# rvignav/diffusion-tts

Hardware: AMD Instinct MI355X
Metric: candidate U-Net steps/sec, EDM ImageNet-64 eps-greedy N=64 (higher is better)
Workload: dtype f16x3; 1 GPU; EDM ImageNet-64 (ADM 295.9M) eps-greedy search iteration, imagenet scorer, sigma step 5/18; candidates_total=64, candidates_per_gpu=64, scorer=imagenet, scorer_dtype=f16x3, denoiser_dtype=f16x3, graph_replay=True, parity_grade=True, parallelism=candidates sharded x1, 1 all-gather of rewards per step

## Files before the change

diffusion_tts_amd/_lib.py:

```python
import ctypes as C
import os

import torch

_HERE = os.path.dirname(os.path.abspath(__file__))
LIB_PATH = os.environ.get('DTS_LIB_PATH') or os.path.join(_HERE, 'libdts_hip.so')

DTS_F32, DTS_BF16, DTS_F16, DTS_F16X3 = 0, 1, 2, 3

_p, _i, _f, _d, _i64 = C.c_void_p, C.c_int, C.c_float, C.c_double, C.c_int64


class ConvArgs(C.Structure):
    _fields_ = [('x1', _p), ('c1', C.c_int32), ('x2', _p), ('c2', C.c_int32), ('w', _p), ('bias', _p),
                ('bias_nc', _p), ('ld_bias_nc', C.c_int32), ('residual', _p), ('out', _p),
                ('n', C.c_int32), ('hin', C.c_int32), ('win', C.c_int32), ('cout', C.c_int32),
                ('ksize', C.c_int32), ('up', C.c_int32), ('out_scale', C.c_float), ('dtype', C.c_int32),
                ('workspace', _p), ('workspace_bytes', C.c_int64), ('stats_out', _p), ('stats_written', C.c_int32),
                ('ev_start', _p), ('ev_stop', _p), ('gn_coef', _p), ('gn_silu', C.c_int32), ('acc_scale', C.c_float), ('out_split2', C.c_int32),
                ('skip_c', C.c_int32), ('skip_x', _p), ('skip_w', _p), ('skip_acc_scale', C.c_float), ('skip_up', C.c_int32)]


class ConvPlanInfo(C.Structure):
    _fields_ = [(f, C.c_int32) for f in ('kernel', 'tile', 'waves', 'stages', 'pf', 'gn', 'sk', 'dbg', 'splits', 'ks_per_split', 'n_ct', 'n_pt', 'nblk',
                                         'threads', 'lds_bytes', 'stats_in_kernel', 'stats_in_reduce', 'stats_written', 'epi_rows', 'fuses_gn',
                                         'folds_skip', 'refused', 'phases')]


SIGNATURES = {
    'dts_nchw_to_nhwc': [_p, _p, _i, _i, _i, _i, _i, _p],
    'dts_nhwc_to_nchw': [_p, _i, _p, _i, _i, _i, _i, _p],
    'dts_nchw_to_nhwc_pad': [_p, _p, _i, _i, _i, _i, _i, _i, _p],
    'dts_pack_conv_weight': [_p, _p, _i, _i, _i, _i, _i, _p, _p],
    'dts_conv2d': [C.POINTER(ConvArgs), _p],
    'dts_conv_in3': [_p, _p, _p, _p, _i, _i, _i, _i, _i, _p],
    'dts_conv_out3': [_p, _i, _p, _p, _p, _i, _i, _i, _i, _p],
    'dts_gn_coef': [_p, _i, _p, _i, _i, _i, _i, _i, _f, _p, _p, _p, _i, _p, _p, _p],
    'dts_gn_coef_strips': [_p, _i, _p, _i, _i, _i, _i, _i, _f, _p, _p, _p, _i, _p, _p],
    'dts_gn_apply': [_p, _i, _p, _i, _i, _p, _p, _i, _i, _i, _i, _i, _p],
    'dts_gn_apply_x3': [_p, _i, _p, _i, _p, _p, _p, _i, _i, _i, _i, _i, _p],
    'dts_gn_fused': [_p, _i, _p, _i, _i, _i, _i, _i, _f, _p, _p, _p, _i, _p, _i, _p],
    'dts_resample2x': [_p, _p, _i, _i, _i, _i, _i, _i, _p],
    'dts_resample_fir': [_p, _p, _i, _i, _i, _i, _i, _i, _i, _p],
    'dts_space_to_depth2': [_p, _i, _p, _i, _i, _i, _i, _i, _i, _i, _p],
    'dts_attention': [_p, _p, _i, _i, _i, _i, _i, _f, _p],
    'dts_attention_masked': [_p, _p, _i, _i, _i, _i, _i, _f, _i, _p, _p],
    'dts_cross_attention': [_p, _p, _p, _i, _p, _i, _i, _i, _i, _i, _i, _f, _p],
    'dts_layer_norm': [_p, _p, _i, _i64, _i, _f, _p, _p, _p],
    'dts_geglu': [_p, _p, _i, _i64, _i, _p],
    'dts_group_rows': [_p, _i, _i64, _p, _p, _p, _p, _p],
    'dts_patchify': [_p, _p, _i, _i, _i, _i, _i, _p],
    'dts_vit_tokens': [_p, _p, _p, _p, _i, _i, _i, _i, _p],
    'dts_text_tokens': [_p, _p, _p, _p, _i, _i, _i, _i, _i, _p],
    'dts_gelu': [_p, _p, _i, _i64, _i, _p],
    'dts_vit_head': [_p, _p, _i, _i, _i, _i, _f, _p, _p, _p],
    'dts_layer_norm_x3': [_p, _p, _p, _i64, _i, _f, _p, _p, _p],
    'dts_gelu_x3': [_p, _p, _i64, _i, _i, _p],
    'dts_patchify_x3': [_p, _p, _i, _i, _i, _i, _p],
    'dts_vit_tokens_f32': [_p, _p, _p, _p, _i, _i, _i, _p],
    'dts_vit_head_f32': [_p, _p, _i, _i, _i, _f, _p, _p, _p],
    'dts_text_tokens_f32': [_p, _p, _p, _p, _i, _i, _i, _i, _p],
    'dts_linear': [_p, _i, _p, _p, _p, _i, _i, _i, _i, _i, _i, _i, _p],
    'dts_pos_embedding': [_p, _p, _p, _i, _i, _i, _p],
    'dts_edm_precond_in': [_p, _p, _i, _f, _p, _p, _i, _i, _p],
    'dts_edm_precond_out': [_p, _p, _p, _p, _i, _i, _p],
    'dts_precond_in': [_i, _p, _p, _i, _p, _p, _i, _p, _p, _i, _i, _p],
    'dts_split3_f16': [_p, _i, _p, _i, _p, _i64, _p],
    'dts_split2_f16': [_p, _i, _p, _i64, _p],
    'dts_attention_x3': [_p, _p, _i, _i, _i, _i, _i, _f, _p],
    'dts_attention_x3_masked': [_p, _p, _i, _i, _i, _i, _i, _f, _i, _p, _p],
    'dts_cast_from_f32': [_p, _p, _i, _i64, _p],
    'dts_cast_to_f32': [_p, _i, _p, _i64, _p],
    'dts_heun_xhat': [_p, _i, _i, _p, _i, _d, _p, _i, _i, _p],
    'dts_heun_euler': [_p, _p, _d, _d, _p, _p, _i64, _p],
    'dts_heun_correct': [_p, _p, _p, _d, _d, _p, _i64, _p],
    'dts_ode_xhat': [_p, _p, _i, _d, _d, _d, _p, _p, _i64, _p],
    'dts_ode_slope': [_p, _p, _d, _d, _p, _d, _d, _p, _p, _p, _i64, _p],
    'dts_ode_correct': [_p, _p, _p, _p, _d, _d, _d, _d, _d, _p, _i64, _p],
    'dts_quantize_u8': [_p, _i, _p, _i64, _p],
    'dts_brightness': [_p, _p, _i, _i, _p],
    'dts_u8_to_unit_f32': [_p, _p, _i64, _p],
    'dts_resample_u8': [_p, _p, _i, _i, _i, _i, _i, _p, _p, _i, _p],
    'dts_lut_u8_f32': [_p, _p, _p, _i, _i, _i, _p],
    'dts_jpeg_size': [_p, _p, _i, _i, _i, _p, _p, _i64, _p, _p],
    'dts_cosine_rows': [_p, _p, _i, _p, _i, _i, _p],
    'dts_attnpool_tokens': [_p, _p, _p, _i, _i, _i, _i, _p],
    'dts_take_token': [_p, _i, _p, _i, _i, _i, _i, _p],
    'dts_softmax_gather': [_p, _p, _p, _i, _i, _p],
    'dts_candidate_noise': [_p, _p, _p, _p, _p, _i, _i, _i, _p],
    'dts_candidate_noise_rows': [_p, _p, _p, _p, _p, _i, _i, _i, _p],
    'dts_candidate_noise_sd': [_p, _p, _p, _p, _p, _i, _i, _i64, _p],
    'dts_candidate_noise_sd_rows': [_p, _p, _p, _p, _p, _i, _i, _i, _i64, _p],
    'dts_cfg_combine': [_p, _p, _f, _p, _i, _i64, _p],
    'dts_ddim_candidates': [_p, _p, _p, _p, _p, _i, _f, _f, _f, _i, _i64, _p],
    'dts_ddim_candidates_groups': [_p, _p, _p, _p, _p, _i, _f, _f, _f, _i, _i, _i64, _p],
}
OTHER = {'dts_version': ([], _i), 'dts_conv_fuses_gn': ([C.POINTER(ConvArgs)], _i), 'dts_conv_kernel': ([C.POINTER(ConvArgs)], _i), 'dts_conv_folds_skip': ([C.POINTER(ConvArgs)], _i), 'dts_conv_takes_phases': ([C.POINTER(ConvArgs)], _i), 'dts_conv_plan': ([C.POINTER(ConvArgs), C.POINTER(ConvPlanInfo)], _i), 'dts_set_tuning': ([_i, _i], _i), 'dts_get_tuning': ([_i], _i), 'dts_last_error': ([], C.c_char_p), 'dts_gn_ws_floats': ([_i, _i], _i64),
         'dts_jpeg_workspace_bytes': ([_i, _i, _i], _i64)}

_lib = None
ABI_VERSION = 125


def load():
    global _lib
    if _lib is not None:
        return _lib
    if not os.path.exists(LIB_PATH):
        raise RuntimeError(f'{LIB_PATH} not found: the HIP extension is required (no CPU fallback). '
                           f'Build it with `python -m diffusion_tts_amd.build` or __graft_entry__.build().')
    lib = C.CDLL(LIB_PATH)
    for name, argt in SIGNATURES.items():
        fn = getattr(lib, name)
        fn.argtypes, fn.restype = argt, _i
    for name, (argt, rest) in OTHER.items():
        fn = getattr(lib, name)
        fn.argtypes, fn.restype = argt, rest
    got = lib.dts_version()
    if got != ABI_VERSION or C.sizeof(ConvArgs) != 208:
        raise RuntimeError(f'{LIB_PATH} has ABI version {got}, this binding needs {ABI_VERSION}: rebuild with `python -m diffusion_tts_amd.build --force`')
    _lib = lib
    return lib


def check(status, what=''):
    if status != 0:
        msg = load().dts_last_error().decode(errors='replace')
        raise RuntimeError(f'libdts_hip {what} failed ({status}): {msg}')


KNOBS = {'att_xcd': 0, 'att_qt': 1, 'conv_tile': 2, 'conv_splits': 3, 'conv_variant': 4, 'gn_fuse': 5, 'att_db': 6, 'conv_stages': 7, 'conv_waves': 8, 'conv_half_round': 9, 'conv_epi32': 10, 'conv_skip_fold': 11, 'conv_up_phases': 12}


def set_tuning(name, value):
    check(load().dts_set_tuning(KNOBS[name], int(value)), 'dts_set_tuning')
```

diffusion_tts_amd/classifier.py:

```python
import math
from typing import Dict

import torch

from . import ops
from .config import ClassifierConfig, ClsLayer, classifier_layers


def _qkv_perm_legacy(heads: int, d: int) -> torch.Tensor:
    s, h, c = torch.meshgrid(torch.arange(3), torch.arange(heads), torch.arange(d), indexing='ij')
    return (h * 3 * d + s * d + c).reshape(-1).to(torch.int32)


class _P:
    pass


class EncoderUNetModel:
    def __init__(self, cfg: ClassifierConfig, state_dict: Dict[str, torch.Tensor], device='cuda', dtype=ops.F16X3):
        if not torch.cuda.is_available():
            raise RuntimeError('EncoderUNetModel (HIP) needs a GPU: there is no CPU fallback in this package')
        self.cfg, self.device, self.dtype = cfg, torch.device(device), dtype
        self.act_dtype = ops.act_dtype(dtype)
        self.x3 = dtype == ops.F16X3
        from .graphs import GraphCache
        self._graphs = GraphCache(self._device_forward)
        f = lambda t: t.detach().to(self.device, torch.float32).contiguous()
        sd, dt = state_dict, dtype
        mc = cfg.model_channels
        half = mc // 2
        self.freqs = torch.exp(-math.log(10000) * torch.arange(0, half, dtype=torch.float32) / half).to(self.device)
        self.te0_w, self.te0_b = f(sd['time_embed.0.weight']), f(sd['time_embed.0.bias'])
        self.te2_w, self.te2_b = f(sd['time_embed.2.weight']), f(sd['time_embed.2.bias'])
        self.layers, self.ch, self.res = classifier_layers(cfg)
        self.params: Dict[str, _P] = {}
        emb_w, emb_b, off = [], [], 0
        hc = cfg.num_head_channels
        for L in self.layers:
            P, p = _P(), L.prefix
            if L.kind == 'conv_in':
                P.w, P.b = f(sd[f'{p}.weight']), f(sd[f'{p}.bias'])
            elif L.kind == 'res':
                P.g0, P.b0 = f(sd[f'{p}.in_layers.0.weight']), f(sd[f'{p}.in_layers.0.bias'])
                P.w0, P.cb0 = ops.pack_conv_weight(f(sd[f'{p}.in_layers.2.weight']), dt), f(sd[f'{p}.in_layers.2.bias'])
                emb_w.append(sd[f'{p}.emb_layers.1.weight'])
                emb_b.append(sd[f'{p}.emb_layers.1.bias'])
                P.off, off = off, off + 2 * L.cout
                P.g1, P.b1 = f(sd[f'{p}.out_layers.0.weight']), f(sd[f'{p}.out_layers.0.bias'])
                P.w1, P.cb1 = ops.pack_conv_weight(f(sd[f'{p}.out_layers.3.weight']), dt), f(sd[f'{p}.out_layers.3.bias'])
                P.sw = P.sb = None
                if L.cin != L.cout:
                    P.sw, P.sb = ops.pack_conv_weight(f(sd[f'{p}.skip_connection.weight']), dt), f(sd[f'{p}.skip_connection.bias'])
                    P.cb1_skip = (P.cb1 + P.sb).contiguous()
            else:
                heads = L.cin // hc
                perm = _qkv_perm_legacy(heads, hc).to(self.device)
                P.g, P.b = f(sd[f'{p}.norm.weight']), f(sd[f'{p}.norm.bias'])
                P.wqkv = ops.pack_conv_weight(f(sd[f'{p}.qkv.weight']), dt, out_perm=perm)
                P.bqkv = f(sd[f'{p}.qkv.bias'])[perm.long()].contiguous()
                P.wproj, P.bproj = ops.pack_conv_weight(f(sd[f'{p}.proj_out.weight']), dt), f(sd[f'{p}.proj_out.bias'])
                P.heads = heads
            self.params[p] = P
        self.emb_w = ops.pack_conv_weight(f(torch.cat(emb_w, 0))[:, :, None, None].contiguous(), dt)
        self.emb_b = f(torch.cat(emb_b, 0))
        self.emb_total = off
        self.out_g, self.out_b = f(sd['out.0.weight']), f(sd['out.0.bias'])
        self.pos = f(sd['out.2.positional_embedding'])
        self.pool_wqkv = ops.pack_conv_weight(f(sd['out.2.qkv_proj.weight']), dt)
        self.pool_bqkv = f(sd['out.2.qkv_proj.bias'])
        self.cproj_w = f(sd['out.2.c_proj.weight']).reshape(cfg.out_channels, self.ch).contiguous()
        self.cproj_b = f(sd['out.2.c_proj.bias'])
        torch.cuda.synchronize(self.device)

    def _res(self, L: ClsLayer, x, emb_all):
        P = self.params[L.prefix]
        raw = self.x3 and P.sw is not None
        h = ops.group_norm(x, 32, 1e-5, P.g0, P.b0, silu=True, pool=L.down, split_out=self.x3, raw_split=raw)
        if raw:
            h, x = h
        elif L.down:
            x = ops.resample2x(x, up=False)
        h = ops.conv2d(h, P.w0, P.cb0, gn_stats=True)
        ss = emb_all[:, P.off:P.off + 2 * L.cout]
        h = ops.group_norm(h, 32, 1e-5, P.g1, P.b1, scale_shift=ss, silu=True, split_out=self.x3)
        if raw and ops.conv_folds_skip(h, P.w1, (x, P.sw, False)):
            return ops.conv2d(h, P.w1, P.cb1_skip, skip=(x, P.sw, False), gn_stats=True)
        sk = x if P.sw is None else ops.conv2d(x, P.sw, P.sb)
        return ops.conv2d(h, P.w1, P.cb1, residual=sk, gn_stats=True)

    def _attn(self, L: ClsLayer, x):
        P = self.params[L.prefix]
        n, hh, ww, c = x.shape
        hn = ops.group_norm(x, 32, 1e-5, P.g, P.b, silu=False, split_out=self.x3)
        fx3 = self.x3 and ops.attention_x3_ok(hh * ww, c // P.heads)
        qkv = ops.conv2d(hn, P.wqkv, P.bqkv, out_split2=fx3)
        a = ops.attention(qkv.view(n, hh * ww, 3 * c), P.heads, 1.0 / math.sqrt(c // P.heads), x3=self.x3, split_out=fx3)
        a = ops.SplitAct(a.data.view(n, hh, ww, 2 * c), c) if fx3 else a.view(n, hh, ww, c)
        return ops.conv2d(a, P.wproj, P.bproj, residual=x, gn_stats=True)

    @torch.no_grad()
    def __call__(self, x, timesteps):
        t = timesteps.to(self.device, torch.float32).contiguous()
        return self._graphs(x.to(self.device, torch.float32).contiguous(), t)

    @torch.no_grad()
    def _device_forward(self, x, t):
        n = x.shape[0]
        emb = ops.pos_embedding(t, self.freqs)
        emb = ops.linear(emb, self.te0_w, self.te0_b, act_out=True)
        emb = ops.linear(emb, self.te2_w, self.te2_b, act_out=True)
        e = ops.cast_from_f32(emb, self.act_dtype)
        emb_all = ops.conv2d(e.view(1, n, 1, -1), self.emb_w, self.emb_b).view(n, self.emb_total)
        h = None
        for L in self.layers:
            if L.kind == 'conv_in':
                P = self.params[L.prefix]
                h = ops.conv_in3(x.contiguous(), P.w, P.b, L.cout, self.act_dtype)
            elif L.kind == 'res':
                h = self._res(L, h, emb_all)
            else:
                h = self._attn(L, h)
        h = ops.group_norm(h, 32, 1e-5, self.out_g, self.out_b, silu=True)
        tok = ops.attnpool_tokens(h, self.pos)
        nt = tok.shape[1]
        qkv = ops.conv2d(tok.view(n, nt, 1, self.ch), self.pool_wqkv, self.pool_bqkv)
        heads = self.ch // self.cfg.num_head_channels
        a = ops.attention(qkv.view(n, nt, 3 * self.ch), heads, 1.0 / math.sqrt(self.cfg.num_head_channels), x3=self.x3)
        return ops.linear(ops.take_token(a, 0), self.cproj_w, self.cproj_b)
```

diffusion_tts_amd/csrc/conv_igemm.hip:

```cpp
#include "dts_common.h"
#include <hip/hip_ext.h>
#include <type_traits>

static_assert(sizeof(dts_conv_args) == 208, "dts_conv_args layout changed: bump DTS_ABI_VERSION and update the bindings (_lib.py ConvArgs)");

int dts_conv_launch_phase_form(const void* plan, const void* params, const void* call);

namespace {

struct ConvCall {
  hipStream_t st;
  hipEvent_t ev_start = nullptr, ev_stop = nullptr;
};

struct ConvP {
  const char* x1; const char* x2;
  const char* w;
  const float* bias;
  const char* bias_nc;
  const char* residual;
  char* out;
  int c1, c2, cin;
  int ld_bias_nc;
  int n, hin, win, hout, wout, cout;
  int taps;
  int up;
  int P;
  int n_ct;
  int n_pt;
  int splits;
  int ks_per_split;
  float* partial;
  float* stats;
  float out_scale;
  float acc_scale;
  int out_split2;
  int w_shift, hw_shift;
  const float* gn_coef;
  int gn_silu;
  int epi_rows;
  const char* sk_x; const char* sk_w;
  int sk_c, sk_up;
  float sk_ratio;
};

template <typename T> struct Mma;
template <> struct Mma<bf16_t> {
  static __device__ __forceinline__ void run(f32x4_t& acc, const uint4& a, const uint4& b) {
    acc = __builtin_amdgcn_mfma_f32_16x16x32_bf16(__builtin_bit_cast(bf16x8_t, a), __builtin_bit_cast(bf16x8_t, b), acc, 0, 0, 0);
  }
};
template <> struct Mma<f16_t> {
  static __device__ __forceinline__ void run(f32x4_t& acc, const uint4& a, const uint4& b) {
    acc = __builtin_amdgcn_mfma_f32_16x16x32_f16(__builtin_bit_cast(f16x8_t, a), __builtin_bit_cast(f16x8_t, b), acc, 0, 0, 0);
  }
};
template <> struct Mma<float> {
  static __device__ __forceinline__ void run(f32x4_t& acc, const uint4& a, const uint4& b) {
    acc = __builtin_amdgcn_mfma_f32_16x16x4f32(__builtin_bit_cast(float, a.x), __builtin_bit_cast(float, b.x), acc, 0, 0, 0);
    acc = __builtin_amdgcn_mfma_f32_16x16x4f32(__builtin_bit_cast(float, a.y), __builtin_bit_cast(float, b.y), acc, 0, 0, 0);
    acc = __builtin_amdgcn_mfma_f32_16x16x4f32(__builtin_bit_cast(float, a.z), __builtin_bit_cast(float, b.z), acc, 0, 0, 0);
    acc = __builtin_amdgcn_mfma_f32_16x16x4f32(__builtin_bit_cast(float, a.w), __builtin_bit_cast(float, b.w), acc, 0, 0, 0);
  }
};

__device__ __forceinline__ uint4 f16x8_mul_2m11(const uint4& v) {
  const f16x8_t h = __builtin_bit_cast(f16x8_t, v) * (_Float16)0x1p-11f;
  return __builtin_bit_cast(uint4, h);
}

template <typename T> struct Vec4;
template <> struct Vec4<float> {
  using type = float4;
  static __device__ __forceinline__ void unpack(const float4& v, float* f) { f[0] = v.x; f[1] = v.y; f[2] = v.z; f[3] = v.w; }
  static __device__ __forceinline__ float4 pack(const float* f) { return make_float4(f[0], f[1], f[2], f[3]); }
  static __device__ __forceinline__ void load(const float* p, float* f) {
    const float4 v = *reinterpret_cast<const float4*>(p);
    f[0] = v.x; f[1] = v.y; f[2] = v.z; f[3] = v.w;
  }
  static __device__ __forceinline__ void store(float* p, const float* f) {
    *reinterpret_cast<float4*>(p) = make_float4(f[0], f[1], f[2], f[3]);
  }
};
template <> struct Vec4<bf16_t> {
  using type = uint2;
  static __device__ __forceinline__ uint2 pack(const float* f) {
    return make_uint2(pack2_bf16(f[0], f[1]), pack2_bf16(f[2], f[3]));
  }
  static __device__ __forceinline__ void unpack(const uint2& v, float* f) {
    f[0] = __builtin_bit_cast(float, v.x << 16); f[1] = __builtin_bit_cast(float, v.x & 0xffff0000u);
    f[2] = __builtin_bit_cast(float, v.y << 16); f[3] = __builtin_bit_cast(float, v.y & 0xffff0000u);
  }
  static __device__ __forceinline__ void load(const bf16_t* p, float* f) {
    const uint2 v = *reinterpret_cast<const uint2*>(p);
    f[0] = bf16_bits_to_f32(v.x & 0xffffu); f[1] = bf16_bits_to_f32(v.x >> 16);
    f[2] = bf16_bits_to_f32(v.y & 0xffffu); f[3] = bf16_bits_to_f32(v.y >> 16);
  }
  static __device__ __forceinline__ void store(bf16_t* p, const float* f) {
    *reinterpret_cast<uint2*>(p) = make_uint2(pack2_bf16(f[0], f[1]), pack2_bf16(f[2], f[3]));
  }
};
template <> struct Vec4<f16_t> {
  using type = uint2;
  static __device__ __forceinline__ uint2 pack(const float* f) {
    return make_uint2(pack2_f16(f[0], f[1]), pack2_f16(f[2], f[3]));
  }
  static __device__ __forceinline__ void unpack(const uint2& v, float* f) {
    f[0] = f16_bits_to_f32(v.x & 0xffffu); f[1] = f16_bits_to_f32(v.x >> 16);
    f[2] = f16_bits_to_f32(v.y & 0xffffu); f[3] = f16_bits_to_f32(v.y >> 16);
  }
  static __device__ __forceinline__ void load(const f16_t* p, float* f) {
    const uint2 v = *reinterpret_cast<const uint2*>(p);
    f[0] = f16_bits_to_f32(v.x & 0xffffu); f[1] = f16_bits_to_f32(v.x >> 16);
    f[2] = f16_bits_to_f32(v.y & 0xffffu); f[3] = f16_bits_to_f32(v.y >> 16);
  }
  static __device__ __forceinline__ void store(f16_t* p, const float* f) {
    *reinterpret_cast<uint2*>(p) = make_uint2(pack2_f16(f[0], f[1]), pack2_f16(f[2], f[3]));
  }
};

#ifdef DTS_STAMPS
__device__ unsigned long long g_stamps[8192 * 8];
#define DTS_STAMP(slot_)                                                                                       \
  if (threadIdx.x == 0 && (blockIdx.x + blockIdx.y * gridDim.x) < 8192) {                                       \
    unsigned long long t_;                                                                                      \
    asm volatile("s_memtime %0\n\ts_waitcnt lgkmcnt(0)" : "=s"(t_)::"memory");                                 \
    g_stamps[(blockIdx.x + blockIdx.y * gridDim.x) * 8 + (slot_)] = t_;                                         \
  }
// ... 150 lines not shown
    const int hw = kp.hout * kp.wout;
#pragma unroll
    for (int nt = 0; nt < NT; ++nt) {
      const int pp = tm.pix(prow0 + nt * 16);
      np[nt] = bnc + (size_t)(kp.hw_shift >= 0 ? pp >> kp.hw_shift : pp / hw) * kp.ld_bias_nc + cm0 + col0;
    }
  }
  constexpr bool want_stats = STATS && NT == 4;
  float* sp = want_stats ? kp.stats + ((size_t)tm.strip(wn) * p_cout + cm0 + col0) * 2 : nullptr;
  char* sw = smem + prow0 * ROWB + (lq & 1) * 8;
  int coff[MT];
#pragma unroll
  for (int mt = 0; mt < MT; ++mt) coff[mt] = (((wm * 2 * MT + 2 * mt + (lq >> 1)) ^ (lrow & 7)) << 4);
  const float osc = kp.out_scale;
  if constexpr (RES) {
    if (early_u0 > 0 || early_u1 < ITERS) {
      asm volatile("s_waitcnt vmcnt(0)" ::: "memory");
      __syncthreads();
    }
  }
#pragma unroll
  for (int mt = 0; mt < MT; ++mt) {
    V4 nv[NT], rv[NT];
    if constexpr (BNC) {
#pragma unroll
      for (int nt = 0; nt < NT; ++nt) nv[nt] = *reinterpret_cast<const V4*>(np[nt] + mt * 16);
    }
    if constexpr (RES) {
#pragma unroll
      for (int nt = 0; nt < NT; ++nt) rv[nt] = *reinterpret_cast<const V4*>(sw + nt * 16 * ROWB + coff[mt]);
    }
    typedef float f32x2 __attribute__((ext_vector_type(2)));
    f32x2 ssa = {0.f, 0.f}, ssb = {0.f, 0.f}, sqa = {0.f, 0.f}, sqb = {0.f, 0.f};
#pragma unroll
    for (int nt = 0; nt < NT; ++nt) {
      f32x2 va = {acc[mt][nt][0], acc[mt][nt][1]}, vb = {acc[mt][nt][2], acc[mt][nt][3]};
      if constexpr (BNC) {
        float f[4];
        Vec4<T>::unpack(nv[nt], f);
        va += f32x2{f[0], f[1]}; vb += f32x2{f[2], f[3]};
      }
      if constexpr (RES) {
        float f[4];
        Vec4<T>::unpack(rv[nt], f);
        va += f32x2{f[0], f[1]}; vb += f32x2{f[2], f[3]};
      }
      va *= osc; vb *= osc;
      const float v[4] = {va.x, va.y, vb.x, vb.y};
      const V4 pk = Vec4<T>::pack(v);
      *reinterpret_cast<V4*>(sw + nt * 16 * ROWB + coff[mt]) = pk;
      if constexpr (want_stats) {
        float f[4];
        Vec4<T>::unpack(pk, f);
        const f32x2 fa = {f[0], f[1]}, fb = {f[2], f[3]};
        ssa += fa; ssb += fb;
        sqa = __builtin_elementwise_fma(fa, fa, sqa); sqb = __builtin_elementwise_fma(fb, fb, sqb);
      }
    }
    if constexpr (want_stats) {
      float ss4[4] = {ssa.x, ssa.y, ssb.x, ssb.y}, sq4[4] = {sqa.x, sqa.y, sqb.x, sqb.y};
      row16_sum8(ss4, sq4);
      if (lrow == 0) {
        float4* d = reinterpret_cast<float4*>(sp + mt * 32);
        d[0] = make_float4(ss4[0], sq4[0], ss4[1], sq4[1]);
        d[1] = make_float4(ss4[2], sq4[2], ss4[3], sq4[3]);
      }
    }
  }
  DTS_STAMP(6);
  __syncthreads();
  DTS_STAMP(7);
  int row = tid / CPR, c = tid - row * CPR;
  char* outb = kp.out + (size_t)cm0 * 2;
  typedef unsigned int u32x4_nt __attribute__((ext_vector_type(4)));
#pragma unroll
  for (int u = 0; u < ITERS; ++u) {
    const u32x4_nt v_ = *reinterpret_cast<const u32x4_nt*>(smem + row * ROWB + c * 16);
    __builtin_nontemporal_store(v_, reinterpret_cast<u32x4_nt*>(outb + (size_t)tm.pix(row) * rstride + ((c ^ (row & 7)) << 4)));
    row += DR; c += DC;
    if (c >= CPR) { c -= CPR; ++row; }
  }
}

template <int MT, int NT, typename TM = TileMap>
__device__ __forceinline__ void conv_epilogue_rows_f32(const ConvP& kp, f32x4_t (&acc)[MT][NT], int cm0, const TM& tm, int wm, int wn,
                                                       int lrow, int lq, char* smem, int wave) {
  static_assert(NT == 4, "64-pixel wave strips");
  constexpr int CW = 16 * MT;
  constexpr int LPR = 4 * MT;
  constexpr int RPI = LPR <= 8 ? 8 : (LPR <= 16 ? 4 : 2);
  constexpr int ITERS = 32 / RPI;
  constexpr int ROWB = CW * 4 + 16;
  char* const ws = smem + (size_t)wave * (32 * ROWB);
  const int lane = threadIdx.x & 63;
  const int rsub = lane / LPR, c4 = lane - rsub * LPR;
  const bool act = rsub < RPI;
  const int p_cout = kp.cout;
  const int co = cm0 + wm * CW + c4 * 4;
  const float* __restrict__ res = reinterpret_cast<const float*>(kp.residual);
  if (tm.pix(wn * 64) >= kp.P) return;
  float4 b4 = make_float4(0.f, 0.f, 0.f, 0.f), n4 = make_float4(0.f, 0.f, 0.f, 0.f);
  if (act) {
    if (kp.bias) b4 = *reinterpret_cast<const float4*>(kp.bias + co);
    if (kp.bias_nc) {
      const int pp0 = tm.pix(wn * 64), hw = kp.hout * kp.wout;
      n4 = *reinterpret_cast<const float4*>(reinterpret_cast<const float*>(kp.bias_nc) + (size_t)(kp.hw_shift >= 0 ? pp0 >> kp.hw_shift : pp0 / hw) * kp.ld_bias_nc + co);
    }
  }
  const float asc = kp.acc_scale, osc = kp.out_scale;
  const bool want_stats = kp.stats != nullptr;
  float ss4[4] = {0.f, 0.f, 0.f, 0.f}, sq4[4] = {0.f, 0.f, 0.f, 0.f};
  typedef float f32x4_nt __attribute__((ext_vector_type(4)));
  constexpr int CH = ITERS < 8 ? ITERS : 8;
#pragma unroll
  for (int half = 0; half < 2; ++half) {
#pragma unroll
    for (int n2 = 0; n2 < 2; ++n2)
#pragma unroll
      for (int mt = 0; mt < MT; ++mt)
        *reinterpret_cast<f32x4_t*>(ws + (n2 * 16 + lrow) * ROWB + (mt * 16 + lq * 4) * 4) = acc[mt][half * 2 + n2];
#pragma unroll
   for (int u0 = 0; u0 < ITERS; u0 += CH) {
    size_t prow[CH];
    float4 rv[CH];
#pragma unroll
    for (int u = 0; u < CH; ++u) {
      prow[u] = (size_t)tm.pix(wn * 64 + half * 32 + (u0 + u) * RPI + (act ? rsub : 0)) * p_cout + co;
      rv[u] = make_float4(0.f, 0.f, 0.f, 0.f);
      if (res && act) rv[u] = *reinterpret_cast<const float4*>(res + prow[u]);
    }
#pragma unroll
    for (int u = 0; u < CH; ++u) {
      if (!act) continue;
      const f32x4_t a = *reinterpret_cast<const f32x4_t*>(ws + ((u0 + u) * RPI + rsub) * ROWB + c4 * 16);
      float v[4] = {a[0] * asc + b4.x, a[1] * asc + b4.y, a[2] * asc + b4.z, a[3] * asc + b4.w};
      if (kp.bias_nc) { v[0] += n4.x; v[1] += n4.y; v[2] += n4.z; v[3] += n4.w; }
      if (res) { v[0] += rv[u].x; v[1] += rv[u].y; v[2] += rv[u].z; v[3] += rv[u].w; }
#pragma unroll
      for (int r = 0; r < 4; ++r) v[r] *= osc;
      if (kp.out_split2) {
        float hi[4], lo[4];
#pragma unroll
        for (int r = 0; r < 4; ++r) x2_split(v[r], hi[r], lo[r]);
        const uint2 h = make_uint2(pack2_f16(hi[0], hi[1]), pack2_f16(hi[2], hi[3])), l = make_uint2(pack2_f16(lo[0], lo[1]), pack2_f16(lo[2], lo[3]));
        const bool odd = (c4 & 1) != 0;
        const uint32_t rx = (uint32_t)__builtin_amdgcn_update_dpp(0, (int)(odd ? h.x : l.x), 0xB1, 0xf, 0xf, false);
        const uint32_t ry = (uint32_t)__builtin_amdgcn_update_dpp(0, (int)(odd ? h.y : l.y), 0xB1, 0xf, 0xf, false);
        if (kp.epi_rows == 2) {
          f16_t* o8 = reinterpret_cast<f16_t*>(kp.out) + 2 * (prow[u] - co) + co;
          *reinterpret_cast<uint2*>(o8) = h;
          *reinterpret_cast<uint2*>(o8 + p_cout) = l;
          continue;
        }
        f16_t* orow = reinterpret_cast<f16_t*>(kp.out) + 2 * (prow[u] - co) + (odd ? co - 4 + p_cout : co);
        *reinterpret_cast<uint4*>(orow) = odd ? make_uint4(rx, ry, l.x, l.y) : make_uint4(h.x, h.y, rx, ry);
      } else {
        const f32x4_nt o = {v[0], v[1], v[2], v[3]};
        __builtin_nontemporal_store(o, reinterpret_cast<f32x4_nt*>(reinterpret_cast<float*>(kp.out) + prow[u]));
      }
      if (want_stats) {
#pragma unroll
        for (int r = 0; r < 4; ++r) { ss4[r] += v[r]; sq4[r] += v[r] * v[r]; }
      }
    }
   }
  }
  if (want_stats) {
#pragma unroll
    for (int r = 0; r < 4; ++r) {
      float s_ = ss4[r], q_ = sq4[r];
#pragma unroll
      for (int k = 1; k < RPI; ++k) { s_ += __shfl(ss4[r], c4 + k * LPR, 64); q_ += __shfl(sq4[r], c4 + k * LPR, 64); }
      ss4[r] = s_; sq4[r] = q_;
    }
    if (rsub == 0) {
      float4* d = reinterpret_cast<float4*>(kp.stats + ((size_t)tm.strip(wn) * p_cout + co) * 2);
      d[0] = make_float4(ss4[0], sq4[0], ss4[1], sq4[1]);
      d[1] = make_float4(ss4[2], sq4[2], ss4[3], sq4[3]);
    }
  }
}

template <typename T, int MT, int NT, int BM, int BN, int NTHR, int RING, typename TM = TileMap>
__device__ __forceinline__ void conv_epilogue(const ConvP& kp, f32x4_t (&acc)[MT][NT], int cm0, const TM& tm, int split, int wm, int wn,
                                              int lrow, int lq, char* smem, bool bias_in_acc, int stage_off, int early_u0, int early_u1) {
  const int p_P = kp.P, p_cout = kp.cout, p_hout = kp.hout, p_wout = kp.wout;
  if (kp.splits > 1) {
    float* part = kp.partial + (size_t)split * p_P * p_cout;
#pragma unroll
    for (int nt = 0; nt < NT; ++nt) {
      const int pp = tm.pix(wn * 16 * NT + nt * 16 + lrow);
      if (pp >= p_P) continue;
#pragma unroll
      for (int mt = 0; mt < MT; ++mt) {
        const int co = cm0 + wm * 16 * MT + mt * 16 + lq * 4;
        *reinterpret_cast<float4*>(part + (size_t)pp * p_cout + co) =
            make_float4(acc[mt][nt][0], acc[mt][nt][1], acc[mt][nt][2], acc[mt][nt][3]);
      }
    }
    return;
  }
  if constexpr (sizeof(T) == 4 && NT == 4) {
    constexpr int NWV = NTHR / 64;
    static_assert(NWV * 32 * (16 * MT * 4 + 16) <= RING, "the waves' private transpose slices must fit the caller's LDS ring");
    if (kp.epi_rows && (p_hout * p_wout) % 64 == 0) {
      conv_epilogue_rows_f32<MT, NT>(kp, acc, cm0, tm, wm, wn, lrow, lq, smem, (int)(threadIdx.x >> 6));
      return;
    }
  }
  if constexpr (sizeof(T) == 2) {
    if (tm.pn0 + BN <= p_P) {
      const bool r_ = kp.residual != nullptr, b_ = kp.bias_nc != nullptr, s_ = NT == 4 && kp.stats != nullptr;
#define DTS_EPI(R_, B_, S_) conv_epilogue_fast<T, MT, NT, BM, BN, R_, B_, S_, NTHR>(kp, acc, cm0, tm, wm, wn, lrow, lq, smem, bias_in_acc, stage_off, early_u0, early_u1)
      if (r_) { if (b_) { if (s_) DTS_EPI(true, true, true); else DTS_EPI(true, true, false); }
                else    { if (s_) DTS_EPI(true, false, true); else DTS_EPI(true, false, false); } }
      else    { if (b_) { if (s_) DTS_EPI(false, true, true); else DTS_EPI(false, true, false); }
                else    { if (s_) DTS_EPI(false, false, true); else DTS_EPI(false, false, false); } }
#undef DTS_EPI
      return;
    }
  }
  const T* __restrict__ res = reinterpret_cast<const T*>(kp.residual);
  const T* __restrict__ bnc = reinterpret_cast<const T*>(kp.bias_nc);
  T* __restrict__ out = reinterpret_cast<T*>(kp.out);
  const int hw = p_hout * p_wout;
  using V4 = typename Vec4<T>::type;
  int ppv[NT], nsv[NT];
#pragma unroll
  for (int nt = 0; nt < NT; ++nt) {
    const int pp = tm.pix(wn * 16 * NT + nt * 16 + lrow);
    ppv[nt] = pp < p_P ? pp : -1;
    nsv[nt] = pp < p_P ? pp / hw : 0;
  }
  constexpr int RG = (sizeof(T) == 4 && MT > 4) ? 2 : MT;
  static_assert(MT % RG == 0, "residual slice groups");
  V4 rv[RG][NT], nv[NT];
  float4 bv[MT];
#pragma unroll
  for (int mt = 0; mt < MT; ++mt)
    bv[mt] = (kp.bias && !bias_in_acc) ? *reinterpret_cast<const float4*>(kp.bias + cm0 + wm * 16 * MT + mt * 16 + lq * 4) : make_float4(0.f, 0.f, 0.f, 0.f);
  const float asc = kp.acc_scale;
  constexpr bool VIA_LDS = sizeof(T) == 2;
  constexpr int ROWP = BM * 2 + 16;
  static_assert(!VIA_LDS || BN * ROWP <= RING, "staged tile must fit the caller's LDS ring");
  const bool want_stats = NT == 4 && kp.stats != nullptr;
  float* sp = want_stats ? kp.stats + ((size_t)tm.strip(wn) * p_cout) * 2 : nullptr;
#pragma unroll
  for (int mt = 0; mt < MT; ++mt) {
    const int co = cm0 + wm * 16 * MT + mt * 16 + lq * 4;
    const float4 bcur = bv[mt];
    if (res && mt % RG == 0) {
#pragma unroll
      for (int m2 = 0; m2 < RG; ++m2) {
        const int co_ = cm0 + wm * 16 * MT + (mt + m2) * 16 + lq * 4;
#pragma unroll
        for (int nt = 0; nt < NT; ++nt)
          if (ppv[nt] >= 0) rv[m2][nt] = *reinterpret_cast<const V4*>(res + (size_t)ppv[nt] * p_cout + co_);
      }
    }
    if (bnc) {
#pragma unroll
      for (int nt = 0; nt < NT; ++nt)
        if (ppv[nt] >= 0) nv[nt] = *reinterpret_cast<const V4*>(bnc + (size_t)nsv[nt] * kp.ld_bias_nc + co);
    }
    float ss4[4] = {0.f, 0.f, 0.f, 0.f}, sq4[4] = {0.f, 0.f, 0.f, 0.f};
#pragma unroll
    for (int nt = 0; nt < NT; ++nt) {
      if (ppv[nt] < 0) continue;
      float v[4];
      v[0] = acc[mt][nt][0] * asc + bcur.x; v[1] = acc[mt][nt][1] * asc + bcur.y;
      v[2] = acc[mt][nt][2] * asc + bcur.z; v[3] = acc[mt][nt][3] * asc + bcur.w;
      if (bnc) {
        float f[4];
        Vec4<T>::unpack(nv[nt], f);
#pragma unroll
        for (int r = 0; r < 4; ++r) v[r] += f[r];
      }
      if (res) {
        float f[4];
        Vec4<T>::unpack(rv[mt % RG][nt], f);
#pragma unroll
        for (int r = 0; r < 4; ++r) v[r] += f[r];
      }
#pragma unroll
      for (int r = 0; r < 4; ++r) v[r] *= kp.out_scale;
      const V4 pk = Vec4<T>::pack(v);
      if constexpr (VIA_LDS)
        *reinterpret_cast<V4*>(smem + (wn * 16 * NT + nt * 16 + lrow) * ROWP + (wm * 16 * MT + mt * 16 + lq * 4) * 2) = pk;
      else if (sizeof(T) == 4 && kp.out_split2) {
        float hi[4], lo[4];
#pragma unroll
        for (int r = 0; r < 4; ++r) x2_split(v[r], hi[r], lo[r]);
        f16_t* orow = reinterpret_cast<f16_t*>(kp.out) + (size_t)ppv[nt] * 2 * p_cout + co;
        *reinterpret_cast<uint2*>(orow) = make_uint2(pack2_f16(hi[0], hi[1]), pack2_f16(hi[2], hi[3]));
        *reinterpret_cast<uint2*>(orow + p_cout) = make_uint2(pack2_f16(lo[0], lo[1]), pack2_f16(lo[2], lo[3]));
      } else
        *reinterpret_cast<V4*>(out + (size_t)ppv[nt] * p_cout + co) = pk;
      if (want_stats) {
        float f[4];
        Vec4<T>::unpack(pk, f);
#pragma unroll
        for (int r = 0; r < 4; ++r) { ss4[r] += f[r]; sq4[r] += f[r] * f[r]; }
      }
    }
    if (want_stats) {
#pragma unroll
      for (int r = 0; r < 4; ++r) {
#pragma unroll
        for (int o = 1; o < 16; o <<= 1) { ss4[r] += __shfl_xor(ss4[r], o, 64); sq4[r] += __shfl_xor(sq4[r], o, 64); }
      }
      if (lrow == 0 && tm.pix(wn * 64) < p_P) {
        float4* d = reinterpret_cast<float4*>(sp + (size_t)co * 2);
        d[0] = make_float4(ss4[0], sq4[0], ss4[1], sq4[1]);
        d[1] = make_float4(ss4[2], sq4[2], ss4[3], sq4[3]);
      }
    }
  }
  if constexpr (VIA_LDS) {
    __syncthreads();
    constexpr int CPR = BM / 8;
    char* outb = kp.out + (size_t)cm0 * 2;
    const int rows = min(BN, p_P - tm.pn0);
#pragma unroll 4
    for (int t = threadIdx.x; t < rows * CPR; t += NTHR) {
      const int row = t / CPR, c = t - row * CPR;
      typedef unsigned int u32x4_nt __attribute__((ext_vector_type(4)));
      const u32x4_nt v_ = *reinterpret_cast<const u32x4_nt*>(smem + row * ROWP + c * 16);
      __builtin_nontemporal_store(v_, reinterpret_cast<u32x4_nt*>(outb + (size_t)tm.pix(row) * p_cout * 2 + c * 16));
    }
  }
}

template <typename T, int MT, int NT, int WM, int WN, bool PF, int STAGES = 2, typename OT = T, bool PH = false>
__global__ __launch_bounds__(64 * WM * WN, (WM * WN == 8 || STAGES == 2 ? 2 : 1)) void conv_igemm_kernel(const ConvP kp) {
  const char* const p_x1 = kp.x1; const char* const p_x2 = kp.x2; const char* const p_w = kp.w;
  const int p_c1 = kp.c1, p_c2 = kp.c2, p_cin = kp.cin, p_hin = kp.hin, p_win = kp.win, p_hout = kp.hout, p_wout = kp.wout;
  const int p_taps = kp.taps, p_up = kp.up, p_P = kp.P, p_n_ct = kp.n_ct, p_n_pt = kp.n_pt;
  constexpr int NW = WM * WN;
  constexpr bool X3I = !std::is_same<T, OT>::value;
  static_assert(!X3I || std::is_same<T, f16_t>::value, "split precision runs on the f16 matrix instruction");
  static_assert(!PH || X3I, "the phase form is the split-precision mode's");
  static_assert(NW == 4 || NW == 8, "4 or 8 waves");
  static_assert(STAGES >= 2 && STAGES <= 4, "ring depth");
  constexpr int SLAB = 8 * NW;
  constexpr int BM = 16 * MT * WM;
  constexpr int BN = 16 * NT * WN;
  constexpr int EPV = ET<T>::EPV;
  constexpr int BKE = 8 * EPV;
  constexpr int ES = 16 / EPV;
  constexpr int RA = BM / SLAB;
  constexpr int RB = BN / SLAB;
  static_assert(BM % SLAB == 0 && BN % SLAB == 0, "tile rows must split over the waves x 8 rows");
  constexpr int A_BYTES = BM * 128, B_BYTES = BN * 128, STAGE_BYTES = A_BYTES + B_BYTES;
  extern __shared__ __attribute__((aligned(16))) char smem[];
  DTS_STAMP_RT(4);
  DTS_STAMP(0);

  const int nblk = p_n_ct * p_n_pt * (PH ? 4 : 1);
  int bid = blockIdx.x;
  {
    const int q = nblk >> 3, r = nblk & 7, xcd = bid & 7, j = bid >> 3;
    bid = (xcd < r ? xcd * (q + 1) : r * (q + 1) + (xcd - r) * q) + j;
  }
  const int ct = bid % p_n_ct, pt = PH ? (bid / p_n_ct) >> 2 : bid / p_n_ct;
  const int cm0 = ct * BM, pn0 = pt * BN;
  const int phase = PH ? (bid / p_n_ct) & 3 : 0, ph_y = phase >> 1, ph_x = phase & 1;
  const int g_h = PH ? p_hin : p_hout, g_w = PH ? p_win : p_wout, g_P = PH ? p_P >> 2 : p_P;
  const int g_hw_shift = PH ? kp.hw_shift - 2 : kp.hw_shift, g_w_shift = PH ? kp.w_shift - 1 : kp.w_shift;

  const int tid = threadIdx.x, lane = tid & 63, wid = tid >> 6;
  const int wm = wid % WM, wn = wid / WM;
  const int chunk = tid & 7, r0 = tid >> 3;

  int pix_n[RB], pix_hw[RB];
  const int K = p_taps * p_cin;
  const int steps_per_tap = p_cin / BKE;
  const int nk_all = p_taps * steps_per_tap;
  const int ks_begin = blockIdx.y * kp.ks_per_split;
  const int ks_end = min(nk_all, ks_begin + kp.ks_per_split);

  const int schunk = (chunk ^ (r0 & 7)) * 16;
  const char* zsrc = reinterpret_cast<const char*>(g_zero16);
  const char* arow[RA];
  const char* brow[RB];
  const uint32_t lds_base = (uint32_t)(uintptr_t)(__attribute__((address_space(3))) char*)smem;
  const uint32_t wave_rows = __builtin_amdgcn_readfirstlane(lds_base + (tid >> 6) * 8 * 128);

#define SET_ROWS(tap_, ci0_)                                                                                  \
  {                                                                                                           \
    const int dh_ = PH ? ((tap_) >> 1) - 1 + ph_y : ((p_taps == 9) ? (tap_) / 3 - 1 : 0);                     \
    const int dw_ = PH ? ((tap_) & 1) - 1 + ph_x : ((p_taps == 9) ? (tap_) % 3 - 1 : 0);                      \
    const char* xb; int cs, cofs;                                                                             \
    if ((ci0_) < p_c1) { xb = p_x1; cs = p_c1; cofs = (ci0_); } else { xb = p_x2; cs = p_c2; cofs = (ci0_) - p_c1; } \
    _Pragma("unroll") for (int j = 0; j < RB; ++j) {                                                          \
      const int hu = (pix_hw[j] >> 16) + dh_, wu = (pix_hw[j] & 0xffff) + dw_;                                \
      const bool ok = pix_n[j] >= 0 && (unsigned)hu < (unsigned)g_h && (unsigned)wu < (unsigned)g_w;          \
      const int hs = (!PH && p_up) ? (hu >> 1) : hu, ws = (!PH && p_up) ? (wu >> 1) : wu;                     \
      brow[j] = ok ? xb + ((size_t)(pix_n[j] + hs * p_win + ws) * cs + cofs) * ES + schunk : zsrc;            \
    }                                                                                                         \
  }
#define ISSUE_TILE(buf_)                                                                                      \
  {                                                                                                           \
    const uint32_t sa_ = wave_rows + (buf_) * STAGE_BYTES;                                                    \
    const uint32_t sb_ = sa_ + A_BYTES;                                                                       \
    _Pragma("unroll") for (int j = 0; j < RA; ++j) glds16(arow[j], sa_ + j * SLAB * 128);                     \
    _Pragma("unroll") for (int j = 0; j < RB; ++j) glds16(brow[j], sb_ + j * SLAB * 128);                     \
  }
#define ADVANCE_K()                                                                                           \
  {                                                                                                           \
    ci0 += BKE;                                                                                               \
    _Pragma("unroll") for (int j = 0; j < RA; ++j) arow[j] += BKE * ES;                                       \
    if (ci0 == p_cin) { ci0 = 0; ++tap; SET_ROWS(tap, 0); }                                                   \
    else if (ci0 == p_c1) { SET_ROWS(tap, ci0); }                                                             \
    else { _Pragma("unroll") for (int j = 0; j < RB; ++j) brow[j] += BKE * ES; }                              \
  }

// ... 61 lines not shown
  static_assert(STAGED_BYTES % PIECE == 0 && STAGED_BYTES <= RING_BYTES, "staged tile pieces");
  const bool res_early = sizeof(OT) == 2 && kp.residual != nullptr && kp.splits == 1 && pn0 + BN <= p_P;
  int stage_off = 0, early_u0 = 0, early_u1 = 0;
  int buf = 0;
  for (int ks = ks_begin; ks < ks_end; ++ks) {
    const char* sa = smem + buf * STAGE_BYTES + (wm * 16 * MT) * 128;
    const char* sb = smem + buf * STAGE_BYTES + A_BYTES + (wn * 16 * NT) * 128;
    uint4 fa[MT], fb[NT], ga[MT], gb[NT];
#pragma unroll
    for (int i = 0; i < NT; ++i) fb[i] = *reinterpret_cast<const uint4*>(sb + swz(i * 16 + lrow, lq));
#pragma unroll
    for (int i = 0; i < MT; ++i) fa[i] = *reinterpret_cast<const uint4*>(sa + swz(i * 16 + lrow, lq));
    if (PF) {
#pragma unroll
      for (int i = 0; i < NT; ++i) gb[i] = *reinterpret_cast<const uint4*>(sb + swz(i * 16 + lrow, lq + 4));
#pragma unroll
      for (int i = 0; i < MT; ++i) ga[i] = *reinterpret_cast<const uint4*>(sa + swz(i * 16 + lrow, lq + 4));
    }
    if (ks + STAGES - 1 < ks_end) {
      ADVANCE_K();
      int wr = buf + STAGES - 1;
      if (wr >= STAGES) wr -= STAGES;
      ISSUE_TILE(wr);
    } else if (res_early && ks + 1 == ks_end) {
      const int lo_free = buf * STAGE_BYTES, hi_free = (STAGES - 1 - buf) * STAGE_BYTES;
      int f0, f1;
      if (lo_free >= hi_free) { f0 = 0; f1 = lo_free; stage_off = 0; }
      else { f0 = (buf + 1) * STAGE_BYTES; f1 = RING_BYTES; stage_off = min(f0, RING_BYTES - STAGED_BYTES); }
      early_u0 = max(0, (f0 - stage_off + PIECE - 1) / PIECE);
      early_u1 = min(PIECES, max(0, (f1 - stage_off) / PIECE));
      if (early_u1 < early_u0) early_u1 = early_u0;
      issue_residual_pieces<BM, 64 * NW>(kp, cm0, linear_tile(pn0), lds_base + stage_off, tid, early_u0, early_u1);
    }
    uint4 fs[X3I ? MT : 1];
    if constexpr (X3I) {
#pragma unroll
      for (int i = 0; i < MT; ++i) fs[i] = f16x8_mul_2m11(fa[i]);
    }
    __builtin_amdgcn_s_setprio(1);
#pragma unroll
    for (int i = 0; i < MT; ++i)
#pragma unroll
      for (int j = 0; j < NT; ++j) Mma<T>::run(acc[i][j], fa[i], fb[j]);
    if (!PF) {
      __builtin_amdgcn_s_setprio(0);
#pragma unroll
      for (int i = 0; i < NT; ++i) gb[i] = *reinterpret_cast<const uint4*>(sb + swz(i * 16 + lrow, lq + 4));
#pragma unroll
      for (int i = 0; i < MT; ++i) ga[i] = *reinterpret_cast<const uint4*>(sa + swz(i * 16 + lrow, lq + 4));
      __builtin_amdgcn_s_setprio(1);
    }
    if constexpr (X3I) {
#pragma unroll
      for (int i = 0; i < MT; ++i)
#pragma unroll
        for (int j = 0; j < NT; ++j) Mma<T>::run(acc[i][j], fs[i], gb[j]);
#pragma unroll
      for (int i = 0; i < MT; ++i)
#pragma unroll
        for (int j = 0; j < NT; ++j) Mma<T>::run(acc[i][j], ga[i], fb[j]);
    } else {
#pragma unroll
      for (int i = 0; i < MT; ++i)
#pragma unroll
        for (int j = 0; j < NT; ++j) Mma<T>::run(acc[i][j], ga[i], gb[j]);
    }
    __builtin_amdgcn_s_setprio(0);
    if constexpr (STAGES > 2) {
      const int later = min(STAGES - 2, ks_end - 2 - ks);
      if (later >= 2) asm volatile("s_waitcnt vmcnt(%0) lgkmcnt(0)" ::"n"(2 * LPT) : "memory");
      else if (later == 1) asm volatile("s_waitcnt vmcnt(%0) lgkmcnt(0)" ::"n"(LPT) : "memory");
      else asm volatile("s_waitcnt vmcnt(0) lgkmcnt(0)" ::: "memory");
    } else {
      asm volatile("s_waitcnt vmcnt(0) lgkmcnt(0)" ::: "memory");
    }
    __syncthreads();
    if (++buf == STAGES) buf = 0;
  }

  DTS_STAMP(2);
  if constexpr (PH) {
    const bool sh = kp.hw_shift >= 0;
    const PhaseTileMap tm{pn0, ph_y, ph_x, p_win, p_hin * p_win, sh ? g_w_shift : -1, sh ? g_hw_shift : -1};
    conv_epilogue<OT, MT, NT, BM, BN, 64 * NW, RING_BYTES>(kp, acc, cm0, tm, (int)blockIdx.y, wm, wn, lrow, lq, smem, bias_in_acc, stage_off, early_u0, early_u1);
  } else
  conv_epilogue<OT, MT, NT, BM, BN, 64 * NW, RING_BYTES>(kp, acc, cm0, linear_tile(pn0), (int)blockIdx.y, wm, wn, lrow, lq, smem, bias_in_acc, stage_off, early_u0, early_u1);
  DTS_STAMP(3);
  DTS_STAMP_RT(5);
}
#undef SET_ROWS
#undef ISSUE_TILE
#undef ADVANCE_K

template <typename T>
__device__ __forceinline__ uint4 gn_act8(const uint4 v, const float (&ca)[8], const float (&cb)[8], int silu) {
  float f[8];
  unpack16<T>(v, f);
#pragma unroll
  for (int e = 0; e < 8; ++e) {
    const float y = f[e] * ca[e] + cb[e];
    f[e] = silu ? y * __builtin_amdgcn_rcpf(1.0f + __expf(-y)) : y;
  }
  return pack16<T>(f);
}

template <typename T, int TAPS, int DBG = 0, bool GN = false, int MT = 6, typename OT = T, bool SK = false>
__global__ __launch_bounds__(512, 2) void conv_pp_kernel(const ConvP kp) {
  static_assert(MT == 6 || MT == 4, "cout tile");
  constexpr bool X3I = !std::is_same<T, OT>::value;
  static_assert(!X3I || (std::is_same<T, f16_t>::value && DBG == 0 && !GN), "split precision: the shipped f16 form only");
  constexpr int NT = 4, GM = 16 * MT, BM = 2 * GM, BN = 256, NTHR = 512, AJ = MT / 2;
  constexpr int BKE = 64, ES = 2;
  constexpr int A_HALF = GM * 128, A_RING = 3 * A_HALF, H_OFF = 2 * A_RING, H_BUF = 328 * 128;
  extern __shared__ __attribute__((aligned(16))) char smem[];
  DTS_STAMP_RT(4);
  DTS_STAMP(0);
  const char* const p_x1 = kp.x1; const char* const p_x2 = kp.x2; const char* const p_w = kp.w;
  const int p_c1 = kp.c1, p_c2 = kp.c2, p_cin = kp.cin, W = kp.wout, H = kp.hout, Wi = kp.win, Hi = kp.hin, ups = kp.up ? 1 : 0;
  constexpr int p_taps = TAPS;
  const int p_n_ct = kp.n_ct, p_n_pt = kp.n_pt;

  const int nblk = p_n_ct * p_n_pt;
  int bid = blockIdx.x;
  {
    const int q = nblk >> 3, r = nblk & 7, xcd = bid & 7, j = bid >> 3;
    bid = (xcd < r ? xcd * (q + 1) : r * (q + 1) + (xcd - r) * q) + j;
  }
  const int ct = bid % p_n_ct, pt = bid / p_n_ct;
  const int cm0 = ct * BM;

  const int tid = threadIdx.x, lane = tid & 63;
  const int w = __builtin_amdgcn_readfirstlane(tid >> 6);
  const int grp = w >> 2, wi = w & 3;
  const int wm = grp, wn = wi;
  const int chunk = lane & 7, r0 = lane >> 3;
  const int lrow = lane & 15, lq = lane >> 4;

  const int hw = H * W;
  TileMap tm;
  tm.pn0 = pt * BN; tm.w = W;
  int img0, y0 = 0, x0 = 0;
  if (W >= 32) {
    const int tpr = W >> 4, tpi = tpr * (H >> 4);
    const int tin = pt & (tpi - 1);
    img0 = pt / tpi;
    y0 = (tin / tpr) << 4; x0 = (tin & (tpr - 1)) << 4;
    tm.patch = 1; tm.porg = img0 * hw + y0 * W + x0;
    tm.strip0 = img0 * (hw >> 6) + tin * 4;
  } else {
    img0 = tm.pn0 / hw;
    tm.patch = 0; tm.porg = 0; tm.strip0 = tm.pn0 >> 6;
  }
  constexpr int bd = (p_taps == 9) ? 1 : 0;
  constexpr int hwid = 16 + 2 * bd;
  constexpr int hr_total = hwid * hwid;
  constexpr int npieces = (hr_total + 7) / 8;
  constexpr int NHP = (npieces + 7) / 8;

  const int K = p_taps * p_cin;
  const int nk_all = p_taps * (p_cin / BKE);
  const int ks_begin = blockIdx.y * kp.ks_per_split;
  const int ks_end = min(nk_all, ks_begin + kp.ks_per_split);
  const int nk = ks_end - ks_begin;

  const int schunk = (chunk ^ (r0 & 7)) * 16;
  const uint32_t lds_base = (uint32_t)(uintptr_t)(__attribute__((address_space(3))) char*)smem;

  const dts_i32x4 rs_w = make_rsrc(p_w, (uint32_t)((size_t)kp.cout * K * ES));
  uint32_t avo[AJ];
#pragma unroll
  for (int j = 0; j < AJ; ++j) avo[j] = DBG == 5 ? DTS_OOR : (uint32_t)((cm0 + grp * GM + 8 * (wi + 4 * j) + r0) * K) * ES + schunk;
  const uint32_t a_dst = lds_base + grp * A_RING + (8 * wi) * 128;
  const uint32_t h_dst = lds_base + H_OFF + (8 * w) * 128;

  int hpix[NHP];
#pragma unroll
  for (int j = 0; j < NHP; ++j) {
    const int hr = 8 * (w + 8 * j) + r0;
    hpix[j] = -1;
    if (hr < hr_total) {
      const int hy = hr / hwid, hx = hr - hy * hwid;
      const int y = y0 + hy - bd, x = x0 + hx - bd;
      if ((unsigned)y < (unsigned)H && (unsigned)x < (unsigned)W) hpix[j] = (img0 * Hi + (y >> ups)) * Wi + (x >> ups);
    }
  }
  uint32_t hvo[NHP];
  uint32_t hval = 0;
#pragma unroll
  for (int j = 0; j < NHP; ++j) hval |= (hpix[j] >= 0 ? 1u : 0u) << j;
// ... 250 lines not shown
    static_assert(X3I, "skip fold: split precision only");
    const int sC = kp.sk_c, nks = sC / BKE, su = kp.sk_up & 1, Hs = H >> su, Ws = W >> su;
    const float ratio = kp.sk_ratio;
#pragma unroll
    for (int i = 0; i < MT; ++i)
#pragma unroll
      for (int j = 0; j < NT; ++j) acc[i][j] *= ratio;
    constexpr int S_A = BM * 128, S_B = BN * 128, B_OFF = 2 * S_A;
    static_assert(B_OFF + 3 * S_B <= H_OFF + 2 * H_BUF, "skip fold: the rings fit the kernel's LDS");
    dts_i32x4 rs_sw = make_rsrc(kp.sk_w, (uint32_t)((size_t)kp.cout * sC * ES));
    dts_i32x4 rs_sx = make_rsrc(kp.sk_x, (uint32_t)((size_t)kp.n * Hs * Ws * sC * ES));
#pragma unroll
    for (int e = 0; e < 4; ++e) { rs_sw[e] = __builtin_amdgcn_readfirstlane(rs_sw[e]); rs_sx[e] = __builtin_amdgcn_readfirstlane(rs_sx[e]); }
    uint32_t savo[AJ], sbvo[4];
#pragma unroll
    for (int j = 0; j < AJ; ++j) savo[j] = (uint32_t)((cm0 + 8 * (w + 8 * j) + r0) * sC) * ES + schunk;
#pragma unroll
    for (int j = 0; j < 4; ++j) {
      const int pl = 8 * (w + 8 * j) + r0, y = y0 + (pl >> 4), x = x0 + (pl & 15);
      sbvo[j] = (uint32_t)(((img0 * Hs + (y >> su)) * Ws + (x >> su)) * sC) * ES + schunk;
    }
    const uint32_t sa_dst = lds_base + (8 * w) * 128, sb_dst = lds_base + B_OFF + (8 * w) * 128;
#define SK_ISSUE_A(kt_, slot_)                                                                                 \
    {                                                                                                         \
      const uint32_t so_ = (uint32_t)(kt_) * 128u, d_ = sa_dst + (uint32_t)(slot_) * S_A;                      \
      _Pragma("unroll") for (int j = 0; j < AJ; ++j) bdma16(savo[j], rs_sw, so_, d_ + j * (64 * 128));         \
    }
#define SK_ISSUE_B(kt_, slot_)                                                                                 \
    {                                                                                                         \
      const uint32_t so_ = (uint32_t)(kt_) * 128u, d_ = sb_dst + (uint32_t)(slot_) * S_B;                      \
      _Pragma("unroll") for (int j = 0; j < 4; ++j) bdma16(sbvo[j], rs_sx, so_, d_ + j * (64 * 128));          \
    }
    SK_ISSUE_A(0, 0);
    SK_ISSUE_B(0, 0);
    if (nks > 1) SK_ISSUE_B(1, 1);
    int bs = 0;
#pragma unroll 1
    for (int kt = 0; kt < nks; ++kt) {
      if (kt + 1 < nks) asm volatile("s_waitcnt vmcnt(4)" ::: "memory");
      else asm volatile("s_waitcnt vmcnt(0)" ::: "memory");
      asm volatile("s_barrier" ::: "memory");
      __builtin_amdgcn_sched_barrier(0);
      const int as = kt & 1;
      if (kt + 1 < nks) SK_ISSUE_A(kt + 1, as ^ 1);
      if (kt + 2 < nks) SK_ISSUE_B(kt + 2, bs == 0 ? 2 : bs - 1);
      const char* sa = smem + as * S_A + (grp * GM) * 128;
      const char* sb = smem + B_OFF + bs * S_B;
      bs = bs == 2 ? 0 : bs + 1;
      uint4 fa[MT], fb[NT], ga[MT], gb[NT], fs[MT];
#pragma unroll
      for (int i = 0; i < NT; ++i) fb[i] = *reinterpret_cast<const uint4*>(sb + swz(wn * 64 + i * 16 + lrow, lq));
#pragma unroll
      for (int i = 0; i < MT; ++i) fa[i] = *reinterpret_cast<const uint4*>(sa + swz(i * 16 + lrow, lq));
#pragma unroll
      for (int i = 0; i < NT; ++i) gb[i] = *reinterpret_cast<const uint4*>(sb + (swz(wn * 64 + i * 16 + lrow, lq) ^ 64));
#pragma unroll
      for (int i = 0; i < MT; ++i) ga[i] = *reinterpret_cast<const uint4*>(sa + (swz(i * 16 + lrow, lq) ^ 64));
      __builtin_amdgcn_sched_barrier(0);
#pragma unroll
      for (int i = 0; i < MT; ++i) fs[i] = f16x8_mul_2m11(fa[i]);
      __builtin_amdgcn_sched_barrier(0);
      __builtin_amdgcn_s_setprio(1);
#pragma unroll
      for (int i = 0; i < MT; ++i)
#pragma unroll
        for (int j = 0; j < NT; ++j) Mma<T>::run(acc[i][j], fa[i], fb[j]);
#pragma unroll
      for (int i = 0; i < MT; ++i)
#pragma unroll
        for (int j = 0; j < NT; ++j) Mma<T>::run(acc[i][j], fs[i], gb[j]);
#pragma unroll
      for (int i = 0; i < MT; ++i)
#pragma unroll
        for (int j = 0; j < NT; ++j) Mma<T>::run(acc[i][j], ga[i], fb[j]);
      __builtin_amdgcn_s_setprio(0);
      __builtin_amdgcn_sched_barrier(0);
    }
#undef SK_ISSUE_A
#undef SK_ISSUE_B
  }
  __syncthreads();
  DTS_STAMP(2);

  conv_epilogue<OT, MT, NT, BM, BN, NTHR, H_OFF + 2 * H_BUF>(kp, acc, cm0, tm, (int)blockIdx.y, wm, wn, lrow, lq, smem, bias_in_acc, 0, 0, 0);
  DTS_STAMP(3);
  DTS_STAMP_RT(5);
}

template <typename T, int SPLITS>
__global__ __launch_bounds__(256) void conv_splitk_reduce_kernel(const ConvP kp) {
  const long long total = (long long)kp.P * (kp.cout / 4);
  const T* res = reinterpret_cast<const T*>(kp.residual);
  const T* bnc = reinterpret_cast<const T*>(kp.bias_nc);
  T* out = reinterpret_cast<T*>(kp.out);
  const int hw = kp.hout * kp.wout, c4 = kp.cout / 4;
  const size_t slab = (size_t)kp.P * kp.cout;
  for (long long idx = (long long)blockIdx.x * blockDim.x + threadIdx.x; idx < total; idx += (long long)gridDim.x * blockDim.x) {
    const int pp = (int)(idx / c4), co = (int)(idx - (long long)pp * c4) * 4;
    const float* base = kp.partial + (size_t)pp * kp.cout + co;
    float4 q[SPLITS];
#pragma unroll
    for (int s = 0; s < SPLITS; ++s) q[s] = *reinterpret_cast<const float4*>(base + (size_t)s * slab);
    float v[4] = {0.f, 0.f, 0.f, 0.f};
#pragma unroll
    for (int s = 0; s < SPLITS; ++s) { v[0] += q[s].x; v[1] += q[s].y; v[2] += q[s].z; v[3] += q[s].w; }
    for (int r = 0; r < 4; ++r) v[r] *= kp.acc_scale;
    if (kp.bias) {
      const float4 bv = *reinterpret_cast<const float4*>(kp.bias + co);
      v[0] += bv.x; v[1] += bv.y; v[2] += bv.z; v[3] += bv.w;
    }
    if (bnc) {
      float f[4];
      Vec4<T>::load(bnc + (size_t)(pp / hw) * kp.ld_bias_nc + co, f);
      for (int r = 0; r < 4; ++r) v[r] += f[r];
    }
    if (res) {
      float f[4];
      Vec4<T>::load(res + (size_t)pp * kp.cout + co, f);
      for (int r = 0; r < 4; ++r) v[r] += f[r];
    }
    for (int r = 0; r < 4; ++r) v[r] *= kp.out_scale;
    Vec4<T>::store(out + (size_t)pp * kp.cout + co, v);
  }
}

template <typename T, int SPLITS>
__global__ __launch_bounds__(256) void conv_splitk_reduce_stats_kernel(const ConvP kp) {
  __shared__ float red[16][16][8];
  const int strip = blockIdx.x, q = threadIdx.x & 15, pl = threadIdx.x >> 4;
  const int co = (blockIdx.y * 16 + q) * 4;
  const bool live = co < kp.cout;
  const T* res = reinterpret_cast<const T*>(kp.residual);
  const T* bnc = reinterpret_cast<const T*>(kp.bias_nc);
  T* out = reinterpret_cast<T*>(kp.out);
  const int hw = kp.hout * kp.wout;
  float ss[4] = {0.f, 0.f, 0.f, 0.f}, sq[4] = {0.f, 0.f, 0.f, 0.f};
  if (live) {
    const int p0 = strip * 64 + pl;
    float v[4][4];
#pragma unroll
    for (int i = 0; i < 4; ++i) { v[i][0] = v[i][1] = v[i][2] = v[i][3] = 0.f; }
    {
      const float* base = kp.partial + (size_t)p0 * kp.cout + co;
      const size_t slab = (size_t)kp.P * kp.cout;
      float4 t4[SPLITS][4];
#pragma unroll
      for (int s_ = 0; s_ < SPLITS; ++s_)
#pragma unroll
        for (int i = 0; i < 4; ++i) t4[s_][i] = *reinterpret_cast<const float4*>(base + (size_t)s_ * slab + (size_t)(16 * i) * kp.cout);
#pragma unroll
      for (int s_ = 0; s_ < SPLITS; ++s_)
#pragma unroll
        for (int i = 0; i < 4; ++i) { v[i][0] += t4[s_][i].x; v[i][1] += t4[s_][i].y; v[i][2] += t4[s_][i].z; v[i][3] += t4[s_][i].w; }
    }
    float4 bv = make_float4(0.f, 0.f, 0.f, 0.f);
    if (kp.bias) bv = *reinterpret_cast<const float4*>(kp.bias + co);
    float nb[4] = {0.f, 0.f, 0.f, 0.f};
    if (bnc) Vec4<T>::load(bnc + (size_t)((strip * 64) / hw) * kp.ld_bias_nc + co, nb);
#pragma unroll
    for (int i = 0; i < 4; ++i) {
      const int pp = p0 + 16 * i;
      for (int r = 0; r < 4; ++r) v[i][r] *= kp.acc_scale;
      v[i][0] += bv.x; v[i][1] += bv.y; v[i][2] += bv.z; v[i][3] += bv.w;
      if (bnc) { for (int r = 0; r < 4; ++r) v[i][r] += nb[r]; }
      if (res) {
        float f[4];
        Vec4<T>::load(res + (size_t)pp * kp.cout + co, f);
        for (int r = 0; r < 4; ++r) v[i][r] += f[r];
      }
      for (int r = 0; r < 4; ++r) v[i][r] *= kp.out_scale;
      const typename Vec4<T>::type pk = Vec4<T>::pack(v[i]);
      *reinterpret_cast<typename Vec4<T>::type*>(out + (size_t)pp * kp.cout + co) = pk;
      float f[4];
      Vec4<T>::unpack(pk, f);
      for (int r = 0; r < 4; ++r) { ss[r] += f[r]; sq[r] += f[r] * f[r]; }
    }
  }
  for (int r = 0; r < 4; ++r) { red[pl][q][2 * r] = ss[r]; red[pl][q][2 * r + 1] = sq[r]; }
  __syncthreads();
  if (pl == 0 && live) {
    float o[8];
    for (int j = 0; j < 8; ++j) {
      float a_ = red[0][q][j];
      for (int k = 1; k < 16; ++k) a_ += red[k][q][j];
      o[j] = a_;
    }
    float4* d = reinterpret_cast<float4*>(kp.stats + ((size_t)strip * kp.cout + co) * 2);
    d[0] = make_float4(o[0], o[1], o[2], o[3]);
    d[1] = make_float4(o[4], o[5], o[6], o[7]);
  }
}

constexpr int DTS_MAX_DEVICES = 64;
inline int current_device() {
  int d = 0;
  if (hipGetDevice(&d) != hipSuccess || d < 0 || d >= DTS_MAX_DEVICES) d = 0;
  return d;
}

template <typename T, int SPLITS>
int launch_reduce_n(const ConvP& q, bool with_stats, hipStream_t st) {
  if (with_stats) {
    hipLaunchKernelGGL((conv_splitk_reduce_stats_kernel<T, SPLITS>), dim3(q.P / 64, (q.cout + 63) / 64), dim3(256), 0, st, q);
    DTS_CHECK_LAUNCH("dts_conv2d(split-K reduce + statistics)");
  } else {
    long long g = ((long long)q.P * (q.cout / 4) + 255) / 256;
    if (g > 2048) g = 2048;
    hipLaunchKernelGGL((conv_splitk_reduce_kernel<T, SPLITS>), dim3((int)g), dim3(256), 0, st, q);
    DTS_CHECK_LAUNCH("dts_conv2d(split-K reduce)");
  }
  return DTS_OK;
}
template <typename T>
int launch_reduce(const ConvP& q, bool with_stats, hipStream_t st) {
  switch (q.splits) {
    case 2: return launch_reduce_n<T, 2>(q, with_stats, st);
    case 3: return launch_reduce_n<T, 3>(q, with_stats, st);
    case 4: return launch_reduce_n<T, 4>(q, with_stats, st);
    case 5: return launch_reduce_n<T, 5>(q, with_stats, st);
    case 6: return launch_reduce_n<T, 6>(q, with_stats, st);
    case 7: return launch_reduce_n<T, 7>(q, with_stats, st);
    case 8: return launch_reduce_n<T, 8>(q, with_stats, st);
    default: dts_set_error("dts_conv2d: split-K factor %d outside 2..8", q.splits); return DTS_ERR_ARG;
  }
}


struct ConvKnobs { int variant, tile, splits, stages, waves, half_round, epi32, skip_fold, up_phases; bool f32_tile192; };
ConvKnobs conv_knobs() {
  static const bool f32_192 = !(getenv("DTS_F32_TILE192") && atoi(getenv("DTS_F32_TILE192")) == 0);
  return {dts_knob_get(DTS_KNOB_CONV_VARIANT), dts_knob_get(DTS_KNOB_CONV_TILE), dts_knob_get(DTS_KNOB_CONV_SPLITS),
          dts_knob_get(DTS_KNOB_CONV_STAGES), dts_knob_get(DTS_KNOB_CONV_WAVES), dts_knob_get(DTS_KNOB_CONV_HALF_ROUND),
          dts_knob_get(DTS_KNOB_CONV_EPI32), dts_knob_get(DTS_KNOB_CONV_SKIP_FOLD), dts_knob_get(DTS_KNOB_CONV_UP_PHASES), f32_192};
}

struct ConvPlan : dts_conv_plan_info { char refuse[200]; };

template <auto KERNEL>
int conv_launch(const ConvPlan& pl, const ConvP& q, const ConvCall& call) {
  static bool attr_done[DTS_MAX_DEVICES] = {};
  const int dev = current_device();
  if (!attr_done[dev]) {
    (void)hipFuncSetAttribute(reinterpret_cast<const void*>(KERNEL), hipFuncAttributeMaxDynamicSharedMemorySize, pl.lds_bytes);
    attr_done[dev] = true;
  }
  const dim3 grid(pl.nblk, pl.splits), block(pl.threads);
  if (call.ev_start != nullptr && call.ev_stop != nullptr)
    hipExtLaunchKernelGGL(KERNEL, grid, block, (size_t)pl.lds_bytes, call.st, call.ev_start, call.ev_stop, 0, q);
  else
    hipLaunchKernelGGL(KERNEL, grid, block, (size_t)pl.lds_bytes, call.st, q);
  DTS_CHECK_LAUNCH(pl.kernel != 0 ? "dts_conv2d(ping-pong)" : "dts_conv2d");
  return DTS_OK;
}

template <typename T, typename OT, int MT, int WM, int WN, bool PF, bool PH = false>
int conv_launch_igemm(const ConvPlan& pl, const ConvP& q, const ConvCall& call) {
#define DTS_IGEMM(MT_, WM_, STAGES_) conv_launch<&conv_igemm_kernel<T, MT_, 4, WM_, WN, PF, STAGES_, OT, PH>>(pl, q, call)
  if constexpr (sizeof(T) == 2) {
    if (pl.waves == 8) return pl.stages == 3 ? DTS_IGEMM(MT / 2, WM * 2, 3) : DTS_IGEMM(MT / 2, WM * 2, 2);
    if (pl.stages == 3) return DTS_IGEMM(MT, WM, 3);
    if constexpr (std::is_same<T, OT>::value)
      if (pl.stages == 4) return DTS_IGEMM(MT, WM, 4);
  }
  return DTS_IGEMM(MT, WM, 2);
#undef DTS_IGEMM
}

int igemm_splits(int nblk, int nk, double slab, bool can8, bool x3, bool ws, long long ws_bytes, int forced) {
  const int slots = 512;
  int splits = 1;
  if (ws && nblk < (slots * 3) / 4 && nk >= 16) {
    int smax = 8;
    if (smax > nk / 8) smax = nk / 8;
    while (smax > 1 && (long long)smax * (long long)slab > ws_bytes) --smax;
    if (smax < 1) smax = 1;
    const double KS = x3 ? 1.5 : 1.0;
    auto est = [&](int s_) {
      const int steps = (nk + s_ - 1) / s_;
      double t;
      if (can8 && (long long)nblk * s_ <= 256) t = 5.0 + steps * 0.75 * KS;
      else t = (double)((nblk * s_ + slots - 1) / slots) * (5.5 + steps * 1.25 * KS);
      if (s_ > 1) t += 3.0 + (s_ + 0.5) * slab / 4.0e6;
      return t;
    };
    int best = 1;
    for (int s_ = 2; s_ <= smax; ++s_)
      if (est(s_) < est(best)) best = s_;
    splits = best;
  }
  const int f8 = forced > 8 ? 8 : forced;
  if (f8 > 0 && ws && nk >= 2 * f8 && (long long)f8 * (long long)slab <= ws_bytes) splits = f8;
  return splits;
}

inline bool pp_considers_split(long long nblk) { return nblk < 192; }

int pp_splits(int nblk, int nk, double slab, bool x3, bool ws, long long ws_bytes, int forced) {
  int splits = 1;
  if (!ws || nk < 16) return splits;
  if (forced > 0) splits = forced;
  else if (pp_considers_split(nblk)) {
    const int nchunk = nk / 9;
    double best = 1e30;
    for (int s_ = 1; s_ <= 8 && s_ <= nchunk; ++s_) {
      const int cps = (nchunk + s_ - 1) / s_, se = (nchunk + cps - 1) / cps;
      if (se != s_ || nblk * se > 256) continue;
      double t = 5.0 + cps * 9 * (x3 ? 1.4 : 1.05);
      if (se > 1) t += 3.0 + (se + 0.5) * slab / 4.0e6;
      if (t < best) { best = t; splits = se; }
    }
  }
  if (splits > 8) splits = 8;
  if (forced > 0 && splits > nk / 8) splits = nk / 8;
  if (splits > nk / 9) splits = nk / 9;
  while (splits > 1 && (long long)splits * (long long)slab > ws_bytes) --splits;
  if (splits < 1) splits = 1;
  return splits;
}

bool conv_pp_eligible(int dtype, int ksize, int cout, int c1, int c2, int n, int hin, int win, int up) {
  const int ho = up ? 2 * hin : hin, wo = up ? 2 * win : win;
  const long long P = (long long)n * ho * wo;
  return dtype != DTS_F32 && cout % 192 == 0 && ho == wo && wo >= 16 && (wo & (wo - 1)) == 0 && P % 256 == 0 && P < (1ll << 30) &&
         (long long)n * hin * win * (c1 > c2 ? c1 : c2) * 2 < (1ll << 31) && (long long)cout * ksize * ksize * (c1 + c2) * 2 < (1ll << 31) &&
         (c1 % 64 == 0) && (c2 % 64 == 0);
}

int conv_pick_pp(const ConvKnobs& k, bool f32, const ConvP& p, bool x3) {
  if (f32 || k.variant == 0 || k.tile > 0) return 0;
  if (p.taps != 9) return 0;
  const int mt = p.cout % 192 == 0 ? 6 : (p.cout % 128 == 0 ? 4 : 0);
  if (mt == 0 || !conv_pp_eligible(DTS_BF16, 3, 192, p.c1, p.c2, p.n, p.hin, p.win, p.up)) return 0;
  if ((long long)p.cout * p.taps * p.cin * 2 >= (1ll << 31)) return 0;
  if (p.gn_coef != nullptr) return (mt == 6 && !p.up) ? 6 : 0;
  if (k.variant >= 1) return mt;
  const long long blocks_pp = (long long)(p.cout / (32 * mt)) * ((p.P + 255) / 256);
  const bool short_small = blocks_pp <= 128 && p.taps * (p.cin / 64) <= 27;
  const bool half_round_128 = mt == 4 && blocks_pp > 64 && blocks_pp <= 128 && p.wout >= 32 && p.cout <= 256 && (x3 ? k.half_round == 1 : k.half_round != 0);
  const bool auto_pp = !short_small && !half_round_128;
  return (auto_pp && blocks_pp >= 64) ? mt : 0;
}

int conv_pp_dbg(int variant) {
  if (variant <= 1) return 0;
#ifdef DTS_DIAG_KERNELS
  const int d = variant / 10;
  return (variant % 10 == 1 && d >= 1 && d <= 9 && d != 3) ? d : 0;
#else
  return -1;
#endif
}

template <typename T, typename OT = T>
int conv_launch_plan(const ConvPlan& pl, const ConvP& q, const ConvCall& call) {
  if constexpr (sizeof(T) == 2) {
#define DTS_PP(DBG_, GN_, MT_, SK_) conv_launch<&conv_pp_kernel<T, 9, DBG_, GN_, MT_, OT, SK_>>(pl, q, call)
    if constexpr (!std::is_same<T, OT>::value) {
      if (pl.phases) return dts_conv_launch_phase_form(&pl, &q, &call);
      if (pl.kernel == 6 && pl.sk) return DTS_PP(0, false, 6, true);
      if (pl.kernel == 4 && pl.sk) return DTS_PP(0, false, 4, true);
    } else if (pl.kernel == 6) {
      if (pl.gn) return DTS_PP(0, true, 6, false);
#ifdef DTS_DIAG_KERNELS
      switch (pl.dbg) {
        case 1: return DTS_PP(1, false, 6, false);
        case 2: return DTS_PP(2, false, 6, false);
        case 4: return DTS_PP(4, false, 6, false);
        case 5: return DTS_PP(5, false, 6, false);
        case 6: return DTS_PP(6, false, 6, false);
        case 7: return DTS_PP(7, false, 6, false);
        case 8: return DTS_PP(8, false, 6, false);
        case 9: return DTS_PP(9, false, 6, false);
      }
#endif
    }
    if (pl.kernel == 6) return DTS_PP(0, false, 6, false);
    if (pl.kernel == 4) return DTS_PP(0, false, 4, false);
#undef DTS_PP
  }
  switch (pl.tile) {
    case 192: return pl.pf ? conv_launch_igemm<T, OT, 6, 2, 2, true>(pl, q, call) : conv_launch_igemm<T, OT, 6, 2, 2, false>(pl, q, call);
    case 128: return pl.pf ? conv_launch_igemm<T, OT, 4, 2, 2, true>(pl, q, call) : conv_launch_igemm<T, OT, 4, 2, 2, false>(pl, q, call);
    default: return pl.pf ? conv_launch_igemm<T, OT, 4, 1, 4, true>(pl, q, call) : conv_launch_igemm<T, OT, 4, 1, 4, false>(pl, q, call);
  }
}

void conv_shape_from_args(const dts_conv_args* a, ConvP& p) {
  p.c1 = a->c1; p.c2 = a->c2; p.cin = a->c1 + a->c2;
  p.n = a->n; p.hin = a->hin; p.win = a->win;
  p.hout = a->up ? 2 * a->hin : a->hin; p.wout = a->up ? 2 * a->win : a->win;
  p.cout = a->cout; p.taps = a->ksize * a->ksize; p.up = a->up;
  p.P = (int)((long long)p.n * p.hout * p.wout);
  p.residual = (const char*)a->residual; p.gn_coef = a->gn_coef;
  p.out_split2 = a->out_split2;
}

ConvPlan conv_plan(const dts_conv_args* a) {
  ConvPlan pl{};
  pl.kernel = -1; pl.splits = 1;
  auto refuse = [&](const char* fmt, int v0 = 0, int v1 = 0, int v2 = 0) { pl.refused = 1; snprintf(pl.refuse, sizeof(pl.refuse), fmt, v0, v1, v2); return pl; };
  if (a == nullptr) return refuse("dts_conv2d: null args");
  const ConvKnobs k = conv_knobs();
  const bool f32 = a->dtype == DTS_F32, x3 = a->dtype == DTS_F16X3;
  pl.fuses_gn = a->ksize == 3 && k.variant != 0 && k.tile <= 0 && !a->up &&
                conv_pp_eligible(a->dtype, a->ksize, a->cout, a->c1, a->c2, a->n, a->hin, a->win, a->up) &&
                (k.variant == 1 || (long long)(a->cout / 192) * (((long long)a->n * a->hin * a->win + 255) / 256) >= 64);
  if (a->ksize != 1 && a->ksize != 3) return refuse("dts_conv2d: ksize %d", a->ksize);
  if (a->n <= 0 || a->hin <= 0 || a->win <= 0) return refuse("dts_conv2d: bad shape");
  if (a->cout <= 0) return refuse("dts_conv2d: cout %d must be a multiple of 64", a->cout);
  if ((long long)a->n * a->hin * a->win * (a->up ? 4 : 1) >= (1ll << 30)) return refuse("dts_conv2d: too many pixels");
  ConvP p;
  conv_shape_from_args(a, p);
  const bool ph = a->up == 2;
  if (ph) p.taps = 4;
  const int mt = ph ? 0 : conv_pick_pp(k, f32, p, x3);
  pl.kernel = mt;
  int unit = 1;
  if (mt != 0) {
    pl.n_ct = p.cout / (32 * mt); pl.n_pt = (p.P + 255) / 256;
    pl.threads = 512;
    pl.lds_bytes = (6 * 16 * mt + 2 * 328) * 128;
    unit = 9;
  } else {
    pl.tile = (p.cout % 192 == 0) ? 192 : (p.cout % 128 == 0 ? 128 : 64);
    if (f32 && pl.tile == 192 && !k.f32_tile192) pl.tile = (p.cout % 128 == 0) ? 128 : 64;
    if (k.tile > 0 && p.cout % k.tile == 0) pl.tile = (k.tile == 192 || k.tile == 128) ? k.tile : 64;
    pl.n_ct = p.cout / pl.tile; pl.n_pt = (p.P + (pl.tile == 64 ? 255 : 127)) / (pl.tile == 64 ? 256 : 128);
    if (ph) pl.n_pt = (p.P / 4 + 127) / 128;
    pl.pf = a->ksize == 3 && !f32;
  }
  pl.nblk = pl.n_ct * pl.n_pt * (ph ? 4 : 1);
  const int bke = f32 ? 32 : 64, nk = p.taps * (p.cin / bke);
  pl.gn = a->gn_coef != nullptr;
  {
    const int su = a->skip_up ? 1 : 0;
    pl.folds_skip = x3 && mt != 0 && !a->up && a->residual == nullptr && !a->out_split2 && a->gn_coef == nullptr &&
                    a->skip_c > 0 && a->skip_c % 64 == 0 && k.skip_fold != 0 && k.splits <= 0 && !(su && ((a->hin | a->win) & 1)) &&
                    (!pp_considers_split(pl.nblk) || k.variant == 1) &&
                    (long long)a->n * (a->hin >> su) * (a->win >> su) * a->skip_c * 2 < (1ll << 31) && (long long)a->cout * a->skip_c * 2 < (1ll << 31);
  }
  if (a->cout % 64 != 0) return refuse("dts_conv2d: cout %d must be a multiple of 64", a->cout);
  if (a->c1 <= 0 || a->c1 % bke != 0 || a->c2 % bke != 0) return refuse("dts_conv2d: channels (%d,%d) must be multiples of %d", a->c1, a->c2, bke);
  if ((long long)p.cin * (f32 ? 4 : 2) + 128 > (long long)sizeof(g_zero16))
    return refuse("dts_conv2d: %d input channels exceed the zero-row page (%d bytes)", p.cin, (int)sizeof(g_zero16));
  if (p.hout >= 32768 || p.wout >= 32768) return refuse("dts_conv2d: spatial size too large");
  if (a->out_split2 && !(x3 && a->stats_out == nullptr)) return refuse("dts_conv2d: out_split2 is the split-precision mode's, without strip statistics");
  if (a->acc_scale != 0.f && a->acc_scale != 1.f && !x3) return refuse("dts_conv2d: acc_scale is the split-precision mode's (DTS_F16X3)");
  if (pl.gn && !pl.fuses_gn) return refuse("dts_conv2d: gn_coef given for a launch that cannot fuse the GroupNorm apply (ask dts_conv_fuses_gn first)");
  if (a->skip_c != 0 || a->skip_w != nullptr || a->skip_x != nullptr) {
    if (a->skip_w == nullptr || a->skip_x == nullptr || !pl.folds_skip)
      return refuse("dts_conv2d: skip_* given for a launch that cannot fold the 1x1 skip convolution (ask dts_conv_folds_skip first)");
    pl.sk = true;
  }
  if (pl.gn && x3) return refuse("dts_conv2d: gn_coef is not available in the split-precision mode");
  if (a->dtype < DTS_F32 || a->dtype > DTS_F16X3) return refuse("bad dtype %d", a->dtype);
  if (ph) {
    if (!x3) return refuse("dts_conv2d: up = 2 (phase-packed weights) is the split-precision mode's (DTS_F16X3), dtype %d", a->dtype);
    if (a->ksize != 3) return refuse("dts_conv2d: up = 2 needs ksize 3, got %d", a->ksize);
    if (a->c2 != 0 || a->x2 != nullptr) return refuse("dts_conv2d: up = 2 takes no second input");
    if (a->gn_coef != nullptr || pl.sk || a->out_split2) return refuse("dts_conv2d: up = 2 takes no gn_coef, skip_* or out_split2");
    if (pl.tile == 64) return refuse("dts_conv2d: up = 2 needs cout %d to be a multiple of 128 or 192", a->cout);
    if (a->stats_out != nullptr && (a->hin * a->win) % 64 != 0)
      return refuse("dts_conv2d: up = 2 with strip statistics needs hin*win = %d to be a multiple of 64 (a wave's strip is 64 low-resolution pixels)", a->hin * a->win);
    if (k.up_phases == 0) return refuse("dts_conv2d: up = 2 while DTS_CONV_UP_PHASES=0");
  }
  if (mt == 6 && !x3 && !pl.gn) {
    pl.dbg = conv_pp_dbg(k.variant);
    if (pl.dbg < 0) return refuse("dts_conv2d: DTS_CONV_VARIANT=%d selects a diagnostic kernel that this library was built without (-DDTS_DIAG_KERNELS)", k.variant);
  }
  const bool ws = a->workspace != nullptr && !a->out_split2 && !pl.sk;
  const double slab = (double)p.P * p.cout * 4.0;
  pl.splits = mt != 0 ? pp_splits(pl.nblk, nk, slab, x3, ws, (long long)a->workspace_bytes, k.splits)
                      : igemm_splits(pl.nblk, nk, slab, !f32, x3, ws, (long long)a->workspace_bytes, k.splits);
  {
    const int nunit = nk / unit, per = (nunit + pl.splits - 1) / pl.splits;
    pl.ks_per_split = per * unit;
    pl.splits = (nunit + per - 1) / per;
  }
  if (ph) {
    if (pl.splits > 1) return refuse("dts_conv2d: up = 2 with a K split of %d (the phase form takes none: use the fused-gather route)", pl.splits);
    pl.phases = 1;
  }
  pl.stats_in_kernel = a->stats_out != nullptr && pl.splits == 1;
  pl.stats_in_reduce = a->stats_out != nullptr && pl.splits > 1 && (p.hout * p.wout) % 64 == 0 && p.cout % 4 == 0;
  pl.stats_written = pl.stats_in_kernel || pl.stats_in_reduce;
  pl.epi_rows = k.epi32 < 0 ? (x3 ? 1 : 0) : (k.epi32 == 2 ? 2 : (k.epi32 != 0));
  if (ph && (a->hin * a->win) % 64 != 0) pl.epi_rows = 0;
  if (mt != 0) return pl;
  const bool one_per_cu = (long long)pl.nblk * pl.splits <= 256;
  pl.stages = (one_per_cu && pl.ks_per_split >= 3) ? 3 : 2;
  if (k.stages >= 2 && k.stages <= 4) pl.stages = k.stages;
  if (f32) pl.stages = 2;
  const int stage_bytes = (pl.tile + (pl.tile == 64 ? 256 : 128)) * 128;
  if (pl.stages * stage_bytes > 160 * 1024) pl.stages = 3;
  pl.waves = (!f32 && (k.waves == 8 || (k.waves != 4 && one_per_cu))) ? 8 : 4;
  if (pl.stages == 4 && (pl.waves == 8 || x3)) pl.stages = 3;
  pl.threads = 64 * pl.waves;
  pl.lds_bytes = pl.stages * stage_bytes;
  return pl;
}

}

#ifdef DTS_CONV_PHASE_TU
int dts_conv_launch_phase_form(const void* plan, const void* params, const void* call) {
  const ConvPlan& pl = *static_cast<const ConvPlan*>(plan);
  const ConvP& q = *static_cast<const ConvP*>(params);
  const ConvCall& c = *static_cast<const ConvCall*>(call);
  return pl.tile == 192 ? conv_launch_igemm<f16_t, float, 6, 2, 2, true, true>(pl, q, c) : conv_launch_igemm<f16_t, float, 4, 2, 2, true, true>(pl, q, c);
}
#else

#ifdef DTS_STAMPS
extern "C" int dts_debug_read_stamps(unsigned long long* host, int count) {
  return (int)hipMemcpyFromSymbol(host, HIP_SYMBOL(g_stamps), sizeof(unsigned long long) * (size_t)count);
}
extern "C" int dts_debug_clear_stamps(void) {
  void* p = nullptr;
  if (hipGetSymbolAddress(&p, HIP_SYMBOL(g_stamps)) != hipSuccess) return -1;
  if (hipMemset(p, 0, sizeof(g_stamps)) != hipSuccess) return -1;
  if (hipGetSymbolAddress(&p, HIP_SYMBOL(g_seg)) != hipSuccess) return -1;
  return (int)hipMemset(p, 0, sizeof(g_seg));
}
extern "C" int dts_debug_read_segments(unsigned long long* host, int count) {
  return (int)hipMemcpyFromSymbol(host, HIP_SYMBOL(g_seg), sizeof(unsigned long long) * (size_t)count);
}
#endif

extern "C" int dts_conv_kernel(const dts_conv_args* a) { return conv_plan(a).kernel; }

extern "C" int dts_conv_fuses_gn(const dts_conv_args* a) { return conv_plan(a).fuses_gn ? 1 : 0; }

extern "C" int dts_conv_folds_skip(const dts_conv_args* a) { return conv_plan(a).folds_skip ? 1 : 0; }

extern "C" int dts_conv_takes_phases(const dts_conv_args* a) {
  if (a == nullptr || a->up != 2) return 0;
  const ConvPlan pl = conv_plan(a);
  return (!pl.refused && pl.phases) ? 1 : 0;
}

extern "C" int dts_conv_plan(const dts_conv_args* a, dts_conv_plan_info* out) {
  DTS_CHECK_ARG(out != nullptr, "dts_conv_plan: null output");
  const ConvPlan pl = conv_plan(a);
  *out = pl;
  if (pl.refused) dts_set_error("%s", pl.refuse);
  return pl.kernel < 0 ? DTS_ERR_ARG : DTS_OK;
}

extern "C" int dts_conv2d(dts_conv_args* a, dts_stream s) {
  const ConvPlan pl = conv_plan(a);
  DTS_CHECK_ARG(!pl.refused, "%s", pl.refuse);
  DTS_CHECK_ARG(a->x1 && a->w && a->out, "dts_conv2d: null tensor");
  DTS_CHECK_ARG(a->c2 == 0 || a->x2 != nullptr, "dts_conv2d: c2 without x2");
  DTS_CHECK_ARG(a->bias_nc == nullptr || a->ld_bias_nc >= a->cout, "dts_conv2d: ld_bias_nc");
  ConvP p;
  conv_shape_from_args(a, p);
  if (pl.phases) p.taps = 4;
  DTS_CHECK_ARG(a->stats_out == nullptr || ((p.hout * p.wout) % 64 == 0 && (uintptr_t)a->stats_out % 16 == 0),
                "dts_conv2d: strip statistics need hout*wout to be a multiple of 64 and a 16-byte aligned buffer");
  DTS_CHECK_ARG(a->workspace == nullptr || ((uintptr_t)a->workspace % 16 == 0 && a->workspace_bytes >= 0), "dts_conv2d: workspace");
  p.x1 = (const char*)a->x1; p.x2 = (const char*)a->x2; p.w = (const char*)a->w;
  p.bias = a->bias; p.bias_nc = (const char*)a->bias_nc; p.out = (char*)a->out;
  p.ld_bias_nc = a->ld_bias_nc;
  p.out_scale = a->out_scale; p.acc_scale = a->acc_scale == 0.f ? 1.f : a->acc_scale;
  p.w_shift = p.hw_shift = -1;
  {
    const int hw = p.hout * p.wout;
    if ((p.wout & (p.wout - 1)) == 0 && (hw & (hw - 1)) == 0) { p.w_shift = __builtin_ctz(p.wout); p.hw_shift = __builtin_ctz(hw); }
  }
  p.gn_silu = a->gn_silu;
  p.sk_x = p.sk_w = nullptr; p.sk_c = p.sk_up = 0; p.sk_ratio = 1.f;
  if (pl.sk) {
    const float ss = a->skip_acc_scale == 0.f ? 1.f : a->skip_acc_scale;
    p.sk_x = (const char*)a->skip_x; p.sk_w = (const char*)a->skip_w; p.sk_c = a->skip_c; p.sk_up = a->skip_up ? 1 : 0;
    p.sk_ratio = p.acc_scale / ss; p.acc_scale = ss;
  }
  p.n_ct = pl.n_ct; p.n_pt = pl.n_pt; p.splits = pl.splits; p.ks_per_split = pl.ks_per_split; p.epi_rows = pl.epi_rows;
  p.partial = (float*)a->workspace;
  p.stats = pl.stats_in_kernel ? a->stats_out : nullptr;
  ConvCall call;
  call.st = to_stream(s); call.ev_start = (hipEvent_t)a->ev_start; call.ev_stop = (hipEvent_t)a->ev_stop;
  int rc = DTS_OK;
  if (a->dtype == DTS_F16X3) rc = conv_launch_plan<f16_t, float>(pl, p, call);
  else DTS_DISPATCH_DTYPE(a->dtype, rc = conv_launch_plan<T>(pl, p, call));
  if (rc == DTS_OK && pl.splits > 1) {
    if (pl.stats_in_reduce) p.stats = a->stats_out;
    DTS_DISPATCH_DTYPE(a->dtype == DTS_F16X3 ? DTS_F32 : a->dtype, rc = launch_reduce<T>(p, pl.stats_in_reduce, call.st));
  }
  a->stats_written = pl.stats_written ? 1 : 0;
  return rc;
}
#endif
```

diffusion_tts_amd/csrc/groupnorm.hip:

```cpp
#include "dts_common.h"

namespace {

constexpr int GN_SPLITS = 32;

template <typename T>
__global__ __launch_bounds__(256) void gn_partial_kernel(const T* __restrict__ x1, int c1, const T* __restrict__ x2, int c2,
                                                          int hw, int groups, int splits, float* __restrict__ partial) {
  constexpr int EPV = ET<T>::EPV;
  extern __shared__ float sm[];
  const int C = c1 + c2, cg = C / groups;
  const int nchunk = C / EPV;
  const int slots = nchunk < 256 ? nchunk : 256;
  const int planes = 256 / slots;
  const int n = blockIdx.y, split = blockIdx.x;
  const int per = (hw + splits - 1) / splits;
  const int p0 = split * per, p1 = min(hw, p0 + per);
  const int tid = threadIdx.x;
  const int plane = tid / slots, slot = tid - plane * slots;
  if (plane < planes) {
    for (int chunk = slot; chunk < nchunk; chunk += slots) {
      float s[EPV], ss[EPV];
#pragma unroll
      for (int e = 0; e < EPV; ++e) s[e] = ss[e] = 0.f;
// ... 136 lines not shown
}

__device__ __forceinline__ uint32_t dpp_swap_pair(uint32_t v) {
  return (uint32_t)__builtin_amdgcn_update_dpp(0, (int)v, 0xB1, 0xf, 0xf, false);
}
__device__ __forceinline__ void store_split4_paired(f16_t* orow, int c0, const float* f, bool odd) {
  float hi[4], lo[4];
#pragma unroll
  for (int e = 0; e < 4; ++e) x3_split(f[e], hi[e], lo[e]);
  const uint2 h = make_uint2(pack2_f16(hi[0], hi[1]), pack2_f16(hi[2], hi[3])), l = make_uint2(pack2_f16(lo[0], lo[1]), pack2_f16(lo[2], lo[3]));
  const uint32_t sx = odd ? h.x : l.x, sy = odd ? h.y : l.y;
  const uint32_t rx = dpp_swap_pair(sx), ry = dpp_swap_pair(sy);
  const uint4 v = odd ? make_uint4(rx, ry, l.x, l.y) : make_uint4(h.x, h.y, rx, ry);
  f16_t* d = orow + x3_off(odd ? c0 - 4 : c0) + (odd ? 32 : 0);
  *reinterpret_cast<uint4*>(d) = v;
}

template <typename T, bool SPLIT = false, bool W16 = false>
__global__ __launch_bounds__(256) void gn_apply_rows_kernel(const T* __restrict__ x1, int c1, const T* __restrict__ x2, int c2,
                                                             const float* __restrict__ coef, T* __restrict__ out, int hw, int ppb,
                                                             int silu, f16_t* __restrict__ raw = nullptr) {
  static_assert(!SPLIT || sizeof(T) == 4, "split-precision output is the f32 mode's");
  constexpr int EPV = ET<T>::EPV;
  const int C = c1 + c2, nchunk = C / EPV;
  const int k = blockDim.x / nchunk;
  const int pr = threadIdx.x / nchunk, chunk = threadIdx.x - pr * nchunk;
  const int n = blockIdx.y, c0 = chunk * EPV;
  const bool odd = (chunk & 1) != 0;
#define DTS_STORE_SPLIT(orow_, f_) { if constexpr (W16) store_split4_paired(orow_, c0, f_, odd); else store_split4(orow_, c0, f_); }
  float A[EPV], B[EPV];
#pragma unroll
  for (int e = 0; e < EPV; e += 2) {
    const float4 q = *reinterpret_cast<const float4*>(coef + ((size_t)n * C + c0 + e) * 2);
    A[e] = q.x; B[e] = q.y; A[e + 1] = q.z; B[e + 1] = q.w;
  }
  const T* src; int cs;
  if (c0 < c1) { src = x1 + (size_t)n * hw * c1 + c0; cs = c1; } else { src = x2 + (size_t)n * hw * c2 + (c0 - c1); cs = c2; }
  T* dst = out + (size_t)n * hw * C + c0;
  f16_t* const dst3 = reinterpret_cast<f16_t*>(out) + (size_t)n * hw * 2 * C;
  f16_t* const raw3 = raw ? raw + (size_t)n * hw * 2 * C : nullptr;
  const int p_begin = blockIdx.x * ppb, p_end = min(hw, p_begin + ppb);
  int p = p_begin + pr;
  for (; p + k < p_end; p += 2 * k) {
    const uint4 v0 = *reinterpret_cast<const uint4*>(src + (size_t)p * cs);
    const uint4 v1 = *reinterpret_cast<const uint4*>(src + (size_t)(p + k) * cs);
    float f0[EPV], f1[EPV];
    unpack16<T>(v0, f0);
    unpack16<T>(v1, f1);
    if constexpr (SPLIT) {
      if (raw3) { DTS_STORE_SPLIT(raw3 + (size_t)p * 2 * C, f0); DTS_STORE_SPLIT(raw3 + (size_t)(p + k) * 2 * C, f1); }
    }
#pragma unroll
    for (int e = 0; e < EPV; ++e) {
      const float y0 = f0[e] * A[e] + B[e], y1 = f1[e] * A[e] + B[e];
      f0[e] = silu ? silu_t<T>(y0) : y0;
      f1[e] = silu ? silu_t<T>(y1) : y1;
    }
    if constexpr (SPLIT) {
      DTS_STORE_SPLIT(dst3 + (size_t)p * 2 * C, f0);
      DTS_STORE_SPLIT(dst3 + (size_t)(p + k) * 2 * C, f1);
    } else {
      *reinterpret_cast<uint4*>(dst + (size_t)p * C) = pack16<T>(f0);
      *reinterpret_cast<uint4*>(dst + (size_t)(p + k) * C) = pack16<T>(f1);
    }
  }
  if (p < p_end) {
    const uint4 v0 = *reinterpret_cast<const uint4*>(src + (size_t)p * cs);
    float f0[EPV];
    unpack16<T>(v0, f0);
    if constexpr (SPLIT) {
      if (raw3) DTS_STORE_SPLIT(raw3 + (size_t)p * 2 * C, f0);
    }
#pragma unroll
    for (int e = 0; e < EPV; ++e) { const float y0 = f0[e] * A[e] + B[e]; f0[e] = silu ? silu_t<T>(y0) : y0; }
    if constexpr (SPLIT) DTS_STORE_SPLIT(dst3 + (size_t)p * 2 * C, f0)
    else *reinterpret_cast<uint4*>(dst + (size_t)p * C) = pack16<T>(f0);
  }
}
#undef DTS_STORE_SPLIT

template <typename T, bool POOL, bool SPLIT = false>
__global__ __launch_bounds__(256) void gn_apply_kernel(const T* __restrict__ x1, int c1, const T* __restrict__ x2, int c2,
                                                        const float* __restrict__ coef, T* __restrict__ out,
                                                        int n_total, int h, int w, int silu, f16_t* __restrict__ raw = nullptr) {
  constexpr int EPV = ET<T>::EPV;
  const int C = c1 + c2, nchunk = C / EPV;
  const int ho = POOL ? h / 2 : h, wo = POOL ? w / 2 : w;
  const long long total = (long long)n_total * ho * wo * nchunk;
  for (long long idx = (long long)blockIdx.x * blockDim.x + threadIdx.x; idx < total; idx += (long long)gridDim.x * blockDim.x) {
    const int chunk = (int)(idx % nchunk);
    long long pix = idx / nchunk;
    const int xo = (int)(pix % wo); pix /= wo;
    const int yo = (int)(pix % ho);
    const int n = (int)(pix / ho);
    const int c0 = chunk * EPV;
    const T* base; int cs, co;
    if (c0 < c1) { base = x1; cs = c1; co = c0; } else { base = x2; cs = c2; co = c0 - c1; }
    float A[EPV], B[EPV];
#pragma unroll
    for (int e = 0; e < EPV; e += 2) {
      const float4 q = *reinterpret_cast<const float4*>(coef + ((size_t)n * C + c0 + e) * 2);
      A[e] = q.x; B[e] = q.y; A[e + 1] = q.z; B[e + 1] = q.w;
    }
    float r[EPV], rr[EPV];
    if (!POOL) {
      const uint4 v = *reinterpret_cast<const uint4*>(base + (((size_t)n * h + yo) * w + xo) * cs + co);
      float f[EPV];
      unpack16<T>(v, f);
#pragma unroll
      for (int e = 0; e < EPV; ++e) { rr[e] = f[e]; const float y = f[e] * A[e] + B[e]; r[e] = silu ? silu_t<T>(y) : y; }
    } else {
#pragma unroll
      for (int e = 0; e < EPV; ++e) { r[e] = 0.f; rr[e] = 0.f; }
#pragma unroll
      for (int dy = 0; dy < 2; ++dy)
#pragma unroll
        for (int dx = 0; dx < 2; ++dx) {
          const uint4 v = *reinterpret_cast<const uint4*>(base + (((size_t)n * h + 2 * yo + dy) * w + 2 * xo + dx) * cs + co);
          float f[EPV];
          unpack16<T>(v, f);
#pragma unroll
          for (int e = 0; e < EPV; ++e) { rr[e] += 0.25f * f[e]; const float y = f[e] * A[e] + B[e]; r[e] += 0.25f * (silu ? silu_t<T>(y) : y); }
        }
    }
    if constexpr (SPLIT) {
      store_split4(reinterpret_cast<f16_t*>(out) + (((size_t)n * ho + yo) * wo + xo) * 2 * C, c0, r);
      if (raw) store_split4(raw + (((size_t)n * ho + yo) * wo + xo) * 2 * C, c0, rr);
    } else
      *reinterpret_cast<uint4*>(out + (((size_t)n * ho + yo) * wo + xo) * C + c0) = pack16<T>(r);
  }
}

template <typename T> struct Pair;
template <> struct Pair<float> {
  static __device__ __forceinline__ void load(const float* p, float& a, float& b) { const float2 v = *reinterpret_cast<const float2*>(p); a = v.x; b = v.y; }
  static __device__ __forceinline__ void store(float* p, float a, float b) { *reinterpret_cast<float2*>(p) = make_float2(a, b); }
};
template <> struct Pair<bf16_t> {
  static __device__ __forceinline__ void load(const bf16_t* p, float& a, float& b) {
    const uint32_t v = *reinterpret_cast<const uint32_t*>(p); a = bf16_bits_to_f32(v & 0xffffu); b = bf16_bits_to_f32(v >> 16);
  }
  static __device__ __forceinline__ void store(bf16_t* p, float a, float b) {
    *reinterpret_cast<uint32_t*>(p) = pack2_bf16(a, b);
  }
};
template <> struct Pair<f16_t> {
  static __device__ __forceinline__ void load(const f16_t* p, float& a, float& b) {
    const uint32_t v = *reinterpret_cast<const uint32_t*>(p); a = f16_bits_to_f32(v & 0xffffu); b = f16_bits_to_f32(v >> 16);
  }
  static __device__ __forceinline__ void store(f16_t* p, float a, float b) {
    *reinterpret_cast<uint32_t*>(p) = pack2_f16(a, b);
  }
};

template <typename T>
__global__ __launch_bounds__(256) void gn_fused_kernel(const T* __restrict__ x1, int c1, const T* __restrict__ x2, int c2, int hw,
                                                        int groups, float eps, const float* __restrict__ gamma,
                                                        const float* __restrict__ beta, const T* __restrict__ ss, int ld_ss,
                                                        T* __restrict__ out, int silu) {
  __shared__ double red[2][4];
  __shared__ float sAB[2][64];
  const int C = c1 + c2, cg = C / groups, hp = cg / 2;
  const int g = blockIdx.x, n = blockIdx.y, tid = threadIdx.x;
  const int npair = hw * hp;
  float s = 0.f, q = 0.f;
  for (int e = tid; e < npair; e += 256) {
    const int p = e / hp, c = g * cg + (e - p * hp) * 2;
    const T* src = c < c1 ? x1 + ((size_t)n * hw + p) * c1 + c : x2 + ((size_t)n * hw + p) * c2 + (c - c1);
    float a, b;
    Pair<T>::load(src, a, b);
    s += a + b;
    q += a * a + b * b;
  }
  double ds = wave_sum((double)s), dq = wave_sum((double)q);
  if ((tid & 63) == 0) { red[0][tid >> 6] = ds; red[1][tid >> 6] = dq; }
  __syncthreads();
  if (tid < cg) {
    const double cnt = (double)hw * cg;
    const double mean = (red[0][0] + red[0][1] + red[0][2] + red[0][3]) / cnt;
    double var = (red[1][0] + red[1][1] + red[1][2] + red[1][3]) / cnt - mean * mean;
    if (var < 0.0) var = 0.0;
    const float rstd = (float)(1.0 / sqrt(var + (double)eps));
    const int c = g * cg + tid;
    float A = rstd * (gamma ? gamma[c] : 1.f);
    float B = (beta ? beta[c] : 0.f) - (float)mean * A;
    if (ss) {
      const float sc = 1.f + ld1<T>(ss + (size_t)n * ld_ss + c);
      const float sh = ld1<T>(ss + (size_t)n * ld_ss + C + c);
      A = A * sc;
      B = B * sc + sh;
    }
    sAB[0][tid] = A;
    sAB[1][tid] = B;
  }
  __syncthreads();
  for (int e = tid; e < npair; e += 256) {
    const int p = e / hp, cl = (e - p * hp) * 2, c = g * cg + cl;
    const T* src = c < c1 ? x1 + ((size_t)n * hw + p) * c1 + c : x2 + ((size_t)n * hw + p) * c2 + (c - c1);
    float a, b;
    Pair<T>::load(src, a, b);
    a = a * sAB[0][cl] + sAB[1][cl];
    b = b * sAB[0][cl + 1] + sAB[1][cl + 1];
    if (silu) { a = silu_t<T>(a); b = silu_t<T>(b); }
    Pair<T>::store(out + ((size_t)n * hw + p) * C + c, a, b);
  }
}

template <typename T>
__global__ __launch_bounds__(256) void resample_kernel(const T* __restrict__ x, T* __restrict__ out, int n_total, int h, int w,
                                                        int c, int mode) {
// ... 17 lines not shown
#pragma unroll
      for (int dy = 0; dy < 2; ++dy)
#pragma unroll
        for (int dx = 0; dx < 2; ++dx) {
          const uint4 v = *reinterpret_cast<const uint4*>(x + (((size_t)n * h + 2 * yo + dy) * w + 2 * xo + dx) * c + chunk * EPV);
          float f[EPV];
          unpack16<T>(v, f);
#pragma unroll
          for (int e = 0; e < EPV; ++e) r[e] += 0.25f * f[e];
        }
      o = pack16<T>(r);
    }
    *reinterpret_cast<uint4*>(out + (((size_t)n * ho + yo) * wo + xo) * c + chunk * EPV) = o;
  }
}

inline int gn_splits(int hw) {
  int s = hw / 64;
  if (s < 1) s = 1;
  if (s > GN_SPLITS) s = GN_SPLITS;
  return s;
}

inline int grid_for(long long total, int block) {
  long long g = (total + block - 1) / block;
  if (g > 256 * 16) g = 256 * 16;
  if (g < 1) g = 1;
  return (int)g;
}

}

extern "C" int64_t dts_gn_ws_floats(int n, int groups) { return (int64_t)n * GN_SPLITS * groups * 2; }

extern "C" int dts_gn_coef(const void* x1, int c1, const void* x2, int c2, int dtype, int n, int hw, int groups, float eps,
                           const float* gamma, const float* beta, const void* scale_shift, int ld_ss,
                           float* coef, float* ws, dts_stream s) {
  const int C = c1 + c2;
  DTS_CHECK_ARG(x1 && coef && ws, "dts_gn_coef: null pointer");
  DTS_CHECK_ARG(n > 0 && hw > 0 && groups > 0 && C % groups == 0, "dts_gn_coef: C=%d groups=%d", C, groups);
  DTS_CHECK_ARG(c2 == 0 || x2, "dts_gn_coef: c2 without x2");
  const int epv = dtype == DTS_F32 ? 4 : 8;
  DTS_CHECK_ARG(c1 % epv == 0 && c2 % epv == 0, "dts_gn_coef: channels (%d,%d) unsupported", c1, c2);
  DTS_CHECK_ARG(scale_shift == nullptr || ld_ss >= 2 * C, "dts_gn_coef: ld_ss=%d < 2*C=%d", ld_ss, 2 * C);
  const int splits = gn_splits(hw);
  hipStream_t st = to_stream(s);
  DTS_DISPATCH_DTYPE(dtype, {
    const int nchunk = C / ET<T>::EPV;
    const int planes = 256 / (nchunk < 256 ? nchunk : 256);
    const size_t lds = (size_t)planes * C * 2 * sizeof(float);
    hipLaunchKernelGGL((gn_partial_kernel<T>), dim3(splits, n), dim3(256), lds, st, (const T*)x1, c1, (const T*)x2, c2, hw,
                       groups, splits, ws);
    DTS_CHECK_LAUNCH("dts_gn_coef(partial)");
    const int total = n * C;
    hipLaunchKernelGGL((gn_coef_kernel<T>), dim3((total + 255) / 256), dim3(256), 0, st, ws, splits, groups, C, hw, eps, gamma,
                       beta, (const T*)scale_shift, ld_ss, coef, n);
    DTS_CHECK_LAUNCH("dts_gn_coef(coef)");
  });
  return DTS_OK;
}

extern "C" int dts_gn_coef_strips(const float* st1, int c1, const float* st2, int c2, int dtype, int n, int hw, int groups, float eps,
                                  const float* gamma, const float* beta, const void* scale_shift, int ld_ss, float* coef,
                                  dts_stream s) {
  const int C = c1 + c2;
  DTS_CHECK_ARG(st1 && coef, "dts_gn_coef_strips: null pointer");
  DTS_CHECK_ARG(n > 0 && hw > 0 && hw % 64 == 0 && groups > 0 && C % groups == 0, "dts_gn_coef_strips: hw=%d C=%d groups=%d", hw, C,
                groups);
  DTS_CHECK_ARG(c2 == 0 || st2, "dts_gn_coef_strips: c2 without st2");
  DTS_CHECK_ARG(C / groups <= 128, "dts_gn_coef_strips: %d channels per group (max 128)", C / groups);
  DTS_CHECK_ARG(scale_shift == nullptr || ld_ss >= 2 * C, "dts_gn_coef_strips: ld_ss=%d < 2*C=%d", ld_ss, 2 * C);
  DTS_CHECK_ARG(n <= 65535, "dts_gn_coef_strips: n too large for grid.y");
  hipStream_t st = to_stream(s);
  DTS_DISPATCH_DTYPE(dtype, {
    const int threads = (long long)(hw / 64) * (C / groups) > 4096 ? 256 : 64;
    hipLaunchKernelGGL((gn_coef_strips_kernel<T>), dim3(groups, n), dim3(threads), 0, st, st1, c1, st2, c2, hw / 64, groups, hw, eps,
                       gamma, beta, (const T*)scale_shift, ld_ss, coef);
    DTS_CHECK_LAUNCH("dts_gn_coef_strips");
  });
  return DTS_OK;
}

static int gn_apply_impl(const void* x1, int c1, const void* x2, int c2, int dtype, const float* coef, void* out, int n, int h,
                         int w, int silu, int pool, bool split, dts_stream s, void* raw_out = nullptr);
extern "C" int dts_gn_apply(const void* x1, int c1, const void* x2, int c2, int dtype, const float* coef, void* out, int n, int h,
                            int w, int silu, int pool, dts_stream s) {
  return gn_apply_impl(x1, c1, x2, c2, dtype, coef, out, n, h, w, silu, pool, false, s);
}
extern "C" int dts_gn_apply_x3(const float* x1, int c1, const float* x2, int c2, const float* coef, void* out, void* raw_out, int n, int h,
                               int w, int silu, int pool, dts_stream s) {
  DTS_CHECK_ARG((c1 + c2) % 32 == 0, "dts_gn_apply_x3: %d channels are not a multiple of 32", c1 + c2);
  return gn_apply_impl(x1, c1, x2, c2, DTS_F32, coef, out, n, h, w, silu, pool, true, s, raw_out);
}
static int gn_apply_impl(const void* x1, int c1, const void* x2, int c2, int dtype, const float* coef, void* out, int n, int h,
                         int w, int silu, int pool, bool split, dts_stream s, void* raw_out) {
  const int C = c1 + c2;
  DTS_CHECK_ARG(x1 && coef && out, "dts_gn_apply: null pointer");
  DTS_CHECK_ARG(n > 0 && h > 0 && w > 0 && C > 0, "dts_gn_apply: n=%d h=%d w=%d C=%d", n, h, w, C);
  DTS_CHECK_ARG(c2 == 0 || x2, "dts_gn_apply: c2 without x2");
  const int epv = dtype == DTS_F32 ? 4 : 8;
  DTS_CHECK_ARG(c1 % epv == 0 && c2 % epv == 0, "dts_gn_apply: channels (%d,%d) unsupported", c1, c2);
  DTS_CHECK_ARG(!pool || (h % 2 == 0 && w % 2 == 0), "dts_gn_apply: pool needs even h,w");
  hipStream_t st = to_stream(s);
  const long long total = (long long)n * (pool ? h / 2 : h) * (pool ? w / 2 : w) * (C / epv);
  if (split) {
    using T = float;
    if (pool)
      hipLaunchKernelGGL((gn_apply_kernel<T, true, true>), dim3(grid_for(total, 256)), dim3(256), 0, st, (const T*)x1, c1, (const T*)x2,
                         c2, coef, (T*)out, n, h, w, silu, (f16_t*)raw_out);
    else if (C / epv <= 256 && n <= 65535) {
      const int nchunk = C / epv, k = 256 / nchunk, hw = h * w;
      long long ppb = ((long long)n * hw + 4095) / 4096;
      ppb = ((ppb + 2 * k - 1) / (2 * k)) * (2 * k);
      if (c1 % 8 == 0 && dts_knob_get(DTS_KNOB_GN_FUSE) != 2)
        hipLaunchKernelGGL((gn_apply_rows_kernel<T, true, true>), dim3((unsigned)((hw + ppb - 1) / ppb), n), dim3(k * nchunk), 0, st, (const T*)x1, c1,
                           (const T*)x2, c2, coef, (T*)out, hw, (int)ppb, silu, (f16_t*)raw_out);
      else
      hipLaunchKernelGGL((gn_apply_rows_kernel<T, true>), dim3((unsigned)((hw + ppb - 1) / ppb), n), dim3(k * nchunk), 0, st, (const T*)x1, c1,
                         (const T*)x2, c2, coef, (T*)out, hw, (int)ppb, silu, (f16_t*)raw_out);
    } else
      hipLaunchKernelGGL((gn_apply_kernel<T, false, true>), dim3(grid_for(total, 256)), dim3(256), 0, st, (const T*)x1, c1, (const T*)x2,
                         c2, coef, (T*)out, n, h, w, silu, (f16_t*)raw_out);
    DTS_CHECK_LAUNCH("dts_gn_apply_x3");
    return DTS_OK;
  }
  DTS_DISPATCH_DTYPE(dtype, {
    if (pool)
      hipLaunchKernelGGL((gn_apply_kernel<T, true>), dim3(grid_for(total, 256)), dim3(256), 0, st, (const T*)x1, c1, (const T*)x2,
                         c2, coef, (T*)out, n, h, w, silu);
    else if (C / epv <= 256 && n <= 65535) {
      const int nchunk = C / epv, k = 256 / nchunk, hw = h * w;
      long long ppb = ((long long)n * hw + 4095) / 4096;
      ppb = ((ppb + 2 * k - 1) / (2 * k)) * (2 * k);
      hipLaunchKernelGGL((gn_apply_rows_kernel<T>), dim3((unsigned)((hw + ppb - 1) / ppb), n), dim3(k * nchunk), 0, st, (const T*)x1, c1,
                         (const T*)x2, c2, coef, (T*)out, hw, (int)ppb, silu);
    } else
      hipLaunchKernelGGL((gn_apply_kernel<T, false>), dim3(grid_for(total, 256)), dim3(256), 0, st, (const T*)x1, c1, (const T*)x2,
                         c2, coef, (T*)out, n, h, w, silu);
    DTS_CHECK_LAUNCH("dts_gn_apply");
  });
  return DTS_OK;
}

extern "C" int dts_gn_fused(const void* x1, int c1, const void* x2, int c2, int dtype, int n, int hw, int groups, float eps,
                            const float* gamma, const float* beta, const void* scale_shift, int ld_ss, void* out, int silu,
                            dts_stream s) {
  const int C = c1 + c2;
  DTS_CHECK_ARG(x1 && out, "dts_gn_fused: null pointer");
  DTS_CHECK_ARG(n > 0 && hw > 0 && groups > 0 && C % groups == 0, "dts_gn_fused: C=%d groups=%d", C, groups);
  const int cg = C / groups;
  DTS_CHECK_ARG(cg % 2 == 0 && cg <= 64 && c1 % 2 == 0, "dts_gn_fused: channels per group %d unsupported", cg);
  DTS_CHECK_ARG(c2 == 0 || x2, "dts_gn_fused: c2 without x2");
  DTS_CHECK_ARG(scale_shift == nullptr || ld_ss >= 2 * C, "dts_gn_fused: ld_ss=%d < 2*C=%d", ld_ss, 2 * C);
  DTS_CHECK_ARG(n <= 65535, "dts_gn_fused: n too large for grid.y");
  hipStream_t st = to_stream(s);
  DTS_DISPATCH_DTYPE(dtype, {
    hipLaunchKernelGGL((gn_fused_kernel<T>), dim3(groups, n), dim3(256), 0, st, (const T*)x1, c1, (const T*)x2, c2, hw, groups, eps,
                       gamma, beta, (const T*)scale_shift, ld_ss, (T*)out, silu);
    DTS_CHECK_LAUNCH("dts_gn_fused");
  });
  return DTS_OK;
}

extern "C" int dts_resample2x(const void* x, void* out, int dtype, int n, int h, int w, int c, int mode, dts_stream s) {
  DTS_CHECK_ARG(x && out, "dts_resample2x: null pointer");
  const int epv = dtype == DTS_F32 ? 4 : 8;
  DTS_CHECK_ARG(c % epv == 0, "dts_resample2x: c=%d", c);
  DTS_CHECK_ARG(mode == 1 || (h % 2 == 0 && w % 2 == 0), "dts_resample2x: down needs even h,w");
  hipStream_t st = to_stream(s);
  const long long total = (long long)n * (mode ? 2 * h : h / 2) * (mode ? 2 * w : w / 2) * (c / epv);
  DTS_DISPATCH_DTYPE(dtype, {
    hipLaunchKernelGGL((resample_kernel<T>), dim3(grid_for(total, 256)), dim3(256), 0, st, (const T*)x, (T*)out, n, h, w, c, mode);
    DTS_CHECK_LAUNCH("dts_resample2x");
  });
  return DTS_OK;
}
```

diffusion_tts_amd/networks.py:

```python
import math
import os
from typing import Dict, Optional

import numpy as np
import torch

from . import ops
from .config import EDMConfig, Block, edm_blocks


def _qkv_perm_edm(heads: int, d: int) -> torch.Tensor:
    s, h, c = torch.meshgrid(torch.arange(3), torch.arange(heads), torch.arange(d), indexing='ij')
    return (h * 3 * d + c * 3 + s).reshape(-1).to(torch.int32)


class _BlockParams:
    pass


class EDMPrecond:

    def __init__(self, cfg: EDMConfig, state_dict: Dict[str, torch.Tensor], device='cuda', dtype=ops.F16X3):
        if not torch.cuda.is_available():
            raise RuntimeError('EDMPrecond (HIP) needs a GPU: there is no CPU fallback in this package')
# ... 86 lines not shown
                P.bqkv = f(g('qkv.bias'))[perm.long()].contiguous()
                P.wproj, P.bproj = ops.pack_conv_weight(f(g('proj.weight')), dt), f(g('proj.bias'))
            self.blocks[n] = P
        self.aff_w = ops.pack_conv_weight(f(torch.cat(aff_w, 0))[:, :, None, None].contiguous(), dt)
        self.aff_b = f(torch.cat(aff_b, 0))
        self.aff_total = off
        r = cfg.img_resolution
        on, oc = ('out_norm', 'out_conv') if self.adm else (f'dec.{r}x{r}_aux_norm', f'dec.{r}x{r}_aux_conv')
        self.out_g, self.out_b = f(sd[f'{on}.weight']), f(sd[f'{on}.bias'])
        ow, ob = sd[f'{oc}.weight'], sd[f'{oc}.bias']
        if ow.shape[0] != cfg.out_channels or ob.shape[0] != cfg.out_channels:
            raise ValueError(f'{oc}: {ow.shape[0]} output channels, {cfg.out_channels} expected for precond={cfg.precond!r}')
        self.out_w = f(ow[:cfg.img_channels]).permute(0, 2, 3, 1).contiguous()
        self.out_cb = f(ob[:cfg.img_channels])
        self.cfin = cfin
        torch.cuda.synchronize(dev)

    def _load_precond(self, state_dict):
        cfg = self.cfg
        self.u = self.u_dev = None
        if self.precond == 'edm':
            return
        self.pre_params = ops.precond_params(self.precond, M=cfg.M, beta_d=cfg.beta_d, beta_min=cfg.beta_min)
        if self.precond == 'iddpm':
            from .checkpoint import check_iddpm_table
            check_iddpm_table(state_dict.get('u'), cfg.M)
            self.u = state_dict['u'].detach().to('cpu', torch.float32).reshape(-1).contiguous()
            self.u_dev = self.u.to(self.device).contiguous()
            torch.cuda.synchronize(self.device)

    def to(self, device):
        return self

    def eval(self):
        return self

    def round_sigma(self, sigma, return_index=False):
        sigma = torch.as_tensor(sigma)
        if self.precond != 'iddpm':
            if return_index:
                raise TypeError('round_sigma(return_index=True): iDDPMPrecond only')
            return sigma
        index = torch.cdist(sigma.to('cpu', torch.float32).reshape(1, -1, 1), self.u.reshape(1, -1, 1)).argmin(2)
        result = index if return_index else self.u[index.flatten()].to(sigma.dtype)
        return result.reshape(sigma.shape).to(sigma.device)

    @staticmethod
    def _groups(c):
        return min(32, c // 4)

    def _embedding(self, c_noise, class_labels, n):
        cfg = self.cfg
        emb = ops.pos_embedding(c_noise, self.freqs, swap=not self.adm)
        if self.adm:
            h = ops.linear(emb, self.map0_w, self.map0_b, act_out=True)
            if not cfg.label_dim:
                return ops.linear(h, self.map1_w, self.map1_b, act_out=True)
            h = ops.linear(h, self.map1_w, self.map1_b)
            lab = self._labels(class_labels, n)
            return ops.linear(lab, self.label_w, None, out=h, accumulate=True, act_out=True)
        if cfg.label_dim:
            lab = self._labels(class_labels, n) * math.sqrt(cfg.label_dim)
            ops.linear(lab.contiguous(), self.label_w, self.label_b, out=emb, accumulate=True)
        h = ops.linear(emb, self.map0_w, self.map0_b, act_out=True)
        return ops.linear(h, self.map1_w, self.map1_b, act_out=True)

    def _labels(self, class_labels, n):
        L = self.cfg.label_dim
        if class_labels is None:
            lab = torch.zeros([1, L], device=self.device)
        else:
            lab = class_labels.to(self.device, torch.float32).reshape(-1, L)
        if lab.shape[0] == 1 and n > 1:
            lab = lab.expand(n, L)
        if lab.shape[0] != n:
            raise ValueError(f'class_labels rows {lab.shape[0]} != batch {n}')
        return lab.contiguous()

    def _block(self, b: Block, x1, x2, aff):
        P = self.blocks[b.name]
        G = self._groups
        ss = aff[:, P.aff_off:P.aff_off + P.caff]
        bnc = None if self.adm else ss
        skip_src = None
        fir = self.fir and (b.up or b.down)
        up = b.up and not fir
        if fir:
            h = ops.group_norm(x1, G(b.cin), self.eps, P.g0, P.b0, x2=x2, silu=True)
            h = ops.conv2d(ops.resample_fir(h, b.up, split_out=self.x3), P.w0, P.cb0, bias_nc=bnc, gn_stats=True)
            if x2 is not None:
                raise NotImplementedError('a resampling block with a concatenated input')
            skip_src = ops.resample_fir(x1, b.up, split_out=self.x3)
        elif self.fuse_gn and not b.down and ops.conv_fuses_gn(x1, P.w0, x2=x2, up=b.up):
            coef = ops.gn_coefficients(x1, G(b.cin), self.eps, P.g0, P.b0, x2=x2)
            h = ops.conv2d(x1, P.w0, P.cb0, x2=x2, up=b.up, bias_nc=bnc, gn_stats=True, gn_coef=coef, gn_silu=True)
        else:
            raw = self.x3 and P.skip_w is not None and os.environ.get('DTS_X3_RAW_SPLIT', '1') != '0'
            h = ops.group_norm(x1, G(b.cin), self.eps, P.g0, P.b0, x2=x2, silu=True, pool=b.down, split_out=self.x3, raw_split=raw)
            if raw:
                h, skip_src = h
            h = ops.conv2d(h, P.w0, P.cb0, up=b.up, bias_nc=bnc, gn_stats=True)
        fuse1 = self.fuse_gn and ops.conv_fuses_gn(h, P.w1)
        if fuse1:
            coef1 = ops.gn_coefficients(h, G(b.cout), self.eps, P.g1, P.b1, scale_shift=ss if self.adm else None)
        else:
            h = ops.group_norm(h, G(b.cout), self.eps, P.g1, P.b1, scale_shift=ss if self.adm else None, silu=True, split_out=self.x3)
        if P.skip_w is not None and skip_src is not None and ops.conv_folds_skip(h, P.w1, (skip_src, P.skip_w, up)):
            sk = None
        elif P.skip_w is not None and skip_src is not None:
            sk = ops.conv2d(skip_src, P.skip_w, P.skip_b, up=up)
        elif P.skip_w is not None:
            src1, src2 = (ops.resample2x(x1, up=False), None) if b.down else (x1, x2)
            sk = ops.conv2d(src1, P.skip_w, P.skip_b, x2=src2, up=b.up)
        elif b.up or b.down:
            sk = ops.resample2x(x1, up=b.up)
        else:
            sk = x1
        if sk is None:
            x = ops.conv2d(h, P.w1, P.cb1_skip, skip=(skip_src, P.skip_w, up), out_scale=self.skip_scale, gn_stats=True)
        else:
            x = ops.conv2d(h, P.w1, P.cb1, residual=sk, out_scale=self.skip_scale, gn_stats=True,
                           gn_coef=coef1 if fuse1 else None, gn_silu=True)
        if b.heads:
            n, hh, ww, c = x.shape
            hn = ops.group_norm(x, G(c), self.eps, P.g2, P.b2, silu=False, split_out=self.x3)
            fx3 = self.x3 and ops.attention_x3_ok(hh * ww, c // b.heads)
            qkv = ops.conv2d(hn, P.wqkv, P.bqkv, out_split2=fx3)
            a = ops.attention(qkv.view(n, hh * ww, 3 * c), b.heads, 1.0 / math.sqrt(c // b.heads), x3=self.x3, split_out=fx3)
            a = ops.SplitAct(a.data.view(n, hh, ww, 2 * c), c) if fx3 else a.view(n, hh, ww, c)
            x = ops.conv2d(a, P.wproj, P.bproj, residual=x, out_scale=self.skip_scale, gn_stats=True)
        return x

    @torch.no_grad()
    def unet(self, xin, c_noise, class_labels):
        n = xin.shape[0]
        emb = self._embedding(c_noise, class_labels, n)
        e = ops.cast_from_f32(emb, self.act_dtype)
        aff = ops.conv2d(e.view(1, n, 1, -1), self.aff_w, self.aff_b).view(n, self.aff_total)
        x = ops.conv_in3(xin, self.conv_in_w, self.conv_in_b, self.enc[0].cout, self.act_dtype)
        skips = [x]
        aux, aux_nchw = xin, True
        for b in self.enc[1:]:
            if b.kind == 'aux_residual':
                P = self.blocks[b.name]
                s2d = ops.space_to_depth2(aux, self.dtype, nchw=aux_nchw, cpad=P.cpad)
                x = ops.conv2d(s2d, P.w, P.b, residual=x, out_scale=math.sqrt(0.5), gn_stats=True)
                skips[-1] = aux = x
                aux_nchw = False
                continue
            x = self._block(b, x, None, aff)
            skips.append(x)
        for b in self.dec:
            x2 = skips.pop() if x.shape[-1] != b.cin else None
            x = self._block(b, x, x2, aff)
        h = ops.group_norm(x, self._groups(self.cfin), 1e-5 if self.adm else 1e-6, self.out_g, self.out_b, silu=True)
        return ops.conv_out3(h, self.out_w, self.out_cb)

    @torch.no_grad()
    def _device_forward(self, x, sigma, class_labels):
        if self.precond == 'edm':
            xin, coef = ops.edm_precond_in(x, sigma, self.sigma_data)
        else:
            xin, coef = ops.precond_in(self.precond, x, sigma, self.pre_params, self.u_dev)
        F = self.unet(xin, coef[:, 3].contiguous(), class_labels)
        return ops.edm_precond_out(x, F, coef)

    @torch.no_grad()
    def __call__(self, x, sigma, class_labels=None, force_fp32=False, **model_kwargs):
        if force_fp32 and self.dtype == torch.float16:
            raise ValueError('force_fp32=True: this network was built with dtype=float16; build it with dtype=ops.F16X3 (default) or float32')
        aug = model_kwargs.pop('augment_labels', None)
        if aug is not None:
            raise NotImplementedError('augment_labels: training-time augmentation conditioning is outside the sampling path (networks.py:330-331)')
        if model_kwargs:
            raise TypeError(f'unexpected keyword arguments {sorted(model_kwargs)} (the reference U-Nets would raise too)')
        x = x.to(self.device, torch.float64).contiguous()
        n = x.shape[0]
        sigma = torch.as_tensor(sigma).to(self.device, torch.float64).reshape(-1).contiguous()
        if sigma.numel() not in (1, n):
            raise ValueError(f'sigma has {sigma.numel()} entries for batch {n}')
        if class_labels is not None:
            class_labels = class_labels.to(self.device, torch.float32).contiguous()
        self.evals += n
        return self._graphs(x, sigma, class_labels)
```

diffusion_tts_amd/ops.py:

```python
import ctypes as C
import math
import os

import torch

from . import _lib as L

_DT = {torch.float32: L.DTS_F32, torch.bfloat16: L.DTS_BF16, torch.float16: L.DTS_F16}

F16X3 = 'f16x3'


def act_dtype(dtype):
    return torch.float32 if dtype == F16X3 else dtype


def dtype_name(dtype):
    return dtype if isinstance(dtype, str) else {torch.float32: 'f32', torch.bfloat16: 'bf16', torch.float16: 'f16'}[dtype]


class X3Weight:

    def __init__(self, packed, acc_scale, shape):
        self.packed, self.acc_scale, self.shape = packed, float(acc_scale), tuple(shape)
# ... 138 lines not shown
    out = torch.empty((O, kh, kw, I), dtype=dtype, device=w.device)
    _call('dts_pack_conv_weight', _ptr(w, 'w', torch.float32), _ptr(out), dt_code(dtype), O, I, kh, kw,
          _ptr(out_perm, 'perm', torch.int32))
    return out


_CONV_WS = {}
CONV_WS_BYTES = 96 << 20


def _conv_workspace(device):
    key = (device.type, device.index)
    ws = _CONV_WS.get(key)
    if ws is None:
        ws = _CONV_WS[key] = torch.empty(CONV_WS_BYTES, dtype=torch.uint8, device=device)
    return ws


def _conv_args(x1, w, x2, up):
    n, hin, win, c1 = x1.shape
    a = L.ConvArgs()
    a.c1, a.c2 = c1, 0 if x2 is None else x2.shape[-1]
    a.n, a.hin, a.win, a.cout, a.ksize = n, hin, win, w.shape[0], w.shape[1]
    a.up, a.dtype = int(up), dt_code(x1.dtype)
    return a


def conv_kernel(x1, w, x2=None, up=False, residual=None, gn_coef=None, gn_stats=False):
    a = _conv_args(x1, w, x2, up)
    if isinstance(w, X3Weight):
        a.c1, a.c2, a.dtype = 2 * (a.c1 + a.c2), 0, L.DTS_F16X3
    a.residual = _ptr(residual)
    a.gn_coef = _ptr(gn_coef, 'gn_coef', torch.float32)
    if up and x2 is None and getattr(w, 'phases', None) is not None:
        a.workspace, a.workspace_bytes = 16, CONV_WS_BYTES
        if gn_stats and (4 * a.hin * a.win) % 64 == 0:
            a.stats_out = 16
        _route_phases(a, w, None)
    return int(L.load().dts_conv_kernel(C.byref(a)))


def _route_phases(a, w, phases):
    if phases is False or getattr(w, 'phases', None) is None or a.up != 1:
        return False
    keep = (a.up, a.w, a.acc_scale)
    a.up, a.w, a.acc_scale = 2, (w.phases.data_ptr() if w.phases.is_cuda else None), w.phase_acc_scale
    if phases is None and not L.load().dts_conv_takes_phases(C.byref(a)):
        a.up, a.w, a.acc_scale = keep
        return False
    return True


def conv_takes_phases(x1, w, bias=None, **kw):
    kw.pop('up', None)
    a, *_keep = _conv2d_args(x1, w, bias, up=True, **kw)
    return a.up == 2


def conv_fuses_gn(x1, w, *, x2=None, up=False):
    return bool(L.load().dts_conv_fuses_gn(C.byref(_conv_args(x1, w, x2, up))))


def _skip_fields(a, skip, n, ho, wo, cout):
    src, sw, sup = skip
    if not isinstance(src, SplitAct) or not isinstance(sw, X3Weight):
        raise ValueError('conv2d: skip = (SplitAct, X3Weight, up)')
    sh = (n, ho // 2, wo // 2) if sup else (n, ho, wo)
    if tuple(src.shape[:3]) != sh or tuple(sw.shape) != (cout, 1, 1, src.shape[3]):
        raise ValueError(f'conv2d: skip source {tuple(src.shape)} / weight {tuple(sw.shape)} do not match an output of {(n, ho, wo, cout)} (up={bool(sup)})')
    a.skip_c, a.skip_x, a.skip_w = src.data.shape[-1], _ptr(src.data, 'skip_x', torch.float16), _ptr(sw.packed, 'skip_w', torch.float16)
    a.skip_acc_scale, a.skip_up = sw.acc_scale, int(bool(sup))


def conv_folds_skip(x1, w, skip):
    if not isinstance(w, X3Weight) or skip is None or not isinstance(skip[0], SplitAct):
        return False
    a = _conv_args(x1, w, None, False)
    a.c1, a.c2, a.dtype = 2 * a.c1, 0, L.DTS_F16X3
    _skip_fields(a, skip, a.n, a.hin, a.win, a.cout)
    return bool(L.load().dts_conv_folds_skip(C.byref(a)))


def _conv2d_args(x1, w, bias=None, *, x2=None, bias_nc=None, residual=None, up=False, out_scale=1.0, out=None, gn_stats=False,
                 timing_events=None, gn_coef=None, gn_silu=True, out_split2=False, skip=None, phases=None):
    n, hin, win, c1 = x1.shape
    c2 = 0 if x2 is None else x2.shape[-1]
    cout, kh, kw, cin = w.shape
    if cin != c1 + c2 or kh != kw:
        raise ValueError(f'conv2d: weight {tuple(w.shape)} does not match inputs ({c1}+{c2})')
    ho, wo = (2 * hin, 2 * win) if up else (hin, win)
    x3 = isinstance(w, X3Weight)
    if x3 and (x1.dtype != torch.float32 or gn_coef is not None):
        raise ValueError('conv2d: a split-precision weight takes float32 activations (and no fused input GroupNorm)')
    if isinstance(x1, SplitAct) and (not x3 or x2 is not None):
        raise ValueError('conv2d: a split activation feeds a split-precision weight, alone')
    out_split2 = bool(out_split2) and x3 and not gn_stats
    if out_split2:
        out = torch.empty((n, ho, wo, 2 * cout), dtype=torch.float16, device=x1.device)
    elif out is None:
        out = torch.empty((n, ho, wo, cout), dtype=x1.dtype, device=x1.device)
    a, xs = L.ConvArgs(), None
    a.out_split2 = int(out_split2)
    dt_in = x1.dtype
    if x3:
        xs = x1.data if isinstance(x1, SplitAct) else split3_f16(x1, x2)
        a.x1, a.c1, a.x2, a.c2 = _ptr(xs, 'x1', torch.float16), 2 * (c1 + c2), None, 0
        a.w, a.acc_scale = _ptr(w.packed, 'w', torch.float16), w.acc_scale
    else:
        a.x1, a.c1 = _ptr(x1, 'x1'), c1
        a.x2, a.c2 = _ptr(x2, 'x2', x1.dtype), c2
        a.w = _ptr(w, 'w', x1.dtype)
    a.bias = _ptr(bias, 'bias', torch.float32)
    a.bias_nc, a.ld_bias_nc = _rows(bias_nc, 'bias_nc', x1.dtype)
    a.residual = _ptr(residual, 'residual', x1.dtype)
    if residual is not None and tuple(residual.shape) != (n, ho, wo, cout):
        raise ValueError(f'conv2d: residual shape {tuple(residual.shape)} != {(n, ho, wo, cout)}')
    a.out = _ptr(out, 'out', torch.float16 if out_split2 else x1.dtype)
    a.n, a.hin, a.win, a.cout, a.ksize = n, hin, win, cout, kh
    a.up, a.out_scale, a.dtype = int(up), float(out_scale), (L.DTS_F16X3 if x3 else dt_code(x1.dtype))
    ws = _conv_workspace(x1.device)
    a.workspace, a.workspace_bytes = ws.data_ptr(), ws.numel()
    st = None
    if gn_stats and (ho * wo) % 64 == 0:
        st = torch.empty(((n * ho * wo) // 64, cout, 2), dtype=torch.float32, device=x1.device)
        a.stats_out = st.data_ptr()
    if timing_events is not None:
        a.ev_start, a.ev_stop = timing_events
    if skip is not None:
        if not x3 or residual is not None or up:
            raise ValueError('conv2d: skip= is the split-precision mode\'s, without residual / upsample')
        _skip_fields(a, skip, n, ho, wo, cout)
    if gn_coef is not None:
        if tuple(gn_coef.shape) != (n, c1 + c2, 2):
            raise ValueError(f'conv2d: gn_coef shape {tuple(gn_coef.shape)} != {(n, c1 + c2, 2)}')
        a.gn_coef, a.gn_silu = _ptr(gn_coef, 'gn_coef', torch.float32), int(gn_silu)
    if x3 and up:
        _route_phases(a, w, phases)
    return a, out, st, out_split2, (xs, ws)


def conv_plan(*args, **kw):
    a, *_keep = _conv2d_args(*args, **kw)
    info = L.ConvPlanInfo()
    _call('dts_conv_plan', C.byref(a), C.byref(info))
    return {f: int(getattr(info, f)) for f, _ in L.ConvPlanInfo._fields_}


def conv2d(x1, w, bias=None, *, x2=None, bias_nc=None, residual=None, up=False, out_scale=1.0, out=None, gn_stats=False,
           timing_events=None, gn_coef=None, gn_silu=True, out_split2=False, skip=None, phases=None):
    a, out, st, out_split2, _keep = _conv2d_args(x1, w, bias, x2=x2, bias_nc=bias_nc, residual=residual, up=up, out_scale=out_scale, out=out,
                                                 gn_stats=gn_stats, timing_events=timing_events, gn_coef=gn_coef, gn_silu=gn_silu,
                                                 out_split2=out_split2, skip=skip, phases=phases)
    _call('dts_conv2d', C.byref(a))
    if out_split2:
        return SplitQKV(out, (out.shape[0], out.shape[1], out.shape[2], out.shape[3] // 2))
    out._gn_stats = st if (st is not None and a.stats_written) else None
    return out


def split3_f16(x1, x2=None):
    n, h, w, c1 = x1.shape
    c2 = 0 if x2 is None else x2.shape[-1]
    out = torch.empty((n, h, w, 2 * (c1 + c2)), dtype=torch.float16, device=x1.device)
    _call('dts_split3_f16', _ptr(x1, 'x1', torch.float32), c1, _ptr(x2, 'x2', torch.float32), c2, _ptr(out), n * h * w)
    return out


def split2_f16(x):
    c = x.shape[-1]
    out = torch.empty(tuple(x.shape[:-1]) + (2 * c,), dtype=torch.float16, device=x.device)
    _call('dts_split2_f16', _ptr(x, 'x', torch.float32), c, _ptr(out), x.numel() // c)
    return out


def _out(who, out, shape, dtype, device):
    if out is None:
        return torch.empty(shape, dtype=dtype, device=device)
    if not torch.is_tensor(out) or tuple(out.shape) != tuple(shape) or out.dtype != dtype or out.device != device:
        raise ValueError(f'{who}: out {tuple(out.shape)} {out.dtype} on {out.device} != {tuple(shape)} {dtype} on {device}'
                         if torch.is_tensor(out) else f'{who}: out is a {type(out).__name__}')
    return out


def conv_in3(x, w, bias, cout, dtype, out=None):
    n, c, h, wd = x.shape
    assert c == 3
    out = _out('conv_in3', out, (n, h, wd, cout), dtype, x.device)
    _call('dts_conv_in3', _ptr(x, 'x', torch.float32), _ptr(w, 'w', torch.float32), _ptr(bias, 'bias', torch.float32),
          _ptr(out, 'out', dtype), dt_code(dtype), n, h, wd, cout)
    return out


def conv_out3(x, w_ohwi, bias, out=None):
    n, h, wd, c = x.shape
    out = _out('conv_out3', out, (n, 3, h, wd), torch.float32, x.device)
    _call('dts_conv_out3', _ptr(x), dt_code(x.dtype), _ptr(w_ohwi, 'w', torch.float32), _ptr(bias, 'bias', torch.float32),
          _ptr(out, 'out', torch.float32), n, h, wd, c)
    return out


def gn_coef(x1, groups, eps, gamma, beta, *, x2=None, scale_shift=None):
    n, h, w, c1 = x1.shape
    c2 = 0 if x2 is None else x2.shape[-1]
    C_ = c1 + c2
    lib = L.load()
    ws = torch.empty((lib.dts_gn_ws_floats(n, groups),), dtype=torch.float32, device=x1.device)
    coef = torch.empty((n, C_, 2), dtype=torch.float32, device=x1.device)
    ss_ptr, ss_ld = _rows(scale_shift, 'scale_shift', x1.dtype)
    _call('dts_gn_coef', _ptr(x1, 'x1'), c1, _ptr(x2, 'x2', x1.dtype), c2, dt_code(x1.dtype), n, h * w, groups, float(eps),
          _ptr(gamma, 'gamma', torch.float32), _ptr(beta, 'beta', torch.float32), ss_ptr, ss_ld, _ptr(coef), _ptr(ws))
    return coef


def gn_apply(x1, coef, *, x2=None, silu=True, pool=False, split_out=False, raw_split=False):
    n, h, w, c1 = x1.shape
    c2 = 0 if x2 is None else x2.shape[-1]
    ho, wo = (h // 2, w // 2) if pool else (h, w)
    if split_out:
        out = torch.empty((n, ho, wo, 2 * (c1 + c2)), dtype=torch.float16, device=x1.device)
        raw = torch.empty_like(out) if raw_split else None
        _call('dts_gn_apply_x3', _ptr(x1, 'x1', torch.float32), c1, _ptr(x2, 'x2', torch.float32), c2, _ptr(coef, 'coef', torch.float32),
              _ptr(out), _ptr(raw), n, h, w, int(silu), int(pool))
        return (SplitAct(out, c1 + c2), SplitAct(raw, c1 + c2)) if raw_split else SplitAct(out, c1 + c2)
    out = torch.empty((n, ho, wo, c1 + c2), dtype=x1.dtype, device=x1.device)
    _call('dts_gn_apply', _ptr(x1, 'x1'), c1, _ptr(x2, 'x2', x1.dtype), c2, dt_code(x1.dtype),
          _ptr(coef, 'coef', torch.float32), _ptr(out), n, h, w, int(silu), int(pool))
    return out


GN_FUSED_MAX_HW = 64


def _coef_from_strips(x1, x2, groups, eps, gamma, beta, scale_shift):
    n, h, w, c1 = x1.shape
    c2 = 0 if x2 is None else x2.shape[-1]
    st1 = getattr(x1, '_gn_stats', None)
    st2 = None if x2 is None else getattr(x2, '_gn_stats', None)
    if st1 is None or (x2 is not None and st2 is None) or (h * w) % 64 != 0:
        return None
    coef = torch.empty((n, c1 + c2, 2), dtype=torch.float32, device=x1.device)
    ss_ptr, ss_ld = _rows(scale_shift, 'scale_shift', x1.dtype)
    _call('dts_gn_coef_strips', _ptr(st1, 'st1', torch.float32), c1, _ptr(st2, 'st2', torch.float32), c2, dt_code(x1.dtype), n,
          h * w, groups, float(eps), _ptr(gamma, 'gamma', torch.float32), _ptr(beta, 'beta', torch.float32), ss_ptr, ss_ld,
          _ptr(coef))
    return coef


def gn_coefficients(x1, groups, eps, gamma, beta, *, x2=None, scale_shift=None):
    coef = _coef_from_strips(x1, x2, groups, eps, gamma, beta, scale_shift)
    return coef if coef is not None else gn_coef(x1, groups, eps, gamma, beta, x2=x2, scale_shift=scale_shift)


def group_norm(x1, groups, eps, gamma, beta, *, x2=None, scale_shift=None, silu=True, pool=False, path=None, split_out=False, raw_split=False):
    n, h, w, c1 = x1.shape
    c2 = 0 if x2 is None else x2.shape[-1]
    cg = (c1 + c2) // groups
    fused_ok = (not pool) and cg % 2 == 0 and cg <= 64
    if path in (None, 'strips'):
        coef = _coef_from_strips(x1, x2, groups, eps, gamma, beta, scale_shift)
        if coef is not None:
            return gn_apply(x1, coef, x2=x2, silu=silu, pool=pool, split_out=split_out, raw_split=raw_split)
    if path == 'strips':
        raise ValueError('strip statistics are not attached to the input(s)')
    if path is None:
        path = 'fused' if (fused_ok and h * w <= GN_FUSED_MAX_HW and not split_out) else 'split'
    if path == 'fused':
        if not fused_ok:
            raise ValueError('fused GroupNorm needs pool=False and an even number (<= 64) of channels per group')
        out = torch.empty((n, h, w, c1 + c2), dtype=x1.dtype, device=x1.device)
        ss_ptr, ss_ld = _rows(scale_shift, 'scale_shift', x1.dtype)
        _call('dts_gn_fused', _ptr(x1, 'x1'), c1, _ptr(x2, 'x2', x1.dtype), c2, dt_code(x1.dtype), n, h * w, groups, float(eps),
              _ptr(gamma, 'gamma', torch.float32), _ptr(beta, 'beta', torch.float32), ss_ptr, ss_ld, _ptr(out), int(silu))
        return out
    return gn_apply(x1, gn_coef(x1, groups, eps, gamma, beta, x2=x2, scale_shift=scale_shift), x2=x2, silu=silu, pool=pool,
                    split_out=split_out, raw_split=raw_split)


def resample2x(x, up):
    n, h, w, c = x.shape
    ho, wo = (2 * h, 2 * w) if up else (h // 2, w // 2)
    out = torch.empty((n, ho, wo, c), dtype=x.dtype, device=x.device)
    _call('dts_resample2x', _ptr(x), _ptr(out), dt_code(x.dtype), n, h, w, c, int(up))
    return out


FIR_TAPS = (1, 3, 3, 1)


def resample_fir(x, up, split_out=False):
    n, h, w, c = x.shape
    ho, wo = (2 * h, 2 * w) if up else (h // 2, w // 2)
    if split_out:
        out = torch.empty((n, ho, wo, 2 * c), dtype=torch.float16, device=x.device)
        _call('dts_resample_fir', _ptr(x, 'x', torch.float32), _ptr(out), L.DTS_F32, n, h, w, c, int(up), 1)
        return SplitAct(out, c)
    out = torch.empty((n, ho, wo, c), dtype=x.dtype, device=x.device)
    _call('dts_resample_fir', _ptr(x), _ptr(out), dt_code(x.dtype), n, h, w, c, int(up), 0)
    return out


def conv_cin_granule(dtype):
    return 32 if dtype in (F16X3, torch.float32) else 64


def space_to_depth2(x, dtype, nchw=False, cpad=None):
    if nchw:
        n, c, h, w = x.shape
    else:
        n, h, w, c = x.shape
    g = conv_cin_granule(dtype)
    cpad = -(-4 * c // g) * g if cpad is None else cpad
    x3, adt = dtype == F16X3, act_dtype(dtype)
    if x.dtype != (torch.float32 if nchw else adt):
        raise ValueError(f'space_to_depth2: input dtype {x.dtype} in compute mode {dtype_name(dtype)}')
    out = torch.empty((n, h // 2, w // 2, 2 * cpad if x3 else cpad), dtype=torch.float16 if x3 else adt, device=x.device)
    _call('dts_space_to_depth2', _ptr(x), int(nchw), _ptr(out), dt_code(adt), n, h, w, c, cpad, int(x3))
    return SplitAct(out, cpad) if x3 else out


def fused_down_weight(w, taps=FIR_TAPS, cpad=None, out_dtype=torch.float32):
    O, Cin, kh, kw = w.shape
    if (kh, kw) != (3, 3) or len(taps) != 4:
        raise ValueError('fused_down_weight: a 3x3 weight and a 4-tap filter')
    k = torch.tensor(list(taps), dtype=torch.float64, device=w.device)
    F2 = torch.outer(k, k) / k.sum() ** 2
    w64 = w.detach().to(torch.float64)
    w6 = torch.zeros((O, Cin, 6, 6), dtype=torch.float64, device=w.device)
    for a in range(4):
        for b in range(4):
            w6[:, :, a:a + 3, b:b + 3] += F2[a, b] * w64
    w3 = w6.view(O, Cin, 3, 2, 3, 2).permute(0, 3, 5, 1, 2, 4).reshape(O, 4 * Cin, 3, 3)
    cpad = 4 * Cin if cpad is None else cpad
    out = torch.zeros((O, cpad, 3, 3), dtype=out_dtype, device=w.device)
    out[:, :4 * Cin] = w3.to(out_dtype)
    return out


def attention(qkv, heads, scale, x3=False, split_out=False):
    n, t, c3 = qkv.shape
    c = c3 // 3
    d = c // heads
    pre = isinstance(qkv, SplitQKV)
    if pre or (x3 and d == 64 and t >= 128 and qkv.dtype == torch.float32):
        if pre:
            sp = qkv.data
        else:
            sp = torch.empty((n, t, 2 * c3), dtype=torch.float16, device=qkv.device)
            _call('dts_split2_f16', _ptr(qkv, 'qkv', torch.float32), c3, _ptr(sp), n * t)
        if split_out:
            out = torch.empty((n, t, 2 * c), dtype=torch.float16, device=qkv.device)
            _call('dts_attention_x3', _ptr(sp), _ptr(out), 1, n, t, heads, d, float(scale))
            return SplitAct(out.view(n, t, 1, 2 * c), c)
        out = torch.empty((n, t, c), dtype=torch.float32, device=qkv.device)
        _call('dts_attention_x3', _ptr(sp), _ptr(out), 0, n, t, heads, d, float(scale))
        return out
    out = torch.empty((n, t, c), dtype=qkv.dtype, device=qkv.device)
    _call('dts_attention', _ptr(qkv), _ptr(out), dt_code(qkv.dtype), n, t, heads, d, float(scale))
    return out
# ... 610 lines not shown
```

include/dts.h:

```cpp
#ifndef DTS_H_
#define DTS_H_

#include <stdint.h>

#ifdef __cplusplus
extern "C" {
#endif

typedef void* dts_stream;

enum dts_dtype { DTS_F32 = 0, DTS_BF16 = 1, DTS_F16 = 2,
                 DTS_F16X3 = 3 };
enum dts_status { DTS_OK = 0, DTS_ERR_ARG = -1, DTS_ERR_LAUNCH = -2, DTS_ERR_UNSUPPORTED = -3 };

#define DTS_ABI_VERSION 125
int dts_version(void);
const char* dts_last_error(void);
int dts_set_tuning(int knob, int value);
int dts_get_tuning(int knob);

int dts_nchw_to_nhwc(const float* src, void* dst, int dtype, int n, int c, int h, int w, dts_stream s);
int dts_nhwc_to_nchw(const void* src, int dtype, float* dst, int n, int c, int h, int w, dts_stream s);
int dts_nchw_to_nhwc_pad(const float* src, void* dst, int dtype, int n, int c, int h, int w, int cpad, dts_stream s);
int dts_pack_conv_weight(const float* w_oihw, void* dst, int dtype, int O, int I, int kh, int kw,
                         const int32_t* out_perm, dts_stream s);

typedef struct dts_conv_args {
  const void* x1; int32_t c1;
  const void* x2; int32_t c2;
  const void* w;
  const float* bias;
  const void* bias_nc;
  int32_t ld_bias_nc;
  const void* residual;
  void* out;
  int32_t n, hin, win;
  int32_t cout;
  int32_t ksize;
  int32_t up;
  float out_scale;
  int32_t dtype;
  void* workspace;
  int64_t workspace_bytes;
  float* stats_out;
  int32_t stats_written;
  void* ev_start; void* ev_stop;
  const float* gn_coef;
  int32_t gn_silu;
  float acc_scale;
  int32_t out_split2;
  int32_t skip_c;
  const void* skip_x;
  const void* skip_w;
  float skip_acc_scale;
  int32_t skip_up;
} dts_conv_args;
int dts_conv_fuses_gn(const dts_conv_args* a);
int dts_conv_folds_skip(const dts_conv_args* a);
int dts_conv_takes_phases(const dts_conv_args* a);
int dts_conv_kernel(const dts_conv_args* a);
typedef struct dts_conv_plan_info {
  int32_t kernel;
  int32_t tile, waves, stages, pf;
  int32_t gn, sk, dbg;
  int32_t splits, ks_per_split;
  int32_t n_ct, n_pt, nblk;
  int32_t threads, lds_bytes;
  int32_t stats_in_kernel, stats_in_reduce, stats_written;
  int32_t epi_rows;
  int32_t fuses_gn, folds_skip;
  int32_t refused;
  int32_t phases;
} dts_conv_plan_info;
int dts_conv_plan(const dts_conv_args* a, dts_conv_plan_info* out);
int dts_conv2d(dts_conv_args* a, dts_stream s);

int dts_conv_in3(const float* x, const float* w, const float* bias, void* out, int dtype,
                 int n, int h, int w_, int cout, dts_stream s);
int dts_conv_out3(const void* x, int dtype, const float* w, const float* bias, float* out,
                  int n, int h, int w_, int c, dts_stream s);

int64_t dts_gn_ws_floats(int n, int groups);
int dts_gn_coef(const void* x1, int c1, const void* x2, int c2, int dtype, int n, int hw, int groups, float eps,
                const float* gamma, const float* beta, const void* scale_shift, int ld_ss,
                float* coef, float* ws, dts_stream s);
int dts_gn_coef_strips(const float* st1, int c1, const float* st2, int c2, int dtype, int n, int hw, int groups, float eps,
                       const float* gamma, const float* beta, const void* scale_shift, int ld_ss, float* coef, dts_stream s);
int dts_gn_apply(const void* x1, int c1, const void* x2, int c2, int dtype, const float* coef,
                 void* out, int n, int h, int w, int silu, int pool, dts_stream s);
int dts_gn_apply_x3(const float* x1, int c1, const float* x2, int c2, const float* coef, void* out, void* raw_out, int n, int h, int w, int silu,
                    int pool, dts_stream s);
int dts_gn_fused(const void* x1, int c1, const void* x2, int c2, int dtype, int n, int hw, int groups, float eps,
                 const float* gamma, const float* beta, const void* scale_shift, int ld_ss, void* out, int silu, dts_stream s);
int dts_resample2x(const void* x, void* out, int dtype, int n, int h, int w, int c, int mode, dts_stream s);
int dts_resample_fir(const void* x, void* out, int dtype, int n, int h, int w, int c, int up, int split_out, dts_stream s);
int dts_space_to_depth2(const void* x, int x_nchw_f32, void* out, int dtype, int n, int h, int w, int c, int cpad, int split_out, dts_stream s);

int dts_attention(const void* qkv, void* out, int dtype, int n, int t, int heads, int d, float scale, dts_stream s);
int dts_attention_x3(const void* qkv_split, void* out, int out_split3, int n, int t, int heads, int d, float scale, dts_stream s);
int dts_attention_masked(const void* qkv, void* out, int dtype, int n, int t, int heads, int d, float scale, int causal,
                         const int32_t* key_len, dts_stream s);
int dts_attention_x3_masked(const void* qkv_split, void* out, int out_split3, int n, int t, int heads, int d, float scale, int causal,
                            const int32_t* key_len, dts_stream s);

int dts_cross_attention(const void* q, const void* kv, const int32_t* kv_rows, int kv_n, void* out, int dtype, int n, int tq, int tk,
                        int heads, int d, float scale, dts_stream s);
int dts_layer_norm(const void* x, void* out, int dtype, int64_t rows, int c, float eps, const float* gamma, const float* beta, dts_stream s);
int dts_geglu(const void* x, void* out, int dtype, int64_t rows, int inner, dts_stream s);
int dts_group_rows(const void* rows, int n, int64_t row_bytes, void* workspace, int32_t* slot, int32_t* reps, int32_t* count, dts_stream s);

int dts_patchify(const float* x, void* out, int dtype, int n, int size, int patch, int kpad, dts_stream s);
int dts_vit_tokens(const void* patches, const float* cls, const float* pos, void* tokens, int dtype, int n, int t, int c, dts_stream s);
int dts_gelu(const void* x, void* out, int dtype, int64_t count, int kind, dts_stream s);
int dts_text_tokens(const int32_t* ids, const float* tok, const float* pos, void* out, int dtype, int n, int t, int c, int vocab, dts_stream s);
int dts_vit_head(const void* tokens, float* out, int dtype, int n, int t, int c, float eps, const float* gamma, const float* beta, dts_stream s);

int dts_layer_norm_x3(const float* x, float* out_f32, void* out_split, int64_t rows, int c, float eps, const float* gamma, const float* beta,
                      dts_stream s);
int dts_gelu_x3(const float* x, void* out_split, int64_t rows, int c, int kind, dts_stream s);
int dts_patchify_x3(const float* x, void* out_split, int n, int size, int patch, int kpad, dts_stream s);
int dts_vit_tokens_f32(const float* patches, const float* cls, const float* pos, float* tokens, int n, int t, int c, dts_stream s);
int dts_vit_head_f32(const float* tokens, float* out, int n, int t, int c, float eps, const float* gamma, const float* beta, dts_stream s);
int dts_text_tokens_f32(const int32_t* ids, const float* tok, const float* pos, float* out, int n, int t, int c, int vocab, dts_stream s);

int dts_linear(const float* x, int ldx, const float* w, const float* bias, float* y, int ldy,
               int m, int k, int n, int act_in, int act_out, int accumulate, dts_stream s);
int dts_pos_embedding(const float* v, const float* freqs, float* out, int n, int half, int swap, dts_stream s);
int dts_edm_precond_in(const double* x, const double* sigma, int nsigma, float sigma_data,
                       float* xin, float* coef, int n, int chw, dts_stream s);
enum dts_precond_kind { DTS_PRECOND_VP = 1, DTS_PRECOND_VE = 2, DTS_PRECOND_IDDPM = 3 };
#define DTS_PRECOND_NPARAMS 5
int dts_precond_in(int kind, const float* params, const float* table, int table_n, const double* x, const double* sigma, int nsigma,
                   float* xin, float* coef, int n, int chw, dts_stream s);
int dts_edm_precond_out(const double* x, const float* F, const float* coef, float* D, int n, int chw, dts_stream s);
int dts_split3_f16(const float* x1, int c1, const float* x2, int c2, void* out, int64_t rows, dts_stream s);
int dts_split2_f16(const float* x, int c, void* out, int64_t rows, dts_stream s);
int dts_cast_from_f32(const float* src, void* dst, int dtype, int64_t count, dts_stream s);
int dts_cast_to_f32(const void* src, int dtype, float* dst, int64_t count, dts_stream s);

int dts_heun_xhat(const double* x_cur, int xb, int bcast, const void* eps, int eps_f32, double noise_coef,
                  double* x_hat, int nb, int chw, dts_stream s);
int dts_heun_euler(const double* x_hat, const float* D, double t_hat, double t_next,
                   double* d_cur, double* x_next, int64_t count, dts_stream s);
int dts_heun_correct(const double* x_hat, const float* D2, const double* d_cur, double t_hat, double t_next,
                     double* x_next, int64_t count, dts_stream s);

int dts_ode_xhat(const double* x_cur, const void* eps, int eps_f32, double ratio, double noise_coef, double s_hat,
                 double* x_hat, double* x_in, int64_t count, dts_stream s);
int dts_ode_slope(const double* x, const float* D, double a, double b, const double* base, double step, double s_out,
                  double* d, double* x_out, double* x_in, int64_t count, dts_stream s);
int dts_ode_correct(const double* x_hat, const double* x_prime, const float* D2, const double* d_cur, double a, double b,
                    double h, double w0, double w1, double* x_next, int64_t count, dts_stream s);

int dts_quantize_u8(const void* x, int is_f32, uint8_t* out, int64_t count, dts_stream s);
int dts_brightness(const uint8_t* img, float* rewards, int n, int hw, dts_stream s);
int dts_cosine_rows(const float* a, const float* b, int b_rows, float* out, int n, int d, dts_stream s);
int dts_resample_u8(const uint8_t* src, uint8_t* dst, int planes, int h, int w, int out_len, int axis, const int32_t* bounds,
                    const int32_t* coefs, int ksize, dts_stream s);
int dts_lut_u8_f32(const uint8_t* img, const float* lut, float* out, int n, int c, int hw, dts_stream s);
int dts_u8_to_unit_f32(const uint8_t* img, float* out, int64_t count, dts_stream s);

int64_t dts_jpeg_workspace_bytes(int n, int h, int w);
int dts_jpeg_size(const uint8_t* img, int32_t* sizes, int n, int h, int w, const uint16_t* qtab, void* workspace, int64_t workspace_bytes,
                  int16_t* coef_out, dts_stream s);

int dts_attnpool_tokens(const void* x, const float* pos, void* tokens, int dtype, int n, int hw, int c, dts_stream s);
int dts_take_token(const void* src, int dtype, float* out, int n, int t, int c, int token, dts_stream s);
int dts_softmax_gather(const float* logits, const int32_t* target, float* rewards, int n, int k, dts_stream s);

int dts_candidate_noise(const double* pivot, const double* g, const int32_t* mode, const float* scale,
                        double* cand, int nb, int b, int chw, dts_stream s);
int dts_candidate_noise_rows(const double* pivot, const double* g, const int32_t* mode, const float* scale,
                             double* cand, int nb, int b, int chw, dts_stream s);
int dts_candidate_noise_sd(const void* pivot, const void* u, const int32_t* mode, const float* scale, void* cand, int dtype, int n,
// ... 15 lines not shown
```

Before: 1532 candidate U-Net steps/sec.

## Read half-resolution residuals in place and emit pooled skip from GroupNorm pass

Adds a residual_up mode to the conv epilogues and split-K reduces, so a 3x3 conv at upsampled resolution reads the residual from the half-resolution tensor directly instead of from a separately materialized upsampled copy. The GroupNorm apply pass on down blocks can also write the pooled raw input alongside the normalized output, removing a separate resample2x pass. Both remove full-tensor memory passes and kernel launches, at the cost of more template instantiations, an ABI change to the conv args struct, and strided gather loads in the epilogue.

```diff
diff --git a/diffusion_tts_amd/_lib.py b/diffusion_tts_amd/_lib.py
--- a/diffusion_tts_amd/_lib.py
+++ b/diffusion_tts_amd/_lib.py
@@ -18,13 +18,14 @@
                 ('ksize', C.c_int32), ('up', C.c_int32), ('out_scale', C.c_float), ('dtype', C.c_int32),
                 ('workspace', _p), ('workspace_bytes', C.c_int64), ('stats_out', _p), ('stats_written', C.c_int32),
                 ('ev_start', _p), ('ev_stop', _p), ('gn_coef', _p), ('gn_silu', C.c_int32), ('acc_scale', C.c_float), ('out_split2', C.c_int32),
-                ('skip_c', C.c_int32), ('skip_x', _p), ('skip_w', _p), ('skip_acc_scale', C.c_float), ('skip_up', C.c_int32)]
+                ('skip_c', C.c_int32), ('skip_x', _p), ('skip_w', _p), ('skip_acc_scale', C.c_float), ('skip_up', C.c_int32),
+                ('residual_up', C.c_int32)]
 
 
 class ConvPlanInfo(C.Structure):
     _fields_ = [(f, C.c_int32) for f in ('kernel', 'tile', 'waves', 'stages', 'pf', 'gn', 'sk', 'dbg', 'splits', 'ks_per_split', 'n_ct', 'n_pt', 'nblk',
                                          'threads', 'lds_bytes', 'stats_in_kernel', 'stats_in_reduce', 'stats_written', 'epi_rows', 'fuses_gn',
-                                         'folds_skip', 'refused', 'phases')]
+                                         'folds_skip', 'refused', 'phases', 'residual_up_ok')]
 
 
 SIGNATURES = {
@@ -39,6 +40,7 @@
     'dts_gn_coef_strips': [_p, _i, _p, _i, _i, _i, _i, _i, _f, _p, _p, _p, _i, _p, _p],
     'dts_gn_apply': [_p, _i, _p, _i, _i, _p, _p, _i, _i, _i, _i, _i, _p],
     'dts_gn_apply_x3': [_p, _i, _p, _i, _p, _p, _p, _i, _i, _i, _i, _i, _p],
+    'dts_gn_apply_x3_pooled': [_p, _i, _p, _i, _p, _p, _p, _p, _i, _i, _i, _i, _p],
     'dts_gn_fused': [_p, _i, _p, _i, _i, _i, _i, _i, _f, _p, _p, _p, _i, _p, _i, _p],
     'dts_resample2x': [_p, _p, _i, _i, _i, _i, _i, _i, _p],
     'dts_resample_fir': [_p, _p, _i, _i, _i, _i, _i, _i, _i, _p],
@@ -95,7 +97,7 @@
     'dts_ddim_candidates': [_p, _p, _p, _p, _p, _i, _f, _f, _f, _i, _i64, _p],
     'dts_ddim_candidates_groups': [_p, _p, _p, _p, _p, _i, _f, _f, _f, _i, _i, _i64, _p],
 }
-OTHER = {'dts_version': ([], _i), 'dts_conv_fuses_gn': ([C.POINTER(ConvArgs)], _i), 'dts_conv_kernel': ([C.POINTER(ConvArgs)], _i), 'dts_conv_folds_skip': ([C.POINTER(ConvArgs)], _i), 'dts_conv_takes_phases': ([C.POINTER(ConvArgs)], _i), 'dts_conv_plan': ([C.POINTER(ConvArgs), C.POINTER(ConvPlanInfo)], _i), 'dts_set_tuning': ([_i, _i], _i), 'dts_get_tuning': ([_i], _i), 'dts_last_error': ([], C.c_char_p), 'dts_gn_ws_floats': ([_i, _i], _i64),
+OTHER = {'dts_version': ([], _i), 'dts_conv_args_size': ([], _i), 'dts_conv_fuses_gn': ([C.POINTER(ConvArgs)], _i), 'dts_conv_kernel': ([C.POINTER(ConvArgs)], _i), 'dts_conv_folds_skip': ([C.POINTER(ConvArgs)], _i), 'dts_conv_takes_phases': ([C.POINTER(ConvArgs)], _i), 'dts_conv_residual_up_ok': ([C.POINTER(ConvArgs)], _i), 'dts_conv_plan': ([C.POINTER(ConvArgs), C.POINTER(ConvPlanInfo)], _i), 'dts_set_tuning': ([_i, _i], _i), 'dts_get_tuning': ([_i], _i), 'dts_last_error': ([], C.c_char_p), 'dts_gn_ws_floats': ([_i, _i], _i64),
          'dts_jpeg_workspace_bytes': ([_i, _i, _i], _i64)}
 
 _lib = None
@@ -110,6 +112,9 @@
         raise RuntimeError(f'{LIB_PATH} not found: the HIP extension is required (no CPU fallback). '
                            f'Build it with `python -m diffusion_tts_amd.build` or __graft_entry__.build().')
     lib = C.CDLL(LIB_PATH)
+    missing = [name for name in list(SIGNATURES) + list(OTHER) if not hasattr(lib, name)]
+    if missing:
+        raise RuntimeError(f'{LIB_PATH} lacks {missing}: rebuild with `python -m diffusion_tts_amd.build --force`')
     for name, argt in SIGNATURES.items():
         fn = getattr(lib, name)
         fn.argtypes, fn.restype = argt, _i
@@ -117,7 +122,7 @@
         fn = getattr(lib, name)
         fn.argtypes, fn.restype = argt, rest
     got = lib.dts_version()
-    if got != ABI_VERSION or C.sizeof(ConvArgs) != 208:
+    if got != ABI_VERSION or C.sizeof(ConvArgs) != 216 or lib.dts_conv_args_size() != C.sizeof(ConvArgs):
         raise RuntimeError(f'{LIB_PATH} has ABI version {got}, this binding needs {ABI_VERSION}: rebuild with `python -m diffusion_tts_amd.build --force`')
     _lib = lib
     return lib
diff --git a/diffusion_tts_amd/classifier.py b/diffusion_tts_amd/classifier.py
--- a/diffusion_tts_amd/classifier.py
+++ b/diffusion_tts_amd/classifier.py
@@ -75,8 +75,9 @@
     def _res(self, L: ClsLayer, x, emb_all):
         P = self.params[L.prefix]
         raw = self.x3 and P.sw is not None
-        h = ops.group_norm(x, 32, 1e-5, P.g0, P.b0, silu=True, pool=L.down, split_out=self.x3, raw_split=raw)
-        if raw:
+        pooled = self.x3 and L.down and not raw and ops.residual_in_place()
+        h = ops.group_norm(x, 32, 1e-5, P.g0, P.b0, silu=True, pool=L.down, split_out=self.x3, raw_split=raw, pooled_out=pooled)
+        if raw or pooled:
             h, x = h
         elif L.down:
             x = ops.resample2x(x, up=False)
diff --git a/diffusion_tts_amd/csrc/conv_igemm.hip b/diffusion_tts_amd/csrc/conv_igemm.hip
--- a/diffusion_tts_amd/csrc/conv_igemm.hip
+++ b/diffusion_tts_amd/csrc/conv_igemm.hip
@@ -2,9 +2,11 @@
 #include <hip/hip_ext.h>
 #include <type_traits>
 
-static_assert(sizeof(dts_conv_args) == 208, "dts_conv_args layout changed: bump DTS_ABI_VERSION and update the bindings (_lib.py ConvArgs)");
+static_assert(sizeof(dts_conv_args) == 216, "dts_conv_args layout changed: update the bindings (_lib.py ConvArgs checks dts_conv_args_size()) and see DTS_ABI_VERSION");
 
 int dts_conv_launch_phase_form(const void* plan, const void* params, const void* call);
+int dts_conv_launch_res_up_form(const void* plan, const void* params, const void* call);
+int dts_conv_launch_res_up_reduce(const void* params, int with_stats, const void* call);
 
 namespace {
 
@@ -44,6 +46,21 @@
   float sk_ratio;
 };
 
+__device__ __forceinline__ int residual_up_row(const ConvP& kp, int pp) {
+  int n, y, x;
+  if (kp.hw_shift >= 0) {
+    n = pp >> kp.hw_shift;
+    const int rem = pp & ((1 << kp.hw_shift) - 1);
+    y = rem >> kp.w_shift; x = rem & ((1 << kp.w_shift) - 1);
+  } else {
+    const int hw = kp.hout * kp.wout;
+    n = pp / hw;
+    const int rem = pp - n * hw;
+    y = rem / kp.wout; x = rem - y * kp.wout;
+  }
+  return (n * (kp.hout >> 1) + (y >> 1)) * (kp.wout >> 1) + (x >> 1);
+}
+
 template <typename T> struct Mma;
 template <> struct Mma<bf16_t> {
   static __device__ __forceinline__ void run(f32x4_t& acc, const uint4& a, const uint4& b) {
@@ -360,7 +377,7 @@
   }
 }
 
-template <int MT, int NT, typename TM = TileMap>
+template <int MT, int NT, bool RU = false, typename TM = TileMap>
 __device__ __forceinline__ void conv_epilogue_rows_f32(const ConvP& kp, f32x4_t (&acc)[MT][NT], int cm0, const TM& tm, int wm, int wn,
                                                        int lrow, int lq, char* smem, int wave) {
   static_assert(NT == 4, "64-pixel wave strips");
@@ -403,9 +420,10 @@
     float4 rv[CH];
 #pragma unroll
     for (int u = 0; u < CH; ++u) {
-      prow[u] = (size_t)tm.pix(wn * 64 + half * 32 + (u0 + u) * RPI + (act ? rsub : 0)) * p_cout + co;
+      const int pp = tm.pix(wn * 64 + half * 32 + (u0 + u) * RPI + (act ? rsub : 0));
+      prow[u] = (size_t)pp * p_cout + co;
       rv[u] = make_float4(0.f, 0.f, 0.f, 0.f);
-      if (res && act) rv[u] = *reinterpret_cast<const float4*>(res + prow[u]);
+      if (res && act) rv[u] = *reinterpret_cast<const float4*>(res + (RU ? (size_t)residual_up_row(kp, pp) * p_cout + co : prow[u]));
     }
 #pragma unroll
     for (int u = 0; u < CH; ++u) {
@@ -459,7 +477,7 @@
   }
 }
 
-template <typename T, int MT, int NT, int BM, int BN, int NTHR, int RING, typename TM = TileMap>
+template <typename T, int MT, int NT, int BM, int BN, int NTHR, int RING, bool RU = false, typename TM = TileMap>
 __device__ __forceinline__ void conv_epilogue(const ConvP& kp, f32x4_t (&acc)[MT][NT], int cm0, const TM& tm, int split, int wm, int wn,
                                               int lrow, int lq, char* smem, bool bias_in_acc, int stage_off, int early_u0, int early_u1) {
   const int p_P = kp.P, p_cout = kp.cout, p_hout = kp.hout, p_wout = kp.wout;
@@ -482,7 +500,7 @@
     constexpr int NWV = NTHR / 64;
     static_assert(NWV * 32 * (16 * MT * 4 + 16) <= RING, "the waves' private transpose slices must fit the caller's LDS ring");
     if (kp.epi_rows && (p_hout * p_wout) % 64 == 0) {
-      conv_epilogue_rows_f32<MT, NT>(kp, acc, cm0, tm, wm, wn, lrow, lq, smem, (int)(threadIdx.x >> 6));
+      conv_epilogue_rows_f32<MT, NT, RU>(kp, acc, cm0, tm, wm, wn, lrow, lq, smem, (int)(threadIdx.x >> 6));
       return;
     }
   }
@@ -609,7 +627,7 @@
   }
 }
 
-template <typename T, int MT, int NT, int WM, int WN, bool PF, int STAGES = 2, typename OT = T, bool PH = false>
+template <typename T, int MT, int NT, int WM, int WN, bool PF, int STAGES = 2, typename OT = T, bool PH = false, bool RU = false>
 __global__ __launch_bounds__(64 * WM * WN, (WM * WN == 8 || STAGES == 2 ? 2 : 1)) void conv_igemm_kernel(const ConvP kp) {
   const char* const p_x1 = kp.x1; const char* const p_x2 = kp.x2; const char* const p_w = kp.w;
   const int p_c1 = kp.c1, p_c2 = kp.c2, p_cin = kp.cin, p_hin = kp.hin, p_win = kp.win, p_hout = kp.hout, p_wout = kp.wout;
@@ -837,9 +855,9 @@
   if constexpr (PH) {
     const bool sh = kp.hw_shift >= 0;
     const PhaseTileMap tm{pn0, ph_y, ph_x, p_win, p_hin * p_win, sh ? g_w_shift : -1, sh ? g_hw_shift : -1};
-    conv_epilogue<OT, MT, NT, BM, BN, 64 * NW, RING_BYTES>(kp, acc, cm0, tm, (int)blockIdx.y, wm, wn, lrow, lq, smem, bias_in_acc, stage_off, early_u0, early_u1);
+    conv_epilogue<OT, MT, NT, BM, BN, 64 * NW, RING_BYTES, RU>(kp, acc, cm0, tm, (int)blockIdx.y, wm, wn, lrow, lq, smem, bias_in_acc, stage_off, early_u0, early_u1);
   } else
-  conv_epilogue<OT, MT, NT, BM, BN, 64 * NW, RING_BYTES>(kp, acc, cm0, linear_tile(pn0), (int)blockIdx.y, wm, wn, lrow, lq, smem, bias_in_acc, stage_off, early_u0, early_u1);
+  conv_epilogue<OT, MT, NT, BM, BN, 64 * NW, RING_BYTES, RU>(kp, acc, cm0, linear_tile(pn0), (int)blockIdx.y, wm, wn, lrow, lq, smem, bias_in_acc, stage_off, early_u0, early_u1);
   DTS_STAMP(3);
   DTS_STAMP_RT(5);
 }
@@ -859,7 +877,7 @@
   return pack16<T>(f);
 }
 
-template <typename T, int TAPS, int DBG = 0, bool GN = false, int MT = 6, typename OT = T, bool SK = false>
+template <typename T, int TAPS, int DBG = 0, bool GN = false, int MT = 6, typename OT = T, bool SK = false, bool RU = false>
 __global__ __launch_bounds__(512, 2) void conv_pp_kernel(const ConvP kp) {
   static_assert(MT == 6 || MT == 4, "cout tile");
   constexpr bool X3I = !std::is_same<T, OT>::value;
@@ -1276,12 +1294,12 @@
   __syncthreads();
   DTS_STAMP(2);
 
-  conv_epilogue<OT, MT, NT, BM, BN, NTHR, H_OFF + 2 * H_BUF>(kp, acc, cm0, tm, (int)blockIdx.y, wm, wn, lrow, lq, smem, bias_in_acc, 0, 0, 0);
+  conv_epilogue<OT, MT, NT, BM, BN, NTHR, H_OFF + 2 * H_BUF, RU>(kp, acc, cm0, tm, (int)blockIdx.y, wm, wn, lrow, lq, smem, bias_in_acc, 0, 0, 0);
   DTS_STAMP(3);
   DTS_STAMP_RT(5);
 }
 
-template <typename T, int SPLITS>
+template <typename T, int SPLITS, bool RU = false>
 __global__ __launch_bounds__(256) void conv_splitk_reduce_kernel(const ConvP kp) {
   const long long total = (long long)kp.P * (kp.cout / 4);
   const T* res = reinterpret_cast<const T*>(kp.residual);
@@ -1310,7 +1328,7 @@
     }
     if (res) {
       float f[4];
-      Vec4<T>::load(res + (size_t)pp * kp.cout + co, f);
+      Vec4<T>::load(res + (size_t)(RU ? residual_up_row(kp, pp) : pp) * kp.cout + co, f);
       for (int r = 0; r < 4; ++r) v[r] += f[r];
     }
     for (int r = 0; r < 4; ++r) v[r] *= kp.out_scale;
@@ -1318,7 +1336,7 @@
   }
 }
 
-template <typename T, int SPLITS>
+template <typename T, int SPLITS, bool RU = false>
 __global__ __launch_bounds__(256) void conv_splitk_reduce_stats_kernel(const ConvP kp) {
   __shared__ float red[16][16][8];
   const int strip = blockIdx.x, q = threadIdx.x & 15, pl = threadIdx.x >> 4;
@@ -1359,7 +1377,7 @@
       if (bnc) { for (int r = 0; r < 4; ++r) v[i][r] += nb[r]; }
       if (res) {
         float f[4];
-        Vec4<T>::load(res + (size_t)pp * kp.cout + co, f);
+        Vec4<T>::load(res + (size_t)(RU ? residual_up_row(kp, pp) : pp) * kp.cout + co, f);
         for (int r = 0; r < 4; ++r) v[i][r] += f[r];
       }
       for (int r = 0; r < 4; ++r) v[i][r] *= kp.out_scale;
@@ -1392,15 +1410,15 @@
   return d;
 }
 
-template <typename T, int SPLITS>
+template <typename T, int SPLITS, bool RU = false>
 int launch_reduce_n(const ConvP& q, bool with_stats, hipStream_t st) {
   if (with_stats) {
-    hipLaunchKernelGGL((conv_splitk_reduce_stats_kernel<T, SPLITS>), dim3(q.P / 64, (q.cout + 63) / 64), dim3(256), 0, st, q);
+    hipLaunchKernelGGL((conv_splitk_reduce_stats_kernel<T, SPLITS, RU>), dim3(q.P / 64, (q.cout + 63) / 64), dim3(256), 0, st, q);
     DTS_CHECK_LAUNCH("dts_conv2d(split-K reduce + statistics)");
   } else {
     long long g = ((long long)q.P * (q.cout / 4) + 255) / 256;
     if (g > 2048) g = 2048;
-    hipLaunchKernelGGL((conv_splitk_reduce_kernel<T, SPLITS>), dim3((int)g), dim3(256), 0, st, q);
+    hipLaunchKernelGGL((conv_splitk_reduce_kernel<T, SPLITS, RU>), dim3((int)g), dim3(256), 0, st, q);
     DTS_CHECK_LAUNCH("dts_conv2d(split-K reduce)");
   }
   return DTS_OK;
@@ -1428,7 +1446,7 @@
           dts_knob_get(DTS_KNOB_CONV_EPI32), dts_knob_get(DTS_KNOB_CONV_SKIP_FOLD), dts_knob_get(DTS_KNOB_CONV_UP_PHASES), f32_192};
 }
 
-struct ConvPlan : dts_conv_plan_info { char refuse[200]; };
+struct ConvPlan : dts_conv_plan_info { int res_up; char refuse[200]; };
 
 template <auto KERNEL>
 int conv_launch(const ConvPlan& pl, const ConvP& q, const ConvCall& call) {
@@ -1447,9 +1465,9 @@
   return DTS_OK;
 }
 
-template <typename T, typename OT, int MT, int WM, int WN, bool PF, bool PH = false>
+template <typename T, typename OT, int MT, int WM, int WN, bool PF, bool PH = false, bool RU = false>
 int conv_launch_igemm(const ConvPlan& pl, const ConvP& q, const ConvCall& call) {
-#define DTS_IGEMM(MT_, WM_, STAGES_) conv_launch<&conv_igemm_kernel<T, MT_, 4, WM_, WN, PF, STAGES_, OT, PH>>(pl, q, call)
+#define DTS_IGEMM(MT_, WM_, STAGES_) conv_launch<&conv_igemm_kernel<T, MT_, 4, WM_, WN, PF, STAGES_, OT, PH, RU>>(pl, q, call)
   if constexpr (sizeof(T) == 2) {
     if (pl.waves == 8) return pl.stages == 3 ? DTS_IGEMM(MT / 2, WM * 2, 3) : DTS_IGEMM(MT / 2, WM * 2, 2);
     if (pl.stages == 3) return DTS_IGEMM(MT, WM, 3);
@@ -1551,6 +1569,7 @@
 #define DTS_PP(DBG_, GN_, MT_, SK_) conv_launch<&conv_pp_kernel<T, 9, DBG_, GN_, MT_, OT, SK_>>(pl, q, call)
     if constexpr (!std::is_same<T, OT>::value) {
       if (pl.phases) return dts_conv_launch_phase_form(&pl, &q, &call);
+      if (pl.res_up) return dts_conv_launch_res_up_form(&pl, &q, &call);
       if (pl.kernel == 6 && pl.sk) return DTS_PP(0, false, 6, true);
       if (pl.kernel == 4 && pl.sk) return DTS_PP(0, false, 4, true);
     } else if (pl.kernel == 6) {
@@ -1680,6 +1699,12 @@
   pl.stats_written = pl.stats_in_kernel || pl.stats_in_reduce;
   pl.epi_rows = k.epi32 < 0 ? (x3 ? 1 : 0) : (k.epi32 == 2 ? 2 : (k.epi32 != 0));
   if (ph && (a->hin * a->win) % 64 != 0) pl.epi_rows = 0;
+  pl.residual_up_ok = x3 && !ph && !pl.sk && a->ksize == 3 && ((p.hout | p.wout) & 1) == 0 &&
+                      (pl.splits > 1 || (pl.epi_rows != 0 && (p.hout * p.wout) % 64 == 0));
+  if (a->residual_up != 0 && (a->residual_up != 1 || a->residual == nullptr || !pl.residual_up_ok))
+    return refuse("dts_conv2d: residual_up = %d for a launch that cannot read a half-resolution residual in place (hout %d, wout %d; ask dts_conv_residual_up_ok first)",
+                  a->residual_up, p.hout, p.wout);
+  pl.res_up = a->residual_up;
   if (mt != 0) return pl;
   const bool one_per_cu = (long long)pl.nblk * pl.splits <= 256;
   pl.stages = (one_per_cu && pl.ks_per_split >= 3) ? 3 : 2;
@@ -1703,6 +1728,33 @@
   const ConvCall& c = *static_cast<const ConvCall*>(call);
   return pl.tile == 192 ? conv_launch_igemm<f16_t, float, 6, 2, 2, true, true>(pl, q, c) : conv_launch_igemm<f16_t, float, 4, 2, 2, true, true>(pl, q, c);
 }
+int dts_conv_launch_res_up_form(const void* plan, const void* params, const void* call) {
+  const ConvPlan& pl = *static_cast<const ConvPlan*>(plan);
+  const ConvP& q = *static_cast<const ConvP*>(params);
+  const ConvCall& c = *static_cast<const ConvCall*>(call);
+  if (pl.kernel == 6) return conv_launch<&conv_pp_kernel<f16_t, 9, 0, false, 6, float, false, true>>(pl, q, c);
+  if (pl.kernel == 4) return conv_launch<&conv_pp_kernel<f16_t, 9, 0, false, 4, float, false, true>>(pl, q, c);
+  if (!pl.pf) { dts_set_error("dts_conv2d: residual_up without fragment prefetch (a 1x1 launch)"); return DTS_ERR_ARG; }
+  switch (pl.tile) {
+    case 192: return conv_launch_igemm<f16_t, float, 6, 2, 2, true, false, true>(pl, q, c);
+    case 128: return conv_launch_igemm<f16_t, float, 4, 2, 2, true, false, true>(pl, q, c);
+    default: return conv_launch_igemm<f16_t, float, 4, 1, 4, true, false, true>(pl, q, c);
+  }
+}
+int dts_conv_launch_res_up_reduce(const void* params, int with_stats, const void* call) {
+  const ConvP& q = *static_cast<const ConvP*>(params);
+  const hipStream_t st = static_cast<const ConvCall*>(call)->st;
+  switch (q.splits) {
+    case 2: return launch_reduce_n<float, 2, true>(q, with_stats != 0, st);
+    case 3: return launch_reduce_n<float, 3, true>(q, with_stats != 0, st);
+    case 4: return launch_reduce_n<float, 4, true>(q, with_stats != 0, st);
+    case 5: return launch_reduce_n<float, 5, true>(q, with_stats != 0, st);
+    case 6: return launch_reduce_n<float, 6, true>(q, with_stats != 0, st);
+    case 7: return launch_reduce_n<float, 7, true>(q, with_stats != 0, st);
+    case 8: return launch_reduce_n<float, 8, true>(q, with_stats != 0, st);
+    default: dts_set_error("dts_conv2d: split-K factor %d outside 2..8", q.splits); return DTS_ERR_ARG;
+  }
+}
 #else
 
 #ifdef DTS_STAMPS
@@ -1723,9 +1775,13 @@
 
 extern "C" int dts_conv_kernel(const dts_conv_args* a) { return conv_plan(a).kernel; }
 
+extern "C" int dts_conv_args_size(void) { return (int)sizeof(dts_conv_args); }
+
 extern "C" int dts_conv_fuses_gn(const dts_conv_args* a) { return conv_plan(a).fuses_gn ? 1 : 0; }
 
 extern "C" int dts_conv_folds_skip(const dts_conv_args* a) { return conv_plan(a).folds_skip ? 1 : 0; }
+
+extern "C" int dts_conv_residual_up_ok(const dts_conv_args* a) { return conv_plan(a).residual_up_ok ? 1 : 0; }
 
 extern "C" int dts_conv_takes_phases(const dts_conv_args* a) {
   if (a == nullptr || a->up != 2) return 0;
@@ -1779,7 +1835,8 @@
   else DTS_DISPATCH_DTYPE(a->dtype, rc = conv_launch_plan<T>(pl, p, call));
   if (rc == DTS_OK && pl.splits > 1) {
     if (pl.stats_in_reduce) p.stats = a->stats_out;
-    DTS_DISPATCH_DTYPE(a->dtype == DTS_F16X3 ? DTS_F32 : a->dtype, rc = launch_reduce<T>(p, pl.stats_in_reduce, call.st));
+    if (pl.res_up) rc = dts_conv_launch_res_up_reduce(&p, pl.stats_in_reduce ? 1 : 0, &call);
+    else DTS_DISPATCH_DTYPE(a->dtype == DTS_F16X3 ? DTS_F32 : a->dtype, rc = launch_reduce<T>(p, pl.stats_in_reduce, call.st));
   }
   a->stats_written = pl.stats_written ? 1 : 0;
   return rc;
diff --git a/diffusion_tts_amd/csrc/groupnorm.hip b/diffusion_tts_amd/csrc/groupnorm.hip
--- a/diffusion_tts_amd/csrc/groupnorm.hip
+++ b/diffusion_tts_amd/csrc/groupnorm.hip
@@ -242,7 +242,8 @@
 template <typename T, bool POOL, bool SPLIT = false>
 __global__ __launch_bounds__(256) void gn_apply_kernel(const T* __restrict__ x1, int c1, const T* __restrict__ x2, int c2,
                                                         const float* __restrict__ coef, T* __restrict__ out,
-                                                        int n_total, int h, int w, int silu, f16_t* __restrict__ raw = nullptr) {
+                                                        int n_total, int h, int w, int silu, f16_t* __restrict__ raw = nullptr,
+                                                        float* __restrict__ pooled = nullptr) {
   constexpr int EPV = ET<T>::EPV;
   const int C = c1 + c2, nchunk = C / EPV;
   const int ho = POOL ? h / 2 : h, wo = POOL ? w / 2 : w;
@@ -286,6 +287,9 @@
     if constexpr (SPLIT) {
       store_split4(reinterpret_cast<f16_t*>(out) + (((size_t)n * ho + yo) * wo + xo) * 2 * C, c0, r);
       if (raw) store_split4(raw + (((size_t)n * ho + yo) * wo + xo) * 2 * C, c0, rr);
+      if constexpr (POOL) {
+        if (pooled) *reinterpret_cast<float4*>(pooled + (((size_t)n * ho + yo) * wo + xo) * C + c0) = make_float4(rr[0], rr[1], rr[2], rr[3]);
+      }
     } else
       *reinterpret_cast<uint4*>(out + (((size_t)n * ho + yo) * wo + xo) * C + c0) = pack16<T>(r);
   }
@@ -469,7 +473,7 @@
 }
 
 static int gn_apply_impl(const void* x1, int c1, const void* x2, int c2, int dtype, const float* coef, void* out, int n, int h,
-                         int w, int silu, int pool, bool split, dts_stream s, void* raw_out = nullptr);
+                         int w, int silu, int pool, bool split, dts_stream s, void* raw_out = nullptr, float* pooled_out = nullptr);
 extern "C" int dts_gn_apply(const void* x1, int c1, const void* x2, int c2, int dtype, const float* coef, void* out, int n, int h,
                             int w, int silu, int pool, dts_stream s) {
   return gn_apply_impl(x1, c1, x2, c2, dtype, coef, out, n, h, w, silu, pool, false, s);
@@ -479,8 +483,14 @@
   DTS_CHECK_ARG((c1 + c2) % 32 == 0, "dts_gn_apply_x3: %d channels are not a multiple of 32", c1 + c2);
   return gn_apply_impl(x1, c1, x2, c2, DTS_F32, coef, out, n, h, w, silu, pool, true, s, raw_out);
 }
+extern "C" int dts_gn_apply_x3_pooled(const float* x1, int c1, const float* x2, int c2, const float* coef, void* out, void* raw_out,
+                                      float* pooled_out, int n, int h, int w, int silu, dts_stream s) {
+  DTS_CHECK_ARG((c1 + c2) % 32 == 0, "dts_gn_apply_x3_pooled: %d channels are not a multiple of 32", c1 + c2);
+  DTS_CHECK_ARG(pooled_out == nullptr || (uintptr_t)pooled_out % 16 == 0, "dts_gn_apply_x3_pooled: pooled_out is not 16-byte aligned");
+  return gn_apply_impl(x1, c1, x2, c2, DTS_F32, coef, out, n, h, w, silu, 1, true, s, raw_out, pooled_out);
+}
 static int gn_apply_impl(const void* x1, int c1, const void* x2, int c2, int dtype, const float* coef, void* out, int n, int h,
-                         int w, int silu, int pool, bool split, dts_stream s, void* raw_out) {
+                         int w, int silu, int pool, bool split, dts_stream s, void* raw_out, float* pooled_out) {
   const int C = c1 + c2;
   DTS_CHECK_ARG(x1 && coef && out, "dts_gn_apply: null pointer");
   DTS_CHECK_ARG(n > 0 && h > 0 && w > 0 && C > 0, "dts_gn_apply: n=%d h=%d w=%d C=%d", n, h, w, C);
@@ -494,7 +504,7 @@
     using T = float;
     if (pool)
       hipLaunchKernelGGL((gn_apply_kernel<T, true, true>), dim3(grid_for(total, 256)), dim3(256), 0, st, (const T*)x1, c1, (const T*)x2,
-                         c2, coef, (T*)out, n, h, w, silu, (f16_t*)raw_out);
+                         c2, coef, (T*)out, n, h, w, silu, (f16_t*)raw_out, pooled_out);
     else if (C / epv <= 256 && n <= 65535) {
       const int nchunk = C / epv, k = 256 / nchunk, hw = h * w;
       long long ppb = ((long long)n * hw + 4095) / 4096;
diff --git a/diffusion_tts_amd/networks.py b/diffusion_tts_amd/networks.py
--- a/diffusion_tts_amd/networks.py
+++ b/diffusion_tts_amd/networks.py
@@ -192,7 +192,8 @@
         G = self._groups
         ss = aff[:, P.aff_off:P.aff_off + P.caff]
         bnc = None if self.adm else ss
-        skip_src = None
+        skip_src = pooled = None
+        res_up = False
         fir = self.fir and (b.up or b.down)
         up = b.up and not fir
         if fir:
@@ -206,9 +207,13 @@
             h = ops.conv2d(x1, P.w0, P.cb0, x2=x2, up=b.up, bias_nc=bnc, gn_stats=True, gn_coef=coef, gn_silu=True)
         else:
             raw = self.x3 and P.skip_w is not None and os.environ.get('DTS_X3_RAW_SPLIT', '1') != '0'
-            h = ops.group_norm(x1, G(b.cin), self.eps, P.g0, P.b0, x2=x2, silu=True, pool=b.down, split_out=self.x3, raw_split=raw)
+            want_pooled = self.x3 and b.down and P.skip_w is None and x2 is None and ops.residual_in_place()
+            h = ops.group_norm(x1, G(b.cin), self.eps, P.g0, P.b0, x2=x2, silu=True, pool=b.down, split_out=self.x3, raw_split=raw,
+                               pooled_out=want_pooled)
             if raw:
                 h, skip_src = h
+            elif want_pooled:
+                h, pooled = h
             h = ops.conv2d(h, P.w0, P.cb0, up=b.up, bias_nc=bnc, gn_stats=True)
         fuse1 = self.fuse_gn and ops.conv_fuses_gn(h, P.w1)
         if fuse1:
@@ -222,6 +227,11 @@
         elif P.skip_w is not None:
             src1, src2 = (ops.resample2x(x1, up=False), None) if b.down else (x1, x2)
             sk = ops.conv2d(src1, P.skip_w, P.skip_b, x2=src2, up=b.up)
+        elif b.down and pooled is not None:
+            sk = pooled
+        elif b.up and self.x3 and not fuse1 and ops.residual_in_place() and \
+                ops.conv_residual_up_ok(h, P.w1, P.cb1, residual=x1, out_scale=self.skip_scale, gn_stats=True):
+            sk, res_up = x1, True
         elif b.up or b.down:
             sk = ops.resample2x(x1, up=b.up)
         else:
@@ -229,7 +239,7 @@
         if sk is None:
             x = ops.conv2d(h, P.w1, P.cb1_skip, skip=(skip_src, P.skip_w, up), out_scale=self.skip_scale, gn_stats=True)
         else:
-            x = ops.conv2d(h, P.w1, P.cb1, residual=sk, out_scale=self.skip_scale, gn_stats=True,
+            x = ops.conv2d(h, P.w1, P.cb1, residual=sk, residual_up=res_up, out_scale=self.skip_scale, gn_stats=True,
                            gn_coef=coef1 if fuse1 else None, gn_silu=True)
         if b.heads:
             n, hh, ww, c = x.shape
diff --git a/diffusion_tts_amd/ops.py b/diffusion_tts_amd/ops.py
--- a/diffusion_tts_amd/ops.py
+++ b/diffusion_tts_amd/ops.py
@@ -244,7 +244,7 @@
 
 
 def _conv2d_args(x1, w, bias=None, *, x2=None, bias_nc=None, residual=None, up=False, out_scale=1.0, out=None, gn_stats=False,
-                 timing_events=None, gn_coef=None, gn_silu=True, out_split2=False, skip=None, phases=None):
+                 timing_events=None, gn_coef=None, gn_silu=True, out_split2=False, skip=None, phases=None, residual_up=False):
     n, hin, win, c1 = x1.shape
     c2 = 0 if x2 is None else x2.shape[-1]
     cout, kh, kw, cin = w.shape
@@ -275,8 +275,12 @@
     a.bias = _ptr(bias, 'bias', torch.float32)
     a.bias_nc, a.ld_bias_nc = _rows(bias_nc, 'bias_nc', x1.dtype)
     a.residual = _ptr(residual, 'residual', x1.dtype)
-    if residual is not None and tuple(residual.shape) != (n, ho, wo, cout):
-        raise ValueError(f'conv2d: residual shape {tuple(residual.shape)} != {(n, ho, wo, cout)}')
+    if residual_up and (residual is None or ho % 2 or wo % 2):
+        raise ValueError(f'conv2d: residual_up needs a residual and an even output size, got {(ho, wo)}')
+    rshape = (n, ho // 2, wo // 2, cout) if residual_up else (n, ho, wo, cout)
+    if residual is not None and tuple(residual.shape) != rshape:
+        raise ValueError(f'conv2d: residual shape {tuple(residual.shape)} != {rshape}')
+    a.residual_up = int(bool(residual_up))
     a.out = _ptr(out, 'out', torch.float16 if out_split2 else x1.dtype)
     a.n, a.hin, a.win, a.cout, a.ksize = n, hin, win, cout, kh
     a.up, a.out_scale, a.dtype = int(up), float(out_scale), (L.DTS_F16X3 if x3 else dt_code(x1.dtype))
@@ -308,11 +312,26 @@
     return {f: int(getattr(info, f)) for f, _ in L.ConvPlanInfo._fields_}
 
 
+def conv_residual_up_ok(x1, w, bias=None, **kw):
+    if not isinstance(w, X3Weight):
+        return False
+    kw.pop('residual_up', None)
+    res = kw.pop('residual', None)
+    n, hin, win, _ = x1.shape
+    ho, wo = (2 * hin, 2 * win) if kw.get('up') else (hin, win)
+    if ho % 2 or wo % 2:
+        return False
+    a, *_keep = _conv2d_args(x1, w, bias, residual=res, residual_up=res is not None, **kw)
+    if res is None:
+        a.residual = 16
+    return bool(L.load().dts_conv_residual_up_ok(C.byref(a)))
+
+
 def conv2d(x1, w, bias=None, *, x2=None, bias_nc=None, residual=None, up=False, out_scale=1.0, out=None, gn_stats=False,
-           timing_events=None, gn_coef=None, gn_silu=True, out_split2=False, skip=None, phases=None):
+           timing_events=None, gn_coef=None, gn_silu=True, out_split2=False, skip=None, phases=None, residual_up=False):
     a, out, st, out_split2, _keep = _conv2d_args(x1, w, bias, x2=x2, bias_nc=bias_nc, residual=residual, up=up, out_scale=out_scale, out=out,
                                                  gn_stats=gn_stats, timing_events=timing_events, gn_coef=gn_coef, gn_silu=gn_silu,
-                                                 out_split2=out_split2, skip=skip, phases=phases)
+                                                 out_split2=out_split2, skip=skip, phases=phases, residual_up=residual_up)
     _call('dts_conv2d', C.byref(a))
     if out_split2:
         return SplitQKV(out, (out.shape[0], out.shape[1], out.shape[2], out.shape[3] // 2))
@@ -374,13 +393,20 @@
     return coef
 
 
-def gn_apply(x1, coef, *, x2=None, silu=True, pool=False, split_out=False, raw_split=False):
+def gn_apply(x1, coef, *, x2=None, silu=True, pool=False, split_out=False, raw_split=False, pooled_out=False):
+    if pooled_out and not (pool and split_out):
+        raise ValueError('gn_apply: pooled_out is the pool pass\'s, in split-precision form (pool=True, split_out=True)')
     n, h, w, c1 = x1.shape
     c2 = 0 if x2 is None else x2.shape[-1]
     ho, wo = (h // 2, w // 2) if pool else (h, w)
     if split_out:
         out = torch.empty((n, ho, wo, 2 * (c1 + c2)), dtype=torch.float16, device=x1.device)
         raw = torch.empty_like(out) if raw_split else None
+        if pooled_out:
+            pooled = torch.empty((n, ho, wo, c1 + c2), dtype=torch.float32, device=x1.device)
+            _call('dts_gn_apply_x3_pooled', _ptr(x1, 'x1', torch.float32), c1, _ptr(x2, 'x2', torch.float32), c2, _ptr(coef, 'coef', torch.float32),
+                  _ptr(out), _ptr(raw), _ptr(pooled), n, h, w, int(silu))
+            return (SplitAct(out, c1 + c2), SplitAct(raw, c1 + c2), pooled) if raw_split else (SplitAct(out, c1 + c2), pooled)
         _call('dts_gn_apply_x3', _ptr(x1, 'x1', torch.float32), c1, _ptr(x2, 'x2', torch.float32), c2, _ptr(coef, 'coef', torch.float32),
               _ptr(out), _ptr(raw), n, h, w, int(silu), int(pool))
         return (SplitAct(out, c1 + c2), SplitAct(raw, c1 + c2)) if raw_split else SplitAct(out, c1 + c2)
@@ -413,7 +439,10 @@
     return coef if coef is not None else gn_coef(x1, groups, eps, gamma, beta, x2=x2, scale_shift=scale_shift)
 
 
-def group_norm(x1, groups, eps, gamma, beta, *, x2=None, scale_shift=None, silu=True, pool=False, path=None, split_out=False, raw_split=False):
+def group_norm(x1, groups, eps, gamma, beta, *, x2=None, scale_shift=None, silu=True, pool=False, path=None, split_out=False, raw_split=False,
+               pooled_out=False):
+    if pooled_out and not (pool and split_out):
+        raise ValueError('group_norm: pooled_out needs pool=True and split_out=True')
     n, h, w, c1 = x1.shape
     c2 = 0 if x2 is None else x2.shape[-1]
     cg = (c1 + c2) // groups
@@ -421,7 +450,7 @@
     if path in (None, 'strips'):
         coef = _coef_from_strips(x1, x2, groups, eps, gamma, beta, scale_shift)
         if coef is not None:
-            return gn_apply(x1, coef, x2=x2, silu=silu, pool=pool, split_out=split_out, raw_split=raw_split)
+            return gn_apply(x1, coef, x2=x2, silu=silu, pool=pool, split_out=split_out, raw_split=raw_split, pooled_out=pooled_out)
     if path == 'strips':
         raise ValueError('strip statistics are not attached to the input(s)')
     if path is None:
@@ -435,7 +464,11 @@
               _ptr(gamma, 'gamma', torch.float32), _ptr(beta, 'beta', torch.float32), ss_ptr, ss_ld, _ptr(out), int(silu))
         return out
     return gn_apply(x1, gn_coef(x1, groups, eps, gamma, beta, x2=x2, scale_shift=scale_shift), x2=x2, silu=silu, pool=pool,
-                    split_out=split_out, raw_split=raw_split)
+                    split_out=split_out, raw_split=raw_split, pooled_out=pooled_out)
+
+
+def residual_in_place():
+    return os.environ.get('DTS_RESIDUAL_IN_PLACE', '1') != '0'
 
 
 def resample2x(x, up):
diff --git a/include/dts.h b/include/dts.h
--- a/include/dts.h
+++ b/include/dts.h
@@ -15,6 +15,7 @@
 
 #define DTS_ABI_VERSION 125
 int dts_version(void);
+int dts_conv_args_size(void);
 const char* dts_last_error(void);
 int dts_set_tuning(int knob, int value);
 int dts_get_tuning(int knob);
@@ -54,9 +55,11 @@
   const void* skip_w;
   float skip_acc_scale;
   int32_t skip_up;
+  int32_t residual_up;
 } dts_conv_args;
 int dts_conv_fuses_gn(const dts_conv_args* a);
 int dts_conv_folds_skip(const dts_conv_args* a);
+int dts_conv_residual_up_ok(const dts_conv_args* a);
 int dts_conv_takes_phases(const dts_conv_args* a);
 int dts_conv_kernel(const dts_conv_args* a);
 typedef struct dts_conv_plan_info {
@@ -71,6 +74,7 @@
   int32_t fuses_gn, folds_skip;
   int32_t refused;
   int32_t phases;
+  int32_t residual_up_ok;
 } dts_conv_plan_info;
 int dts_conv_plan(const dts_conv_args* a, dts_conv_plan_info* out);
 int dts_conv2d(dts_conv_args* a, dts_stream s);
@@ -90,6 +94,8 @@
                  void* out, int n, int h, int w, int silu, int pool, dts_stream s);
 int dts_gn_apply_x3(const float* x1, int c1, const float* x2, int c2, const float* coef, void* out, void* raw_out, int n, int h, int w, int silu,
                     int pool, dts_stream s);
+int dts_gn_apply_x3_pooled(const float* x1, int c1, const float* x2, int c2, const float* coef, void* out, void* raw_out, float* pooled_out,
+                           int n, int h, int w, int silu, dts_stream s);
 int dts_gn_fused(const void* x1, int c1, const void* x2, int c2, int dtype, int n, int hw, int groups, float eps,
                  const float* gamma, const float* beta, const void* scale_shift, int ld_ss, void* out, int silu, dts_stream s);
 int dts_resample2x(const void* x, void* out, int dtype, int n, int h, int w, int c, int mode, dts_stream s);
```

Result: no change. 1543 candidate U-Net steps/sec (median of 6 runs) (+0.7%).
